# dnbaker/dashing

Hardware: AMD Instinct MI355X
Metric: genome-pairs/sec, all-pairs HLL Jaccard (Ertl-MLE), N=10000 p=14 (higher is better)
Workload: dtype u8/u32 popcount + f64 estimator; 1 GPU; BASELINE configs[2]: 10000 synthetic sketches, p=14 (16384 B each), all-pairs dist on MI355X; n_sketches=10000, p=14, k=31, estimator=ERTL_MLE

## Files before the change

### dashing_amd/csrc/abi.hip

```cpp
#include <algorithm>
#include <cstdlib>
#include <cstring>
#include <new>

#include "ctx.h"

using namespace dsh;

extern "C" {

const char *dsh_backend_name(void) { return "hip:gfx950"; }

int dsh_abi_version(void) { return DSH_ABI_VERSION; }

int dsh_device_count(void)
{
    int n = 0;
    if (hipGetDeviceCount(&n) != hipSuccess) return 0;
    return n;
}

static void release_ctx(dsh_ctx *c)
{
    (void)hipSetDevice(c->device);
    for (const Stream *s : {&c->stream, &c->copy_stream, &c->aux_stream, &c->place_stream})
        if (*s) (void)hipStreamSynchronize(*s);
    if (c->xch.spin_running && c->xch.spin_flag.ptr) *(volatile uint32_t *)c->xch.spin_flag.ptr = 1;
    if (c->spin_stream) (void)hipStreamSynchronize(c->spin_stream);
    c->xch.spin_running = false;
    (void)comm_release(c);
}

int dsh_create(int device, dsh_ctx **out)
{
    if (!out) return DSH_EINVAL;
    *out = nullptr;
    int n = 0;
    if (hipGetDeviceCount(&n) != hipSuccess || n <= 0) return DSH_ENODEV;
    if (device < 0 || device >= n) return DSH_EINVAL;
    hipDeviceProp_t prop;
    if (hipGetDeviceProperties(&prop, device) != hipSuccess) return DSH_ENODEV;
    if (std::strncmp(prop.gcnArchName, "gfx950", 6) != 0) return DSH_ENODEV;
    dsh_ctx *c = new (std::nothrow) dsh_ctx;
    if (!c) return DSH_ENOMEM;
    c->device = device;
    if (hipSetDevice(device) != hipSuccess ||
        c->stream.create() != hipSuccess || c->copy_stream.create_copy() != hipSuccess ||
        c->aux_stream.create() != hipSuccess || c->place_stream.create_copy() != hipSuccess ||
        c->ev_aux_fork.ensure() != hipSuccess || c->ev_aux_join.ensure() != hipSuccess) {
        release_ctx(c);
        delete c;
        return DSH_EIO;
    }
    *out = c;
    return DSH_OK;
}

void dsh_destroy(dsh_ctx *c)
{
    if (!c) return;
    release_ctx(c);
    delete c;
}

int dsh_preload(int device, unsigned what)
{
    if (hipSetDevice(device) != hipSuccess) {
        (void)hipGetLastError();
        return DSH_ENODEV;
    }
    hipError_t e = hipSuccess;
    if ((what & DSH_PRELOAD_SKETCH) && e == hipSuccess) e = preload_sketch_kernels();
    if ((what & DSH_PRELOAD_SKETCH) && e == hipSuccess) e = preload_fastx_kernels();
    if ((what & DSH_PRELOAD_COMPARE) && e == hipSuccess) e = preload_compare_kernels();
    if ((what & DSH_PRELOAD_COMPARE) && e == hipSuccess) e = preload_hist_kernels();
    if ((what & DSH_PRELOAD_COMPARE) && e == hipSuccess) e = preload_knn_kernels();
    if ((what & DSH_PRELOAD_COMPARE) && e == hipSuccess) e = preload_exchange_kernels();
    if (e != hipSuccess) (void)hipGetLastError();
    return e == hipSuccess ? DSH_OK : DSH_EIO;
}

const char *dsh_last_error(const dsh_ctx *c) { return c ? c->err.c_str() : "null ctx"; }

int dsh_synchronize(dsh_ctx *c)
{
    if (!c) return DSH_EINVAL;
    int rc = bind(c);
    if (rc) return rc;
    HIPCHK(c, hipStreamSynchronize(c->stream));
    HIPCHK(c, hipStreamSynchronize(c->copy_stream));
    HIPCHK(c, hipStreamSynchronize(c->place_stream));
    return DSH_OK;
}

void *dsh_stream(dsh_ctx *c) { return c ? (void *)c->stream : nullptr; }

int dsh_sketches_alloc(dsh_ctx *c, uint64_t n, int p)
{
    if (!c) return DSH_EINVAL;
    if (p < 4 || p > kMaxP) return fail(c, DSH_EINVAL, "p=%d outside [4,%d]", p, kMaxP);
    int rc = bind(c);
    if (rc) return rc;
    const size_t bytes = std::max<size_t>((size_t)n << p, 256);
    HIPCHK(c, c->regs_own.ensure(bytes));
    HIPCHK(c, hipMemsetAsync(c->regs_own.ptr, 0, bytes, c->stream));
    c->regs = (const uint8_t *)c->regs_own.ptr;
    c->n = n;
    c->p = p;
    c->have_sketches = true;
    invalidate(c);
    return DSH_OK;
}

int dsh_attach_device_sketches(dsh_ctx *c, const void *d_regs, uint64_t n, int p)
{
    if (!c || (!d_regs && n)) return DSH_EINVAL;
    if (p < 4 || p > kMaxP) return fail(c, DSH_EINVAL, "p=%d outside [4,%d]", p, kMaxP);
    if (((uintptr_t)d_regs & 15) != 0) return fail(c, DSH_EINVAL, "device sketches must be 16-byte aligned");
    c->regs = (const uint8_t *)d_regs;
    c->n = n;
    c->p = p;
    c->have_sketches = true;
    invalidate(c);
    return DSH_OK;
}

int dsh_upload_sketches(dsh_ctx *c, const uint8_t *regs, uint64_t first, uint64_t n)
{
    if (!c || (!regs && n)) return DSH_EINVAL;
    if (!c->have_sketches || c->regs != (const uint8_t *)c->regs_own.ptr)
        return fail(c, DSH_ESTATE, "dsh_sketches_alloc first");
    if (!slots_ok(first, n, c->n)) return fail(c, DSH_EINVAL, "slots [%llu,+%llu) out of range", (unsigned long long)first, (unsigned long long)n);
    int rc = bind(c);
    if (rc) return rc;
    if (n) {
        HIPCHK(c, hipMemcpyAsync((uint8_t *)c->regs_own.ptr + (first << c->p), regs, (size_t)n << c->p,
                                 hipMemcpyHostToDevice, c->stream));
        HIPCHK(c, hipStreamSynchronize(c->stream));
    }
    invalidate(c);
    return DSH_OK;
}

int dsh_download_sketches(dsh_ctx *c, uint64_t first, uint64_t n, uint8_t *out)
{
    if (!c || (!out && n)) return DSH_EINVAL;
    if (!c->have_sketches) return fail(c, DSH_ESTATE, "no sketches");
    if (!slots_ok(first, n, c->n)) return fail(c, DSH_EINVAL, "slots out of range");
    int rc = bind(c);
    if (rc) return rc;
    if (n) {
        HIPCHK(c, hipMemcpyAsync(out, c->regs + (first << c->p), (size_t)n << c->p,
                                 hipMemcpyDeviceToHost, c->stream));
        HIPCHK(c, hipStreamSynchronize(c->stream));
    }
    return DSH_OK;
}

// ... 650 lines not shown

int dsh_last_kernel_ms(dsh_ctx *c, double *pair_ms, double *fin_ms, double *prep_ms, uint32_t *launches)
{
    if (!c) return DSH_EINVAL;
    if (pair_ms) *pair_ms = c->pair_ms;
    if (fin_ms) *fin_ms = c->fin_ms;
    if (prep_ms) *prep_ms = c->prep_ms;
    if (launches) *launches = c->pair_launches;
    return DSH_OK;
}

int dsh_last_part_info(dsh_ctx *c, double *ready_ms, uint64_t *floats, uint32_t cap, uint32_t *nparts_out)
{
    if (!c || !nparts_out) return DSH_EINVAL;
    const uint32_t k = (uint32_t)c->part_ready_ms.size();
    *nparts_out = k;
    if (k > cap && (ready_ms || floats)) return DSH_EINVAL;
    for (uint32_t q = 0; q < k; ++q) {
        if (ready_ms) ready_ms[q] = c->part_ready_ms[q];
        if (floats) floats[q] = c->part_floats[q];
    }
    return DSH_OK;
}

int dsh_finalize_phase_cycles(dsh_ctx *c, uint64_t *out16)
{
    if (!c || !out16) return DSH_EINVAL;
    int rc = bind(c);
    if (rc) return rc;
    if (!c->phase_cyc.ptr) return fail(c, DSH_ESTATE, "no call with the option finalize_timing yet");
    HIPCHK(c, hipStreamSynchronize(c->stream));
    HIPCHK(c, hipMemcpy(out16, c->phase_cyc.ptr, 16 * sizeof(uint64_t), hipMemcpyDeviceToHost));
    return DSH_OK;
}

int dsh_get_info(dsh_ctx *c, const char *name, int64_t *out)
{
    if (!c || !name || !out) return DSH_EINVAL;
    if (!std::strcmp(name, "planes")) *out = c->lay.P;
    else if (!std::strcmp(name, "vlo")) *out = c->lay.vlo;
    else if (!std::strcmp(name, "vhi")) *out = c->lay.vhi;
    else if (!std::strcmp(name, "threshold")) *out = c->lay.pbase + (int64_t)c->lay.P;
    else if (!std::strcmp(name, "pbase")) *out = c->lay.pbase;
    else if (!std::strcmp(name, "host_layout_us")) *out = (int64_t)c->host_layout_us;
    else if (!std::strcmp(name, "host_lists_us")) *out = (int64_t)c->host_lists_us;
    else if (!std::strcmp(name, "host_keys_wait_us")) *out = (int64_t)c->host_keys_wait_us;
    else if (!std::strcmp(name, "emax")) *out = c->emax;
    else if (!std::strcmp(name, "elow")) *out = c->elow;
    else if (!std::strcmp(name, "kc")) *out = c->kc;
    else if (!std::strcmp(name, "pair_groups")) *out = c->pair_groups;
    else if (!std::strcmp(name, "pair_round")) *out = c->pp.band_round.empty() ? 0 : c->pp.band_round[0];
    else if (!std::strcmp(name, "tile")) *out = kTile;
    else if (!std::strcmp(name, "parts_done")) *out = c->parts_done;
    else if (!std::strcmp(name, "parts_signalled")) *out = c->parts_signalled ? 1 : 0;
    else if (!std::strcmp(name, "sketch_kernel_us")) *out = (int64_t)(c->sketch_ms * 1000.0);
    else if (!std::strcmp(name, "fastx_decode_us")) *out = (int64_t)(c->fastx_ms * 1000.0);
    else if (!std::strcmp(name, "xch_recv_gated")) *out = c->xch.recv_gated ? 1 : 0;
    else if (!std::strcmp(name, "stats_route")) *out = c->gs.route_last;
    else if (!std::strcmp(name, "linkage_route")) *out = c->lk.route_last;
    else if (!std::strcmp(name, "mst_rounds")) *out = c->mst.rounds_last;
    else if (!std::strcmp(name, "mst_band_us")) *out = (int64_t)(c->mst.band_ms * 1000.0);
    else if (!std::strcmp(name, "place_kernel_us")) *out = (int64_t)(c->xch.place_ms * 1000.0);
    else if (!std::strcmp(name, "whatif_mfma")) {
#ifdef DSH_WHATIF_MFMA
        *out = 1;
#else
        *out = 0;
#endif
    }
    else if (!std::strcmp(name, "npad")) *out = c->lay.Npad;
    else if (!std::strcmp(name, "kpad")) *out = c->Kpad;
    else if (!std::strcmp(name, "cum_bytes")) *out = c->cum_bytes;
    else if (!std::strcmp(name, "sorted")) *out = c->lay.sorted;
    else if (!std::strcmp(name, "ncols")) *out = (int64_t)c->lay.ncols;
    else if (!std::strcmp(name, "lockstep")) *out = c->planes_valid && use_lockstep(c) ? 1 : 0;
    else if (!std::strcmp(name, "tiles")) *out = (int64_t)c->pp.T.size();
    else if (!std::strcmp(name, "bands")) *out = (int64_t)c->last_bands;
    else if (!std::strcmp(name, "items")) *out = (int64_t)c->pp.items.size();
    else if (!std::strcmp(name, "frag_items")) {
        uint64_t f = 0;
        for (uint32_t x : c->pp.band_frags) f += x;
        *out = (int64_t)f;
    }
    else if (!std::strcmp(name, "words_per_plane")) *out = c->W;
    else if (!std::strcmp(name, "avg_tile_planes_x100")) {
        uint64_t tot = 0;
        for (const auto &t : c->pp.T) tot += t.w - t.z;
        *out = c->pp.T.empty() ? 0 : (int64_t)(tot * 100 / c->pp.T.size());
    }
    else return fail(c, DSH_EINVAL, "unknown info %s", name);
    return DSH_OK;
}

int dsh_set_option(dsh_ctx *c, const char *name, int64_t v)
{
    if (!c || !name) return DSH_EINVAL;
    if (!std::strcmp(name, "kc")) {
        if (v != 0 && v != 16 && v != 32) return fail(c, DSH_EINVAL, "kc must be 0 (auto), 16 or 32");
        c->kc_opt = (int)v;
        c->planes_valid = false;
        return DSH_OK;
    }
    if (!std::strcmp(name, "pair_groups")) {
        if (v != 0 && v != 2 && v != 3) return fail(c, DSH_EINVAL, "pair_groups must be 0 (auto), 2 or 3");
        c->pair_groups_opt = (int)v;
        c->planes_valid = false;
        return DSH_OK;
    }
    if (!std::strcmp(name, "cum_budget_bytes")) {
        if (v < (1 << 20)) return fail(c, DSH_EINVAL, "cum_budget_bytes too small");
        c->cum_budget = (uint64_t)v;
        return DSH_OK;
    }
    if (!std::strcmp(name, "knn_square_budget_bytes")) {
        if (v < 0) return fail(c, DSH_EINVAL, "knn_square_budget_bytes must be >= 0");
        c->knn_square_budget = (uint64_t)v;
        return DSH_OK;
    }
    if (!std::strcmp(name, "threshold_band_bytes")) {
        if (v < 4) return fail(c, DSH_EINVAL, "threshold_band_bytes must be at least 4");
        c->threshold_band_bytes = (uint64_t)v;
        return DSH_OK;
    }
    if (!std::strcmp(name, "pairs_chunk")) {
        if (v < 1 || v > (1 << 24)) return fail(c, DSH_EINVAL, "pairs_chunk must be in [1, 2^24]");
        c->pairs.chunk = (uint64_t)v;
        return DSH_OK;
    }
    if (!std::strcmp(name, "cluster_chunk")) {
        if (v < 1 || v > (1 << 26)) return fail(c, DSH_EINVAL, "cluster_chunk must be in [1, 2^26]");
        c->cc.chunk = (uint64_t)v;
        return DSH_OK;
    }
    if (!std::strcmp(name, "stats_route")) {
        if (v < -1 || v > 1) return fail(c, DSH_EINVAL, "stats_route must be -1 (auto), 0 (dense) or 1 (pairs)");
        c->gs.route = (int)v;
        return DSH_OK;
    }
    if (!std::strcmp(name, "linkage_route")) {
        if (v < -1 || v > 1) return fail(c, DSH_EINVAL, "linkage_route must be -1 (auto), 0 (dense) or 1 (pairs)");
        c->lk.route = (int)v;
        return DSH_OK;
    }
    if (!std::strcmp(name, "linkage_partition")) {
        if (v < 0 || v > 1) return fail(c, DSH_EINVAL, "linkage_partition must be 0 or 1");
        c->lk.partition = (int)v;
        return DSH_OK;
    }
    if (!std::strcmp(name, "linkage_budget_bytes")) {
        if (v < 64) return fail(c, DSH_EINVAL, "linkage_budget_bytes must be at least 64");
        c->lk.budget = (uint64_t)v;
        return DSH_OK;
    }
    if (!std::strcmp(name, "linkage_lds_max")) {
        if (v < 0 || v > 6144) return fail(c, DSH_EINVAL, "linkage_lds_max must be in [0, 6144]");
        c->lk.lds_max = (uint32_t)v;
        return DSH_OK;
    }
    if (!std::strcmp(name, "greedy_band_rows")) {
        if (v < 1 || v > (long long)kGreedyMaxRows) return fail(c, DSH_EINVAL, "greedy_band_rows must be in [1, %u]", kGreedyMaxRows);
        c->gr.band_rows = (uint64_t)v;
        return DSH_OK;
    }
    if (!std::strcmp(name, "derive_chunk_bytes")) {
        if (v < 1) return fail(c, DSH_EINVAL, "derive_chunk_bytes must be at least 1");
        c->derive.chunk_bytes = (uint64_t)v;
        return DSH_OK;
    }
    if (!std::strcmp(name, "sort")) {
        if (v < -1 || v > 1) return fail(c, DSH_EINVAL, "sort must be -1, 0 or 1");
        c->sort_mode = (int)v;
        return DSH_OK;
    }
    if (!std::strcmp(name, "range_sort_min_rows")) {
        if (v < 1) return fail(c, DSH_EINVAL, "range_sort_min_rows must be >= 1");
        c->range_sort_min_rows = (int)std::min<int64_t>(v, 1 << 30);
        return DSH_OK;
    }
#ifdef DSH_WHATIF_MFMA
    if (!std::strcmp(name, "pair_mfma")) {
        c->pair_mfma = v != 0;
        return DSH_OK;
    }
#endif
    if (!std::strcmp(name, "finalize_stop")) {
        if (v < 0 || v > 4) return fail(c, DSH_EINVAL, "finalize_stop must be in [0,4]");
        if (v && !c->profiling) return fail(c, DSH_ESTATE, "finalize_stop needs dsh_set_profiling(ctx, 1)");
        c->finalize_stop = (int)v;
        return DSH_OK;
    }
    if (!std::strcmp(name, "finalize_timing")) {
        if (v && !c->profiling) return fail(c, DSH_ESTATE, "finalize_timing needs dsh_set_profiling(ctx, 1)");
        c->finalize_timing = v != 0;
        return DSH_OK;
    }
    if (!std::strcmp(name, "nsplit")) {
        if (v < 0 || v > 64) return fail(c, DSH_EINVAL, "nsplit must be in [0,64]");
        c->nsplit = (int)v;
        return DSH_OK;
    }
    if (!std::strcmp(name, "emax") || !std::strcmp(name, "elow")) {
        if (v < -1 || v > (int64_t)kMaxListSide) return fail(c, DSH_EINVAL, "%s must be in [-1,%u]", name, kMaxListSide);
        (name[1] == 'm' ? c->emax_opt : c->elow_opt) = (int)v;
        return DSH_OK;
    }
    if (!std::strcmp(name, "part_band_tiles")) {
        if (v < 1 || v > (1 << 30)) return fail(c, DSH_EINVAL, "part_band_tiles out of range");
        c->part_band_tiles = (int)v;
        return DSH_OK;
    }
    if (!std::strcmp(name, "xch_tail_bands")) {
        if (v < 0 || v > 8) return fail(c, DSH_EINVAL, "xch_tail_bands out of range");
        c->tail_bands = (int)v;
        return DSH_OK;
    }
    if (!std::strcmp(name, "overflow_frag_permille")) {
        if (v < 0 || v > 1000) return fail(c, DSH_EINVAL, "overflow_frag_permille out of range");
        c->overflow_frag_permille = (int)v;
        return DSH_OK;
    }
    if (!std::strcmp(name, "xch_recv_gate")) {
        if (v < -1 || v > 1) return fail(c, DSH_EINVAL, "xch_recv_gate is -1 (auto), 0 or 1");
        c->xch.recv_gate = (int)v;
        return DSH_OK;
    }
    if (!std::strcmp(name, "finalize_signal")) {
        if (v < -1 || v > 1) return fail(c, DSH_EINVAL, "finalize_signal is -1 (auto), 0 or 1");
        c->finalize_signal = (int)v;
        return DSH_OK;
    }
    return fail(c, DSH_EINVAL, "unknown option %s", name);
}

}
```

### dashing_amd/csrc/ctx.h

```cpp
#pragma once
#include <hip/hip_runtime.h>
#include <rccl/rccl.h>

#include <cstdarg>
#include <cstdio>
#include <cstdlib>
#include <deque>
#include <string>
#include <vector>

#include "../../include/dashing_hip.h"
#include "kernels.h"
#include "plan.h"

struct NoCopy {
    NoCopy() = default;
    NoCopy(const NoCopy &) = delete;
    NoCopy &operator=(const NoCopy &) = delete;
};

struct DevBuf : NoCopy {
    void *ptr = nullptr;
    size_t cap = 0;
    ~DevBuf() { release(); }
// ... 64 lines not shown
        int least = 0, greatest = 0;
        if (hipDeviceGetStreamPriorityRange(&least, &greatest) != hipSuccess) greatest = 0;
        if (const char *e = std::getenv("DSH_COPY_STREAM_PRIORITY")) greatest = std::atoi(e);
        return hipStreamCreateWithPriority(&st, hipStreamNonBlocking, greatest);
    }
    operator hipStream_t() const { return st; }
};

struct Staging : NoCopy {
    PinBuf buf;
    Event sent_ev;
    bool in_flight = false;
    hipError_t wait()
    {
        if (!in_flight) return hipSuccess;
        const hipError_t e = hipEventSynchronize(sent_ev);
        if (e == hipSuccess) in_flight = false;
        return e;
    }
    hipError_t room(size_t bytes)
    {
        const hipError_t e = wait();
        return e == hipSuccess ? buf.ensure(bytes) : e;
    }
    hipError_t sent(hipStream_t st)
    {
        hipError_t e = sent_ev.ensure();
        if (e == hipSuccess) e = hipEventRecord(sent_ev, st);
        if (e == hipSuccess) in_flight = true;
        return e;
    }
    void *ptr() const { return buf.ptr; }
};

struct dsh_ctx {
    int device = 0;
    Stream stream;
    Stream copy_stream;
    Stream aux_stream;
    Stream place_stream;
    Stream spin_stream;
    std::string err;
    DevBuf regs_own;
    const uint8_t *regs = nullptr;
    uint64_t n = 0;
    int p = 0;
    bool have_sketches = false;
    bool planes_valid = false;
    int card_estim = -1;
    uint64_t card_from = 0;
    uint64_t pass_gen = 0, lay_gen = 0;
    DevBuf card, planes, cum, tiles, items, outbuf, exc, excv, exc_n, keys, perm, tailhist;
    Event ev_aux_fork, ev_aux_join;
    bool aux_join_pending = false;
    DevBuf outbuf2[2];
    Event ev_filled[2];
    Event ev_drained[2];
    bool drained_pending[2] = {false, false};
    unsigned out_turn = 0;
    std::deque<Event> tickets;
    uint64_t ticket_next = 0;
    Event ev_first_tiles;
    bool pass_from_zero = false;
    DevBuf hist;
    Event ev_keys;
    DevBuf cidx_rec, cidx_ent;
    uint32_t nbuckets = 0, ent_stride = 0;
    DevBuf colS_n, colS_key, colS_card, colS_th, colS_rl;
    uint32_t rl_stride = 0;
    dsh::plan::Layout lay;
    bool lay_built = false;
    dsh::plan::PairPlan pp;
    std::deque<Event> ev_part;
    uint32_t parts_done = 0;
    DevBuf sig;
    Staging st_sig;
    uint32_t sig_gen = 0;
    bool parts_signalled = false;
    int finalize_signal = -1;
    int can_wait_value = -1;
    int wall_clock_khz = 0;
    PinBuf pin_keys;
    const uint32_t *hk32 = nullptr;
    bool hk32_valid = false;
    double host_layout_us = 0, host_lists_us = 0, host_keys_wait_us = 0;
    Staging st_perm;
    DevBuf rowoff;
    Staging st_lists;
    uint32_t W = 0, Kpad = 0;
    int emax = 0, elow = 0, cum_bytes = 4;
    int kc = 16;
    int kc_opt = 0;
    int pair_groups = 3;
    int pair_groups_opt = 0;
    int emax_opt = -1;
    int elow_opt = -1;
    int part_band_tiles = 2048;
    int overflow_frag_permille = 500;
    int tail_bands = 2;
    std::vector<double> part_ready_ms;
    std::vector<uint64_t> part_floats;
    size_t last_bands = 0;
    uint64_t cum_budget = 8ull << 30;
    int sort_mode = -1;
    int range_sort_min_rows = 1024;
    DevBuf thr_vals;
    uint64_t threshold_band_bytes = (uint64_t)1 << 30;
    uint64_t knn_square_budget = (uint64_t)96 << 30;
    int pair_mfma = 0;
    int finalize_stop = 0;
    int finalize_timing = 0;
    DevBuf phase_cyc;
    int nsplit = 0;
    bool profiling = false;
    double pair_ms = 0, fin_ms = 0, prep_ms = 0, sketch_ms = 0, fastx_ms = 0;
    uint32_t pair_launches = 0;
    std::deque<Event> ev_pool;
    size_t ev_used = 0;

    struct {
        DevBuf seqbuf, workbuf, recbuf;
        Staging work, rec;
        DevBuf rawbuf, fx_tab, fx_summ, fx_state, fx_declen, fx_status;
        Staging fx;
    } sketch;
    struct {
        DevBuf cnt, off, total, col, val, rowptr;
    } thr;
    struct {
        DevBuf card, hist, lhs, rhs, out, err;
        Staging list;
        int card_estim = -1;
        uint64_t chunk = 1u << 18;
    } pairs;
    struct {
        DevBuf parent, state, lhs, rhs, rowptr, seed, labels;
        uint64_t chunk = 1u << 20;
    } cc;
    struct {
        DevBuf assign, state, labels;
        DevBuf best;
        uint64_t band_rows = 4096;
    } gr;
    struct {
        DevBuf labels, acc, grp, out, csr;
        int route = -1;
        int route_last = -1;
    } gs;
    struct {
        DevBuf edges, labels, counts;
        int cus = 0;
    } hs;
    struct {
        DevBuf tab, cells, nodes, labels, state;
        uint64_t budget = 8ull << 30;
        uint32_t lds_max = 4096;
        int partition = 1;
        int route = -1;
        int route_last = -1;
    } lk;
    struct {
        DevBuf best, ckey, cedge, elhs, erhs, ekey, state;
        int rounds_last = 0;
        double band_ms = 0;
    } mst;
    struct {
        DevBuf degree, best, kind, state;
    } db;
    struct {
        DevBuf err, stage, ptr, mem, dst, part[2], out;
        uint64_t chunk_bytes = (uint64_t)256 << 20;
    } derive;
    struct {
        ncclComm_t comm = nullptr;
        int rank = 0, world = 1;
        DevBuf gather_full, gather_local;
        DevBuf stage, tab;
        Staging tabs;
        DevBuf place_tab;
        bool recv_gated = false;
        int recv_gate = -1;
// ... 186 lines not shown
```

### dashing_amd/csrc/engine.hip

```cpp
#include <algorithm>
#include <chrono>
#include <cstring>

#include "ctx.h"

namespace dsh {

int prepare(dsh_ctx *c, int estim, int want_sorted, bool card_only, uint64_t want_rb, uint64_t want_re, uint32_t nparts,
            int rowsorted, const std::vector<uint64_t> *extra_in)
{
    static const std::vector<uint64_t> kNoExtra;
    std::vector<uint64_t> extra_cached;
    const std::vector<uint64_t> *extra = extra_in ? extra_in : &kNoExtra;
    if (!c->have_sketches) return fail(c, DSH_ESTATE, "no sketches loaded");
    if (estim < 0 || estim > 2) return fail(c, DSH_EINVAL, "bad estimator %d", estim);
    if (want_sorted < 0) {
        want_sorted = c->lay.sorted;
        want_rb = c->lay.rb;
        want_re = c->lay.re;
        rowsorted = 0;
        extra_cached = c->lay.extra;
        extra = &extra_cached;
    }
    if (!want_sorted) rowsorted = 0, extra = &kNoExtra;
    if (want_re > c->n) want_re = c->n;
    if (!want_sorted) want_rb = 0, want_re = c->n;
    if (want_rb > want_re) want_rb = want_re;
    const uint64_t n = c->n;
    std::vector<uint64_t> parts, rs_pos;
    if (want_rb >= want_re) extra = &kNoExtra;
    if (want_sorted && !rowsorted) {
        if (extra->empty()) plan::range_parts(n, want_rb, want_re, std::max<uint32_t>(nparts, 1), parts);
        else parts = {want_rb, want_re};
    }
    if (rowsorted) plan::rowsorted_part_positions(n, want_rb, want_re, std::max<uint32_t>(nparts, 1), rs_pos, extra);
    const int emax_new = c->emax_opt >= 0 ? std::min<int>(c->emax_opt, (int)kMaxListSide) : plan::auto_list_cap(c->p, true);
    const int elow_new = c->elow_opt >= 0 ? std::min<int>(c->elow_opt, (int)kMaxListSide) : plan::auto_list_cap(c->p, false);
    if (emax_new != c->emax || elow_new != c->elow) {
        c->planes_valid = false;
        c->card_estim = -1;
    }
    c->emax = emax_new;
    c->elow = elow_new;
    const bool same_layout = c->planes_valid && c->lay_gen == c->pass_gen && c->lay.sorted == want_sorted &&
                             (!want_sorted || (c->lay.rb == want_rb && c->lay.re == want_re && c->lay.rowsorted == rowsorted &&
                                               c->lay.extra == *extra && (rowsorted ? c->lay.part_w == rs_pos : c->lay.parts == parts)));
    const uint64_t need_from = (card_only || !want_sorted || c->pass_from_zero) ? 0 : want_rb;
    const bool have_pass = c->card_estim == estim && c->card_from <= need_from;
    if (have_pass && (card_only || same_layout)) return DSH_OK;
    const bool keep_layout = same_layout && have_pass;
    DeviceTimer timer(c, c->stream);
    if (!have_pass) {
        HIPCHK(c, c->card.ensure(std::max<uint64_t>(n, 1) * sizeof(double)));
        HIPCHK(c, c->exc.ensure(std::max<uint64_t>(n, 1) * kListCap * (c->p <= 15 ? 2 : 4)));
        HIPCHK(c, c->excv.ensure(std::max<uint64_t>(n, 1) * kListCap));
        HIPCHK(c, c->exc_n.ensure(std::max<uint64_t>(n, 1) * sizeof(uint32_t)));
        HIPCHK(c, c->keys.ensure(std::max<uint64_t>(n, 1) * sizeof(uint32_t)));
        HIPCHK(c, c->tailhist.ensure(std::max<uint64_t>(n, 1) * 64));
        HIPCHK(c, c->hist.ensure(std::max<uint64_t>(n, 1) * 64 * sizeof(uint32_t)));
        HIPCHK(c, launch_selfhist_card(c->stream, c->regs, need_from, n, c->p, estim, c->emax, c->elow,
                                       (uint32_t *)c->hist.ptr, c->exc.ptr, (uint8_t *)c->excv.ptr,
                                       (uint32_t *)c->exc_n.ptr, (uint32_t *)c->keys.ptr,
                                       (uint8_t *)c->tailhist.ptr));
        HIPCHK(c, c->pin_keys.ensure(std::max<uint64_t>(n, 1) * sizeof(uint32_t)));
        c->hk32 = (const uint32_t *)c->pin_keys.ptr;
        if (n > need_from)
            HIPCHK(c, hipMemcpyAsync((uint32_t *)c->pin_keys.ptr + need_from, (const uint32_t *)c->keys.ptr + need_from,
                                     (n - need_from) * sizeof(uint32_t), hipMemcpyDeviceToHost, c->stream));
        HIPCHK(c, c->ev_keys.ensure());
        HIPCHK(c, hipEventRecord(c->ev_keys, c->stream));
        HIPCHK(c, launch_card_from_hist(c->stream, (const uint32_t *)c->hist.ptr, (const uint32_t *)c->keys.ptr, need_from, n,
                                        c->p, estim, (double *)c->card.ptr));
        c->card_estim = estim;
        c->card_from = need_from;
        c->hk32_valid = false;
        ++c->pass_gen;
    }
    if (card_only) {
        timer.stop(c->prep_ms, true);
        return DSH_OK;
    }
#ifdef DSH_EXPERIMENT_REUSE_LAYOUT
    const bool reuse_host_layout = !keep_layout && c->lay_built && c->lay.n == n && c->lay.sorted == want_sorted &&
                                   (!want_sorted || (c->lay.rb == want_rb && c->lay.re == want_re && c->lay.rowsorted == rowsorted &&
                                                     c->lay.extra == *extra && (rowsorted ? c->lay.part_w == rs_pos : c->lay.parts == parts)));
#else
    constexpr bool reuse_host_layout = false;
#endif
    if (!keep_layout) {
        if (c->p > kMaxPCompare)
            return fail(c, DSH_EINVAL, "the compare path takes p <= %d (p=%d: sketching and cardinalities only)", kMaxPCompare, c->p);
        if (c->pair_groups_opt == 3 && c->kc_opt == 32)
            return fail(c, DSH_EINVAL, "pair_groups = 3 needs kc = 16 (or kc = 0, auto)");
        const auto t_h0 = std::chrono::steady_clock::now();
        if (!c->hk32_valid && !reuse_host_layout) {
            HIPCHK(c, hipEventSynchronize(c->ev_keys));
            c->hk32_valid = true;
        }
        const auto t_h1 = std::chrono::steady_clock::now();
        c->host_keys_wait_us = std::chrono::duration<double, std::micro>(t_h1 - t_h0).count();
        const uint32_t *k32 = c->hk32;
        for (uint64_t i = c->card_from; i < n && !reuse_host_layout; ++i)
            if (plan::key_bad(k32[i]))
                return fail(c, DSH_EINVAL, "sketch %llu holds a register value above %d (= 64 - p + 1): not an HLL of precision %d (corrupt or foreign .hll?)",
                            (unsigned long long)i, 64 - c->p + 1, c->p);
        c->planes_valid = false;
        plan::Layout &L = c->lay;
        if (!reuse_host_layout)
            plan::build_layout(k32, n, want_sorted, want_rb, want_re, parts, L, rowsorted ? std::max<uint32_t>(nparts, 1) : 0,
                               extra->empty() ? nullptr : extra);
        c->lay_built = true;
        c->cum_bytes = c->p <= 15 ? 2 : 4;
        const uint64_t m = 1ull << c->p;
        c->W = (uint32_t)std::max<uint64_t>(1, m / 32);
        c->pair_groups = c->pair_groups_opt ? c->pair_groups_opt : (c->kc_opt == 32 ? 2 : 3);
        c->kc = c->pair_groups == 3 ? 16 : c->kc_opt ? c->kc_opt : (c->W >= 32 ? 32 : 16);
        if (want_sorted && !reuse_host_layout) {
            const uint64_t nperm = L.perm.size();
            HIPCHK(c, c->perm.ensure(std::max<uint64_t>(nperm, 1) * sizeof(uint32_t)));
            if (nperm) {
                const size_t pb_ = (nperm * sizeof(uint32_t) + 15) & ~(size_t)15;
                const size_t rb_ = L.rowsorted ? L.rowoff.size() * sizeof(uint64_t) : 0;
                HIPCHK(c, c->st_perm.room(pb_ + rb_));
                uint8_t *h = (uint8_t *)c->st_perm.ptr();
                std::memcpy(h, L.perm.data(), nperm * sizeof(uint32_t));
                HIPCHK(c, launch_upload(c->stream, c->perm.ptr, h, nperm * sizeof(uint32_t)));
                if (L.rowsorted) {
                    HIPCHK(c, c->rowoff.ensure(rb_));
                    std::memcpy(h + pb_, L.rowoff.data(), rb_);
                    HIPCHK(c, launch_upload(c->stream, c->rowoff.ptr, h + pb_, rb_));
                }
                HIPCHK(c, c->st_perm.sent(c->stream));
            }
        }
        const uint32_t NT = L.Npad / kTile;
        c->nbuckets = (uint32_t)std::min<uint64_t>(2 * m, kMaxBuckets);
        c->ent_stride = std::max<uint32_t>(1, kTile * (uint32_t)(c->emax + c->elow));
        c->rl_stride = std::max<uint32_t>(1, (uint32_t)(c->emax + c->elow));
        const size_t nbk = std::max<size_t>(NT, 1);
        HIPCHK(c, c->cidx_rec.ensure(nbk * c->nbuckets * (size_t)(colindex_inline(c->p, c->rl_stride) + 1) * sizeof(uint32_t)));
        HIPCHK(c, c->cidx_ent.ensure(nbk * c->ent_stride * sizeof(uint32_t)));
        HIPCHK(c, c->colS_n.ensure(nbk * kTile * sizeof(uint32_t)));
        HIPCHK(c, c->colS_key.ensure(nbk * kTile * sizeof(uint32_t)));
        HIPCHK(c, c->colS_card.ensure(nbk * kTile * sizeof(double)));
        HIPCHK(c, c->colS_th.ensure(nbk * kTile * 64));
        HIPCHK(c, c->colS_rl.ensure(nbk * kTile * (size_t)c->rl_stride * sizeof(uint32_t)));
        c->host_layout_us = std::chrono::duration<double, std::micro>(std::chrono::steady_clock::now() - t_h1).count();
        HIPCHK(c, hipEventRecord(c->ev_aux_fork, c->stream));
        HIPCHK(c, hipStreamWaitEvent(c->aux_stream, c->ev_aux_fork, 0));
        {
            ColIndexLaunch ci;
            ci.exc = c->exc.ptr;
            ci.excv = (const uint8_t *)c->excv.ptr;
            ci.exc_n = (const uint32_t *)c->exc_n.ptr;
            ci.keys = (const uint32_t *)c->keys.ptr;
            ci.card = (const double *)c->card.ptr;
            ci.tailhist = (const uint8_t *)c->tailhist.ptr;
            ci.perm = want_sorted ? (const uint32_t *)c->perm.ptr : nullptr;
            ci.ncols = L.ncols;
            ci.p = c->p;
            ci.nblocks = NT;
            ci.nbuckets = c->nbuckets;
            ci.ent_stride = c->ent_stride;
            ci.E = c->rl_stride;
            ci.rec = (uint32_t *)c->cidx_rec.ptr;
            ci.ent = (uint32_t *)c->cidx_ent.ptr;
            ci.nS = (uint32_t *)c->colS_n.ptr;
            ci.keyS = (uint32_t *)c->colS_key.ptr;
            ci.cardS = (double *)c->colS_card.ptr;
            ci.thS = (uint8_t *)c->colS_th.ptr;
            ci.rl = (uint32_t *)c->colS_rl.ptr;
            HIPCHK(c, launch_build_colindex(c->aux_stream, ci));
        }
        HIPCHK(c, hipEventRecord(c->ev_aux_join, c->aux_stream));
        const uint64_t K = (uint64_t)L.P * c->W;
        c->Kpad = (uint32_t)((K + c->kc - 1) / c->kc * c->kc);
        if (c->Kpad) {
            const size_t bytes = (size_t)c->Kpad * L.Npad * sizeof(uint32_t);
            HIPCHK(c, c->planes.ensure(bytes));
            if (c->Kpad > K)
                HIPCHK(c, hipMemsetAsync((uint32_t *)c->planes.ptr + K * L.Npad, 0,
                                         (size_t)(c->Kpad - K) * L.Npad * sizeof(uint32_t),
                                         c->stream));
            HIPCHK(c, launch_transform(c->stream, c->regs, L.ncols, c->p, L.pbase, L.P, c->W, L.Npad,
                                       (uint32_t *)c->planes.ptr,
                                       want_sorted ? (const uint32_t *)c->perm.ptr : nullptr));
        }
        c->aux_join_pending = true;
        c->lay_gen = c->pass_gen;
        c->planes_valid = true;
    }
    timer.stop(c->prep_ms, true);
    return DSH_OK;
}

namespace {

struct JobLayout {
    int want_sorted = 0;
    uint64_t lrb = 0, lre = 0;
    bool with_parts = false;
    bool with_extra = false;
};

struct PairRun {
    plan::Tuning tu;
    std::vector<uint64_t> item_off;
    plan::U4 *pinT = nullptr, *pinF = nullptr, *pinI = nullptr;
    bool signal = false;
    bool sig_upload = false;
    FinalizeLaunch fin{};
    hipEvent_t e_call0 = nullptr;
    std::vector<std::pair<size_t, hipEvent_t>> ev_part_t;
    std::vector<std::pair<hipEvent_t, hipEvent_t>> evp, evf;
};

JobLayout choose_layout(const dsh_ctx *c, const PairJob &job)
{
    JobLayout jl;
    const uint64_t jre = std::min<uint64_t>(job.row_end, c->n);
    const bool full_tri = !job.rect && job.row_begin == 0 && jre >= c->n;
    jl.with_parts = job.nparts > 0 && !job.rect && !job.sorted_rows;
    jl.lre = c->n;
    if (job.sorted_rows) jl.want_sorted = 1;
    else if (!job.rect && jre > job.row_begin &&
             (jl.with_parts || (c->sort_mode != 0 && (full_tri || jre - job.row_begin >= (uint64_t)c->range_sort_min_rows)))) {
        jl.want_sorted = 1;
        jl.lrb = job.row_begin;
        jl.lre = jre;
    }
    jl.with_extra = jl.want_sorted && jl.with_parts && !job.extra.empty() && jl.lre > jl.lrb;
    return jl;
}

plan::Tuning tuning_of(const dsh_ctx *c)
{
    plan::Tuning tu;
    tu.W = c->W;
    tu.kc = c->kc;
    tu.cum_bytes = c->cum_bytes;
    tu.cum_budget = c->cum_budget;
    tu.nsplit = c->nsplit;
    tu.lockstep = use_lockstep(c);
    tu.round_items = 256u * (uint32_t)c->pair_groups;
    tu.small_round_items = c->pair_groups_opt == 0 && c->pair_groups == 3 ? 512u : 0u;
    tu.part_band_tiles = (uint32_t)c->part_band_tiles;
    tu.overflow_frag_max_permille = (uint32_t)c->overflow_frag_permille;
    tu.tail_bands = (uint32_t)c->tail_bands;
    return tu;
}

int reserve_lists(dsh_ctx *c, PairRun &r)
{
    plan::PairPlan &pp = c->pp;
    const std::vector<plan::U4> &T = pp.T;
    r.item_off.assign(pp.bands.size() + 1, 0);
    for (size_t bi = 0; bi < pp.bands.size(); ++bi) r.item_off[bi + 1] = r.item_off[bi] + plan::band_item_count(r.tu, pp, bi);
    const uint64_t nitems_total = r.item_off.back();
    pp.items.reserve(nitems_total);
    static_assert(sizeof(plan::U4) == sizeof(uint4), "plan::U4 must have the layout of uint4");
    HIPCHK(c, c->st_lists.room((2 * T.size() + std::max<uint64_t>(nitems_total, 1)) * sizeof(uint4)));
    r.pinT = (plan::U4 *)c->st_lists.ptr(), r.pinF = r.pinT + T.size(), r.pinI = r.pinF + T.size();
    HIPCHK(c, c->tiles.ensure(2 * T.size() * sizeof(uint4)));
    HIPCHK(c, c->items.ensure(std::max<uint64_t>(nitems_total, 1) * sizeof(uint4)));
    HIPCHK(c, c->cum.ensure(std::max<uint64_t>(pp.per_tile_bytes * pp.max_band, 256)));
    return DSH_OK;
}

int stage_signal_block(dsh_ctx *c, PairRun &r)
{
    ++c->sig_gen;
    if (c->sig_gen == 0) c->sig_gen = 1;
    HIPCHK(c, c->st_sig.room((2 * kSigMaxParts + 2) * sizeof(uint32_t)));
    static_assert(kSigPartTotal == kSigPartCnt + kSigMaxParts && kSigGen == kSigPartTotal + kSigMaxParts && kSigStamp == kSigGen + 1, "signal block layout");
    uint32_t *blk = (uint32_t *)c->st_sig.ptr(), *tot = blk + kSigMaxParts;
    for (uint32_t qd = 0; qd < kSigMaxParts; ++qd) blk[qd] = 0u;
    for (uint32_t qd = 0; qd < kSigMaxParts; ++qd) tot[qd] = qd < c->pp.part_tiles.size() ? c->pp.part_tiles[qd] : 0u;
    tot[kSigMaxParts] = c->sig_gen;
    tot[kSigMaxParts + 1] = c->profiling ? 1u : 0u;
    r.sig_upload = true;
    return DSH_OK;
}

FinalizeLaunch finalize_invariants(const dsh_ctx *c, const PairJob &job, bool with_extra)
{
    const plan::Layout &L = c->lay;
    FinalizeLaunch f{};
    f.cum_bytes = c->cum_bytes;
    FinalizeArgs &a = f.a;
    a.cum = c->cum.ptr;
    a.perm = L.sorted ? (const uint32_t *)c->perm.ptr : nullptr;
    a.rowoff = L.rowsorted ? (const uint64_t *)c->rowoff.ptr : nullptr;
    a.pbase = L.pbase;
    a.p = c->p;
    a.estim = job.estim;
    a.result_type = job.result_type;
    a.ksinv = job.ksinv_double ? 1. / (double)job.k : (double)(float)(1. / (double)job.k);
    a.nS = (const uint32_t *)c->colS_n.ptr;
    a.keyS = (const uint32_t *)c->colS_key.ptr;
    a.cardS = (const double *)c->colS_card.ptr;
    a.thS = (const uint8_t *)c->colS_th.ptr;
    a.rl = (const uint32_t *)c->colS_rl.ptr;
    a.E = c->rl_stride;
    a.cidx_rec = (const uint32_t *)c->cidx_rec.ptr;
    a.cidx_ent = (const uint32_t *)c->cidx_ent.ptr;
    a.nbuckets = c->nbuckets;
    a.ent_stride = c->ent_stride;
    a.n = c->n;
    a.ncols = L.ncols;
    a.rect = job.rect;
    a.sorted_out = job.sorted_rows;
    a.square = job.square;
    a.knn = job.knn;
    a.out2 = job.d_out2;
    a.knn_ld = job.knn_ld;
    a.knn_rows = job.knn_rows;
    a.stop = c->finalize_stop;
    a.phase_cyc = c->finalize_timing ? (unsigned long long *)c->phase_cyc.ptr : nullptr;
    a.row_begin = job.row_begin;
    a.row_end = with_extra ? c->n : job.row_end;
    a.col_begin = job.col_begin;
    a.col_end = job.col_end;
    a.base_index = job.base_index;
    a.out = job.d_out;
    return f;
}

int upload_band(dsh_ctx *c, PairRun &r, size_t bi)
{
    plan::PairPlan &pp = c->pp;
    const auto &bd = pp.bands[bi];
    const uint32_t nt = (uint32_t)(bd.second - bd.first);
    const size_t nT = pp.T.size();
    const auto t_b0 = std::chrono::steady_clock::now();
    plan::build_band_items(r.tu, pp, bi);
    if (pp.band_items[bi].first != r.item_off[bi] || pp.band_items[bi].second != r.item_off[bi + 1])
        return fail(c, DSH_EIO, "internal: band %zu has %zu items, %llu were planned for", bi,
                    pp.band_items[bi].second - pp.band_items[bi].first, (unsigned long long)(r.item_off[bi + 1] - r.item_off[bi]));
    plan::emit_band_lists(c->lay, pp, bi, r.pinT, r.pinF);
    const uint32_t ni = (uint32_t)(r.item_off[bi + 1] - r.item_off[bi]);
    if (ni) std::memcpy(r.pinI + r.item_off[bi], pp.items.data() + r.item_off[bi], (size_t)ni * sizeof(uint4));
    c->host_lists_us += std::chrono::duration<double, std::micro>(std::chrono::steady_clock::now() - t_b0).count();
    UploadSegs up;
    uint32_t nseg = 0;
    if (r.sig_upload) up.add(nseg, (uint32_t *)c->sig.ptr + kSigPartCnt, c->st_sig.ptr(), (2 * kSigMaxParts + 2) * sizeof(uint32_t));
    up.add(nseg, (uint4 *)c->tiles.ptr + bd.first, r.pinT + bd.first, (size_t)nt * sizeof(uint4));
    up.add(nseg, (uint4 *)c->tiles.ptr + nT + bd.first, r.pinF + bd.first, (size_t)nt * sizeof(uint4));
    up.add(nseg, (uint4 *)c->items.ptr + r.item_off[bi], r.pinI + r.item_off[bi], (size_t)ni * sizeof(uint4));
    HIPCHK(c, launch_upload_segs(c->stream, up, nseg));
    if (r.sig_upload) {
        HIPCHK(c, c->st_sig.sent(c->stream));
        r.sig_upload = false;
    }
    HIPCHK(c, c->st_lists.sent(c->stream));
    return DSH_OK;
}

int launch_tile_kernel(dsh_ctx *c, const PairRun &r, size_t bi, uint64_t nslots)
{
    const plan::Layout &L = c->lay;
    const plan::PairPlan &pp = c->pp;
    const uint4 *dt = (const uint4 *)c->tiles.ptr + pp.bands[bi].first;
    const uint4 *di = (const uint4 *)c->items.ptr + r.item_off[bi];
    const uint32_t ni = (uint32_t)(r.item_off[bi + 1] - r.item_off[bi]);
    if (c->pair_mfma)
        HIPCHK(c, launch_pair_counts_mfma(c->stream, c->kc, c->cum_bytes, (const uint32_t *)c->planes.ptr,
                                          L.Npad, c->Kpad, c->W, L.P, dt, di, ni, c->cum.ptr, nslots));
    else if (use_lockstep(c))
        HIPCHK(c, launch_pair_counts_lockstep(c->stream, c->kc, (int)(pp.band_round[bi] / 256), c->cum_bytes, (const uint32_t *)c->planes.ptr,
                                              L.Npad, c->Kpad, c->W, L.P, dt, di, ni, bi < pp.band_frags.size() ? pp.band_frags[bi] : 0u,
                                              c->cum.ptr, nslots));
    else
        HIPCHK(c, launch_pair_counts(c->stream, c->kc, c->cum_bytes, (const uint32_t *)c->planes.ptr,
                                     L.Npad, c->Kpad, c->W, L.P, dt, di, ni, c->cum.ptr, nslots));
    return DSH_OK;
}

int finalize_band(dsh_ctx *c, PairRun &r, size_t bi)
{
    const plan::PairPlan &pp = c->pp;
    const auto &bd = pp.bands[bi];
    std::vector<plan::Seg> one_seg;
    if (r.signal) {
        plan::Seg all{bd.first, bd.second, -1, 1};
        for (const plan::Seg &sg : pp.segs[bi]) all.hist_bins = std::max(all.hist_bins, sg.hist_bins);
        one_seg.push_back(all);
    }
    for (const plan::Seg &sg : r.signal ? one_seg : pp.segs[bi]) {
        hipStream_t fst = c->stream;
        FinalizeLaunch &f = r.fin;
        f.a.hist_bins = sg.hist_bins;
        f.a.tiles = (const uint4 *)c->tiles.ptr + pp.T.size() + sg.b;
        f.nslots = (uint64_t)(sg.e - sg.b) * kTile * kTile;
        f.a.sig = r.signal ? (uint32_t *)c->sig.ptr : nullptr;
        if (c->aux_join_pending) {
            HIPCHK(c, hipStreamWaitEvent(c->stream, c->ev_aux_join, 0));
            c->aux_join_pending = false;
        }
        HIPCHK(c, launch_finalize(fst, f));
        if (sg.part >= 0) {
            const size_t qp = (size_t)sg.part;
            while (c->ev_part.size() <= qp) HIPCHK(c, add_event(c->ev_part));
            HIPCHK(c, hipEventRecord(c->ev_part[qp], fst));
            c->parts_done = (uint32_t)qp + 1;
            if (r.e_call0) {
                hipEvent_t te = next_event(c);
                if (te) {
                    (void)hipEventRecord(te, fst);
                    r.ev_part_t.emplace_back(qp, te);
                }
            }
        }
    }
    return DSH_OK;
}

int read_profile(dsh_ctx *c, const PairRun &r)
{
    const plan::Layout &L = c->lay;
    HIPCHK(c, hipStreamSynchronize(c->stream));
    for (auto &e : r.evp) {
        float ms = 0;
        (void)hipEventElapsedTime(&ms, e.first, e.second);
        c->pair_ms += ms;
        if (c->Kpad) c->pair_launches++;
    }
    for (auto &e : r.evf) {
        float ms = 0;
        (void)hipEventElapsedTime(&ms, e.first, e.second);
        c->fin_ms += ms;
    }
    auto fill_part_floats = [&] {
        for (size_t i = 0; i < c->part_floats.size(); ++i) {
            if (L.rowsorted && i + 1 < L.part_w.size()) c->part_floats[i] = L.rowoff_w[L.part_w[i + 1]] - L.rowoff_w[L.part_w[i]];
            else if (!L.rowsorted && L.extra.empty() && i + 1 < L.parts.size()) c->part_floats[i] = plan::tri_span(c->n, L.parts[i], L.parts[i + 1]);
            else if (!L.rowsorted) c->part_floats[i] = plan::rowset_span(c->n, L.rb, L.re, L.extra);
        }
    };
    if (r.signal && r.e_call0 && c->wall_clock_khz > 0) {
        std::vector<unsigned long long> st(kSigMaxParts + 1);
        HIPCHK(c, hipMemcpy(st.data(), (uint32_t *)c->sig.ptr + kSigPartTime, kSigMaxParts * sizeof(unsigned long long), hipMemcpyDeviceToHost));
        HIPCHK(c, hipMemcpy(&st[kSigMaxParts], (uint32_t *)c->sig.ptr + kSigT0, sizeof(unsigned long long), hipMemcpyDeviceToHost));
        c->part_ready_ms.assign(c->parts_done, 0.0);
        c->part_floats.assign(c->parts_done, 0);
        for (size_t i = 0; i < c->part_ready_ms.size(); ++i)
            c->part_ready_ms[i] = (double)(long long)(st[i] - st[kSigMaxParts]) / (double)c->wall_clock_khz;
        fill_part_floats();
    } else if (r.e_call0 && !r.ev_part_t.empty()) {
        c->part_ready_ms.assign(c->parts_done, 0.0);
        c->part_floats.assign(c->parts_done, 0);
        for (auto &pe : r.ev_part_t) {
            float ms = 0;
            (void)hipEventElapsedTime(&ms, r.e_call0, pe.second);
            if (pe.first < c->part_ready_ms.size()) c->part_ready_ms[pe.first] = ms;
        }
        fill_part_floats();
    }
    return DSH_OK;
}

}

int run_pairs(dsh_ctx *c, const PairJob &job)
{
    PairRun r;
    const JobLayout jl = choose_layout(c, job);
    c->parts_done = 0;
    c->part_ready_ms.clear();
    c->part_floats.clear();
    if (jl.with_parts) {
        HIPCHK(c, c->sig.ensure((size_t)kSigWords * sizeof(uint32_t)));
        if (c->sig_gen == 0) {
            HIPCHK(c, hipMemsetAsync(c->sig.ptr, 0, (size_t)kSigWords * sizeof(uint32_t), c->stream));
            c->sig_gen = 1;
        }
    }
    if (c->profiling && jl.with_parts) {
        r.e_call0 = next_event(c);
        if (r.e_call0) (void)hipEventRecord(r.e_call0, c->stream);
        HIPCHK(c, launch_wall_stamp(c->stream, reinterpret_cast<unsigned long long *>((uint32_t *)c->sig.ptr + kSigT0)));
    }
    if (!job.extra.empty() && !jl.with_extra) return fail(c, DSH_EINVAL, "internal: extra row segments need a key-ordered range with parts");
    int rc = prepare(c, job.estim, jl.want_sorted, false, jl.lrb, jl.lre, jl.with_parts ? job.nparts : 1, jl.with_parts && job.rowsorted,
                     jl.with_extra ? &job.extra : nullptr);
    if (rc) return rc;
    if (job.result_type < 0 || job.result_type > 8)
        return fail(c, DSH_EINVAL, "unsupported result_type %d", job.result_type);
    if (job.k < 1) return fail(c, DSH_EINVAL, "bad k %d", job.k);
    const auto t_l0 = std::chrono::steady_clock::now();
    plan::PairPlan &pp = c->pp;
    plan::PairQuery q;
    q.rect = job.rect;
    q.sorted_rows = job.sorted_rows;
    q.want_parts = jl.with_parts;
    q.row_begin = job.row_begin;
    q.row_end = job.row_end;
    q.col_begin = job.col_begin;
    q.col_end = job.col_end;
    r.tu = tuning_of(c);
    if (!plan::build_tiles(c->lay, q, r.tu, pp)) {
        pp.T.clear();
        return DSH_OK;
    }
    c->last_bands = pp.bands.size();
    if ((rc = reserve_lists(c, r))) return rc;
    c->host_lists_us = std::chrono::duration<double, std::micro>(std::chrono::steady_clock::now() - t_l0).count();

    if (jl.with_parts && pp.nparts >= 1 && pp.nparts <= kSigMaxParts && !c->finalize_timing && !c->finalize_stop && c->finalize_signal != 0) {
        r.signal = device_can_wait_value(c);
        if (!r.signal && c->finalize_signal == 1) return fail(c, DSH_ENODEV, "option finalize_signal = 1, but the device does not support hipStreamWaitValue32");
    }
    c->parts_signalled = r.signal;
    if (r.signal && (rc = stage_signal_block(c, r))) return rc;
    if (c->finalize_timing) {
        HIPCHK(c, c->phase_cyc.ensure(16 * sizeof(unsigned long long)));
        HIPCHK(c, hipMemsetAsync(c->phase_cyc.ptr, 0, 16 * sizeof(unsigned long long), c->stream));
    }
    r.fin = finalize_invariants(c, job, jl.with_extra);
    for (size_t bi = 0; bi < pp.bands.size(); ++bi) {
        const uint64_t nslots = (uint64_t)(pp.bands[bi].second - pp.bands[bi].first) * kTile * kTile;
        if ((rc = upload_band(c, r, bi))) return rc;
        hipEvent_t a = nullptr, b = nullptr, d = nullptr;
        if (c->profiling) {
            a = next_event(c);
            b = next_event(c);
            d = next_event(c);
            if (a) (void)hipEventRecord(a, c->stream);
        }
        if ((rc = launch_tile_kernel(c, r, bi, nslots))) return rc;
        if (b) (void)hipEventRecord(b, c->stream);
        if (bi == 0) {
            HIPCHK(c, c->ev_first_tiles.ensure());
            HIPCHK(c, hipEventRecord(c->ev_first_tiles, c->stream));
        }
        r.fin.a.nslots = nslots;
        if ((rc = finalize_band(c, r, bi))) return rc;
        if (d) (void)hipEventRecord(d, c->stream);
        if (a && b && d) {
            r.evp.emplace_back(a, b);
            r.evf.emplace_back(b, d);
        }
    }
    if (r.signal) c->parts_done = pp.nparts;
    return c->profiling ? read_profile(c, r) : DSH_OK;
}

}
```

### dashing_amd/csrc/host/plan_capi.cpp

```cpp
#include <algorithm>
#include <cstdarg>
#include <cstdio>
#include <cstring>
#include <vector>

#include "../linkage.h"
#include "../mst.h"
#include "../plan.h"
#include "../uf.h"

using namespace dsh;
using namespace dsh::plan;

namespace {

struct Err {
    char *buf;
    size_t cap;
    int fail(const char *fmt, ...)
    {
        if (buf && cap) {
            va_list ap;
            va_start(ap, fmt);
            vsnprintf(buf, cap, fmt, ap);
            va_end(ap);
        }
        return -1;
    }
};

}

static int plan_check(uint64_t n, const uint32_t *keys, int mode, int want_sorted, uint64_t rb, uint64_t re, uint64_t cb,
                      uint64_t ce, uint32_t nparts, int want_parts, int p, uint64_t cum_budget, int lockstep, int nsplit,
                      int ls_item_chunks, const std::vector<uint64_t> &extra, uint64_t *stats, char *err, size_t cap,
                      uint32_t round_items = 0)
{
    Err E{err, cap};
    if (re > n) re = n;
    const bool rowsorted = mode == 3;
    if (rowsorted) mode = 0, want_sorted = 1, want_parts = 1;
    if (mode == 1 || !want_sorted) want_sorted = mode == 2 ? 1 : 0;
    if (mode == 2) want_sorted = 1;
    std::vector<uint64_t> parts;
    uint64_t lrb = 0, lre = n;
    if (want_sorted && mode == 0) lrb = rb, lre = re;
    if (want_sorted && !rowsorted) range_parts(n, lrb, lre, std::max<uint32_t>(want_parts ? nparts : 1, 1), parts);
    if (!extra.empty() && !(want_sorted && mode == 0)) return E.fail("extra segments need a sorted triangle layout");
    Layout L;
    build_layout(keys, n, want_sorted, lrb, lre, parts, L, rowsorted ? std::max<uint32_t>(nparts, 1) : 0, extra.empty() ? nullptr : &extra);
    std::vector<std::pair<uint64_t, uint64_t>> wsegs;
    wanted_order(n, lrb, lre, &extra, wsegs, rowsorted);
    auto in_rows = [&](uint64_t i) {
        for (auto &w : wsegs)
            if (i >= w.first && i < w.second) return true;
        return false;
    };
    uint64_t nw = 0, wspan = 0;
    for (auto &w : wsegs) nw += w.second - w.first, wspan += tri_span(n, w.first, w.second);
    if (want_sorted && mode == 0 && L.nwanted != nw) return E.fail("nwanted %llu != %llu", (unsigned long long)L.nwanted, (unsigned long long)nw);
    if (rowsorted) {
        auto skey = [&](uint32_t g) { return ((uint32_t)key_T(keys[g]) << 12) | ((uint32_t)key_L(keys[g]) << 6) | (uint32_t)key_hi(keys[g]); };
        for (auto &w : wsegs)
            for (uint64_t s = w.first - lrb + 1; s < w.second - lrb; ++s)
                if (skey(L.perm[s - 1]) > skey(L.perm[s])) return E.fail("row-sorted: a wanted segment is not one key-ordered run at %llu", (unsigned long long)s);
        if (L.part_w.empty() || L.part_w.front() != 0 || L.part_w.back() != nw) return E.fail("row-sorted: part cuts do not span the wanted rows");
        for (size_t q = 1; q + 1 < L.part_w.size(); ++q) {
            if (L.part_w[q] <= L.part_w[q - 1]) return E.fail("row-sorted: cut %zu at %llu", q, (unsigned long long)L.part_w[q]);
            uint64_t w0 = 0;
            bool ok = false;
            for (auto &w : wsegs) {
                if (L.part_w[q] >= w0 && L.part_w[q] < w0 + (w.second - w.first)) ok = (L.part_w[q] - w0) % kTile == 0;
                w0 += w.second - w.first;
            }
            if (!ok) return E.fail("row-sorted: cut %zu at %llu is not at a tile row of the wanted order", q, (unsigned long long)L.part_w[q]);
        }
        if (L.part_w.size() - 1 > std::max<uint32_t>(nparts, 1)) return E.fail("row-sorted: more parts than asked for");
        uint64_t acc = 0, w_ = 0;
        if (L.rowoff_w.size() != nw + 1) return E.fail("row-sorted: rowoff_w size");
        for (auto &w : wsegs)
            for (uint64_t s = w.first - lrb; s < w.second - lrb; ++s, ++w_) {
                if (s >= L.rowoff.size() || L.rowoff[s] != acc || L.rowoff_w[w_] != acc) return E.fail("row-sorted: rowoff[%llu]", (unsigned long long)s);
                acc += n - 1 - L.perm[s];
            }
        if (L.rowoff_w.back() != acc || acc != wspan) return E.fail("row-sorted: the rows do not add up to the span");
    }
    const uint64_t col0 = want_sorted ? lrb : 0;
    if (L.ncols != n - col0) return E.fail("ncols %llu != %llu", (unsigned long long)L.ncols, (unsigned long long)(n - col0));
    if (L.Npad % kTile || L.Npad < L.ncols || L.Npad >= L.ncols + kTile) return E.fail("bad Npad %u", L.Npad);
    std::vector<uint8_t> seen(n, 0);
    for (uint64_t s = 0; s < L.ncols; ++s) {
        const uint32_t g = L.perm[s];
        if (g < col0 || g >= n || seen[g]) return E.fail("perm[%llu] = %u is out of range or repeated", (unsigned long long)s, g);
        seen[g] = 1;
    }
    if (want_sorted) {
        uint64_t s = 0;
        for (size_t q = 0; q + 1 < L.parts.size(); ++q)
            for (uint64_t r = L.parts[q]; r < L.parts[q + 1]; ++r, ++s)
                if (L.perm[s] < L.parts[q] || L.perm[s] >= L.parts[q + 1])
                    return E.fail("column %llu holds sketch %u, not a row of part %zu", (unsigned long long)s, L.perm[s], q);
        if (!rowsorted && extra.empty()) {
            if (L.part_pos.size() != L.parts.size()) return E.fail("part positions and parts differ in number");
            for (size_t q = 0; q < L.parts.size(); ++q)
                if (L.part_pos[q] != L.parts[q] - lrb) return E.fail("part position %zu", q);
        }
        for (; s < L.ncols; ++s)
            if (L.perm[s] < lre) return E.fail("column %llu (after the wanted rows) holds wanted row %u", (unsigned long long)s, L.perm[s]);
        for (auto &w : wsegs)
            for (uint64_t s2 = w.first - lrb; s2 < w.second - lrb; ++s2)
                if (L.perm[s2] < w.first || L.perm[s2] >= w.second) return E.fail("position %llu of a wanted segment holds row %u", (unsigned long long)s2, L.perm[s2]);
        if (!extra.empty())
            for (uint64_t s2 = 0; s2 < L.ncols; ++s2) {
                const uint64_t b = s2 / kTile * kTile;
                if (in_rows(L.perm[s2]) != in_rows(L.perm[b])) return E.fail("block %llu mixes wanted and other rows", (unsigned long long)(b / kTile));
            }
        if (L.whole)
            for (uint64_t i = 0; i < n; ++i)
                if (L.perm[n + L.perm[i]] != i) return E.fail("inverse permutation wrong at %llu", (unsigned long long)i);
    }
    Tuning tu;
    const uint64_t m = 1ull << p;
    tu.W = (uint32_t)std::max<uint64_t>(1, m / 32);
    tu.kc = tu.W >= 32 ? 32 : 16;
    tu.cum_bytes = p <= 15 ? 2 : 4;
    tu.cum_budget = cum_budget;
    tu.nsplit = nsplit;
    tu.lockstep = lockstep && tu.W >= (uint32_t)tu.kc;
    tu.ls_item_chunks = ls_item_chunks;
    if (round_items) tu.round_items = round_items;
    if (round_items > 512) tu.small_round_items = 512;
    PairQuery q;
    q.rect = mode == 1;
    q.sorted_rows = mode == 2;
    q.want_parts = want_parts && mode == 0 && want_sorted;
    q.row_begin = rb;
    q.row_end = re;
    q.col_begin = cb;
    q.col_end = ce;
    PairPlan pp;
    const bool any = build_pairs(L, q, tu, pp);
    for (int i = 0; i < 9; ++i) stats[i] = 0;
    stats[5] = L.Npad;
    stats[6] = L.P;
    std::vector<uint8_t> hit;
    uint64_t wanted = 0;
    auto orig = [&](uint64_t s) -> uint64_t { return L.perm[s]; };
    if (mode == 1) {
        const uint64_t nr = re > rb ? re - rb : 0, nc = ce > cb ? ce - cb : 0;
        wanted = nr * nc;
        hit.assign(wanted, 0);
    } else {
        hit.assign(n * n, 0);
        for (uint64_t i = rb; i < re; ++i) wanted += n - 1 - i;
        for (size_t x = 0; x + 1 < extra.size(); x += 2)
            for (uint64_t i = extra[x]; i < extra[x + 1]; ++i) wanted += n - 1 - i;
        if (mode == 2) {
            wanted = 0;
            for (uint64_t si = rb; si < re; ++si) wanted += n - 1 - si;
        }
    }
    if (!any) {
        if (wanted) return E.fail("nothing planned although %llu pairs are wanted", (unsigned long long)wanted);
        return 0;
    }
    const std::vector<U4> &T = pp.T;
    uint64_t got = 0, planes_sum = 0;
    for (const U4 &t : T) {
        if (t.z > t.w || t.w > L.P) return E.fail("tile (%u,%u) has the plane range [%u,%u) of %u", t.x, t.y, t.z, t.w, L.P);
        planes_sum += t.w - t.z;
        for (uint32_t a = 0; a < kTile; ++a)
            for (uint32_t b = 0; b < kTile; ++b) {
                const uint64_t si = (uint64_t)t.x * kTile + a, sj = (uint64_t)t.y * kTile + b;
                if (si >= L.ncols || sj >= L.ncols) continue;
                const uint64_t i = orig(si), j = orig(sj);
                bool active;
                uint64_t slot;
                if (mode == 1) {
                    active = i >= rb && i < re && j >= cb && j < ce;
                    slot = active ? (i - rb) * (ce - cb) + (j - cb) : 0;
                } else if (mode == 2) {
                    active = si < sj && si >= rb && si < re;
                    slot = si * n + sj;
                } else {
                    const uint64_t oi = std::min(i, j), oj = std::max(i, j);
                    active = si < sj && oi >= rb && oi < (extra.empty() ? re : n);
                    slot = oi * n + oj;
                    if (active && !extra.empty() && !in_rows(oi))
                        return E.fail("tile (%u,%u) computes the pair (%llu,%llu) of a row this rank does not hold", t.x, t.y, (unsigned long long)oi, (unsigned long long)oj);
                }
                if (!active) continue;
                if (hit[slot]++) return E.fail("pair slot %llu computed twice (tile %u,%u)", (unsigned long long)slot, t.x, t.y);
                ++got;
                const uint32_t ka = keys[i], kb = keys[j];
                const int Tp = L.pbase + (int)t.w, Lp = L.pbase + (int)t.z;
                if (Tp < std::max(key_T(ka), key_T(kb))) return E.fail("tile (%u,%u): T %d below a sketch's threshold", t.x, t.y, Tp);
                if (Lp > std::max(std::max(key_lo(ka), key_lo(kb)), std::min(key_L(ka), key_L(kb))))
                    return E.fail("tile (%u,%u): Lp %d above what the low lists cover", t.x, t.y, Lp);
            }
    }
    if (got != wanted) return E.fail("%llu of %llu wanted pairs are covered", (unsigned long long)got, (unsigned long long)wanted);
    size_t at = 0;
    if (pp.bands.size() != pp.segs.size() || pp.bands.size() != pp.band_items.size()) return E.fail("band bookkeeping sizes differ");
    std::vector<int> part_done(pp.nparts, 0);
    int last_part = -1;
    for (size_t bi = 0; bi < pp.bands.size(); ++bi) {
        const auto &bd = pp.bands[bi];
        if (bd.first != at || bd.second <= bd.first || bd.second > T.size()) return E.fail("band %zu = [%zu,%zu) does not follow %zu", bi, bd.first, bd.second, at);
        at = bd.second;
        if (bd.second - bd.first > 1 && (bd.second - bd.first) * pp.per_tile_bytes > cum_budget)
            return E.fail("band %zu needs %llu bytes of C(v), budget %llu", bi, (unsigned long long)((bd.second - bd.first) * pp.per_tile_bytes), (unsigned long long)cum_budget);
        size_t sa = bd.first;
        for (const Seg &sg : pp.segs[bi]) {
            if (sg.b != sa || sg.e <= sg.b || sg.e > bd.second) return E.fail("segment [%zu,%zu) of band %zu does not follow %zu", sg.b, sg.e, bi, sa);
            sa = sg.e;
            if (sg.part >= 0) {
                if ((uint32_t)sg.part >= pp.nparts || part_done[sg.part]++ || sg.part != last_part + 1)
                    return E.fail("part %d completed out of order or twice", sg.part);
                last_part = sg.part;
            }
            if (q.want_parts)
                for (size_t t = sg.b; t < sg.e; ++t) {
                    uint64_t pos0 = ~0ull;
                    for (size_t k = 0; k < L.wtr.size(); ++k)
                        if (T[t].x >= L.wtr[k].first && T[t].x < L.wtr[k].second) pos0 = L.wtr_w[k] + (uint64_t)(T[t].x - L.wtr[k].first) * kTile;
                    const int cur = last_part + (sg.part >= 0 ? 0 : 1);
                    if (cur < 0 || (size_t)cur + 1 >= L.part_w.size() || pos0 < L.part_w[cur] || pos0 >= L.part_w[cur + 1])
                        return E.fail("tile row %u is not in part %d", T[t].x, cur);
                }
        }
        if (sa != bd.second) return E.fail("segments of band %zu end at %zu, not %zu", bi, sa, bd.second);
        const auto &bi_ = pp.band_items[bi];
        if (band_item_count(tu, pp, bi) != bi_.second - bi_.first) return E.fail("band %zu: band_item_count disagrees with the items built", bi);
        std::vector<uint32_t> next(bd.second - bd.first);
        for (size_t t = bd.first; t < bd.second; ++t) next[t - bd.first] = pp.chunks[t].x;
        std::vector<std::vector<std::pair<uint32_t, uint32_t>>> per(bd.second - bd.first);
        const uint32_t cpp_ = tu.W >= (uint32_t)tu.kc ? tu.W / tu.kc : 1;
        const uint32_t nfr = bi < pp.band_frags.size() ? pp.band_frags[bi] : 0u;
        const uint32_t bri = bi < pp.band_round.size() ? pp.band_round[bi] : 0u;
        if (bri != tu.round_items && !(tu.small_round_items && bri == tu.small_round_items)) return E.fail("band %zu: round of %u items", bi, bri);
        if (bi == 0 && round_items) stats[9] = bri;
        if (nfr > bi_.second - bi_.first || nfr > bri) return E.fail("band %zu: %u fragments", bi, nfr);
        if (nfr && (!tu.lockstep || (bi_.second - bi_.first - nfr) % bri)) return E.fail("band %zu: fragments behind %zu whole items", bi, bi_.second - bi_.first - nfr);
        stats[8] += nfr;
        for (size_t it = bi_.first; it < bi_.second; ++it) {
            const U4 &I = pp.items[it];
            if (I.x >= per.size() || I.y >= I.z) return E.fail("item %zu is malformed", it);
            const bool frag = it >= bi_.second - nfr;
            if ((I.w != 0) != frag) return E.fail("item %zu: fragment flag %u at the wrong place", it, I.w);
            if (frag && (I.y / cpp_ != (I.z - 1) / cpp_ || I.z - I.y != pp.items[bi_.second - 1].z - pp.items[bi_.second - 1].y))
                return E.fail("fragment %zu spans two planes or differs in length", it);
            per[I.x].emplace_back(I.y, I.z | (frag ? 0x80000000u : 0u));
        }
        for (size_t t = 0; t < per.size(); ++t) {
            std::sort(per[t].begin(), per[t].end());
            uint32_t x = pp.chunks[bd.first + t].x;
            for (size_t k = 0; k < per[t].size(); ++k) {
                auto &pr = per[t][k];
                const bool frag = (pr.second & 0x80000000u) != 0;
                pr.second &= 0x7FFFFFFFu;
                if (pr.first != x) return E.fail("items of tile %zu leave a gap or overlap at chunk %u", t, x);
                if (!frag && tu.W >= (uint32_t)tu.kc && ((pr.first % cpp_) || (pr.second % cpp_))) return E.fail("an item of tile %zu is not whole planes", t);
                if (frag && (pr.first % cpp_) && !(k > 0 && (per[t][k - 1].second & 0x7FFFFFFFu) == pr.first))
                    return E.fail("a fragment of tile %zu starts inside a plane that fragments do not cover from its start", t);
                x = pr.second;
            }
            if (x != pp.chunks[bd.first + t].y) return E.fail("items of tile %zu end at chunk %u, not %u", t, x, pp.chunks[bd.first + t].y);
        }
    }
    if (at != T.size()) return E.fail("bands end at %zu of %zu tiles", at, T.size());
    for (uint32_t qd = 0; qd < pp.nparts; ++qd)
        if (part_done[qd] != 1) return E.fail("part %u never completes", qd);
    if (pp.nparts) {
        uint64_t tsum = 0;
        if (pp.part_tiles.size() != pp.nparts) return E.fail("part_tiles has %zu entries for %u parts", pp.part_tiles.size(), pp.nparts);
        for (uint32_t c : pp.part_tiles) tsum += c;
        if (tsum != T.size()) return E.fail("the parts hold %llu tiles of %zu", (unsigned long long)tsum, T.size());
    }
    if (q.want_parts && pp.nparts + 1 != L.part_w.size()) return E.fail("%u parts planned, layout has %zu", pp.nparts, L.part_w.size() - 1);
    std::vector<U4> dt(T.size()), df(T.size());
    emit_tile_lists(L, pp, dt.data(), df.data());
    for (size_t bi = 0; bi < pp.bands.size(); ++bi)
        for (const Seg &sg : pp.segs[bi]) {
            std::vector<uint8_t> used(pp.bands[bi].second - pp.bands[bi].first, 0);
            for (size_t t = sg.b; t < sg.e; ++t) {
                const U4 &f = df[t];
                const uint32_t fw = f.w & 0xFFFFu, fpart = f.w >> 16;
                const size_t src = pp.bands[bi].first + fw;
                if (fw >= used.size() || src < sg.b || src >= sg.e || used[fw]++) return E.fail("finalize list names a C(v) block twice or outside its segment");
                if (pp.nparts) {
                    if (fpart >= pp.nparts || src < pp.part_first[fpart] || src >= pp.part_first[fpart + 1])
                        return E.fail("finalize list entry %zu carries part %u, which does not hold tile %zu", t, fpart, src);
                } else if (fpart) {
                    return E.fail("finalize list entry %zu carries a part without parts", t);
                }
                if (f.x != T[src].x || f.y != T[src].y || (f.z & 0xFFu) != T[src].z || ((f.z >> 8) & 0xFFu) != T[src].w)
                    return E.fail("finalize list entry %zu does not match tile %zu", t, src);
                if (dt[src].x != T[src].x || dt[src].y != T[src].y || dt[src].z != (T[src].z | (T[src].w << 8)))
                    return E.fail("tile list entry %zu is wrong", src);
                const int lo = (int)((f.z >> 16) & 0xFFu), hi = (int)(f.z >> 24);
                if (hi - lo + 1 > sg.hist_bins) return E.fail("segment hist_bins %d too small for tile %zu", sg.hist_bins, src);
            }
            {
                std::vector<uint32_t> rows_seen;
                for (size_t t = sg.b + 1; t < sg.e; ++t) {
                    if (df[t - 1].x == df[t].x) {
                        if (df[t - 1].y >= df[t].y) return E.fail("finalize list of a segment is not row-major at %zu", t);
                    } else {
                        rows_seen.push_back(df[t - 1].x);
                        if (std::find(rows_seen.begin(), rows_seen.end(), df[t].x) != rows_seen.end())
                            return E.fail("finalize list of a segment returns to tile row %u at %zu", df[t].x, t);
                    }
                }
            }
        }
    stats[0] = T.size();
    stats[1] = pp.bands.size();
    stats[2] = pp.items.size();
    stats[3] = pp.nparts;
    stats[4] = T.empty() ? 0 : planes_sum * 100 / T.size();
    stats[7] = 0;
    for (size_t b = 0; b < pp.band_items.size(); ++b) {
        const uint32_t nfr = b < pp.band_frags.size() ? pp.band_frags[b] : 0u;
        const uint32_t bri = pp.band_round[b];
        stats[7] += (pp.band_items[b].second - pp.band_items[b].first - nfr + bri - 1) / bri + (nfr ? 1 : 0);
    }
    return 0;
}

extern "C" {

int dshh_plan_check(uint64_t n, const uint32_t *keys, int mode, int want_sorted, uint64_t rb, uint64_t re, uint64_t cb,
                    uint64_t ce, uint32_t nparts, int want_parts, int p, uint64_t cum_budget, int lockstep, int nsplit,
                    int ls_item_chunks, uint64_t *stats, char *err, size_t cap)
{
    return plan_check(n, keys, mode, want_sorted, rb, re, cb, ce, nparts, want_parts, p, cum_budget, lockstep, nsplit, ls_item_chunks,
                      std::vector<uint64_t>(), stats, err, cap);
}

int dshh_plan_check_ri(uint64_t n, const uint32_t *keys, int mode, int want_sorted, uint64_t rb, uint64_t re, uint64_t cb,
                       uint64_t ce, uint32_t nparts, int want_parts, int p, uint64_t cum_budget, int lockstep, int nsplit,
                       int ls_item_chunks, uint32_t round_items, uint64_t *stats, char *err, size_t cap)
{
    Err E{err, cap};
    if (round_items == 0 || round_items % 256) return E.fail("round_items %u is not a positive multiple of 256", round_items);
    return plan_check(n, keys, mode, want_sorted, rb, re, cb, ce, nparts, want_parts, p, cum_budget, lockstep, nsplit, ls_item_chunks,
                      std::vector<uint64_t>(), stats, err, cap, round_items);
}

int dshh_plan_check_rowset(uint64_t n, const uint32_t *keys, const uint64_t *tab, uint32_t rank, int rowsorted, uint32_t nparts, int p,
                           uint64_t cum_budget, uint64_t *stats, char *err, size_t cap)
{
    Err E{err, cap};
    RowSets rs;
    if (const char *why = parse_rowsets(tab, n, rs)) return E.fail("%s", why);
    if (rank >= rs.world) return E.fail("rank %u of %u", rank, rs.world);
    uint64_t rb, re;
    std::vector<uint64_t> extra;
    rs.rank_rows(rank, rb, re, extra);
    for (int i = 0; i < 9; ++i) stats[i] = 0;
    if (rb >= re) return 0;
    return plan_check(n, keys, rowsorted ? 3 : 0, 1, rb, re, 0, 0, rowsorted ? nparts : 1, 1, p, cum_budget, 1, 0, 64, extra, stats, err, cap);
}

uint64_t dshh_rowsorted_split(uint64_t n, uint64_t rb, uint64_t re) { return rowsorted_split(n, rb, re); }

int64_t dshh_threshold_bands(uint64_t n, uint64_t rb, uint64_t re, uint64_t ncols, uint64_t band_bytes, uint64_t row_cap,
                             uint64_t *bounds, uint64_t cap)
{
    const uint64_t band_floats = std::max<uint64_t>(band_bytes / sizeof(float), 1);
    if (!ncols && re > n) re = n;
    uint64_t nb = 0;
    if (cap) bounds[0] = rb;
    for (uint64_t b0 = rb; b0 < re;) {
        b0 = ncols ? std::min<uint64_t>(re, b0 + rect_band_rows(ncols, band_floats)) : tri_band_end(n, b0, re, band_floats, row_cap);
        if (++nb >= cap) return -1;
        bounds[nb] = b0;
    }
    return (int64_t)nb;
}

uint64_t dshh_hist_grid(uint64_t units, uint64_t lds_bytes, uint32_t cus, uint64_t *iters)
{
    const uint64_t grid = hist_grid(units, lds_bytes, cus);
    if (iters) *iters = units / (4 * grid) + (units % (4 * grid) ? 1 : 0);
    return grid;
}

int64_t dshh_greedy_bands(uint64_t n, uint64_t band_bytes, uint64_t row_cap, uint64_t *bounds, uint64_t cap)
{
    const uint64_t band_floats = std::max<uint64_t>(band_bytes / sizeof(float), 1);
    uint64_t nb = 0;
    if (cap) bounds[0] = 0;
    for (uint64_t b0 = 0; b0 + 1 < n;) {
        b0 = tri_band_end(n, b0, n, band_floats, row_cap);
        if (++nb >= cap) return -1;
        bounds[nb] = b0;
    }
    return (int64_t)nb;
}

int64_t dshh_greedy_extend_bands(const uint32_t *labels_in, uint64_t m, uint64_t n, uint64_t band_bytes, uint64_t *bounds, uint64_t cap)
{
    if (m > n) return -1;
    const uint64_t band_floats = std::max<uint64_t>(band_bytes / sizeof(float), 1);
    uint64_t nb = 0, b0 = 0, b1 = 0;
    for (uint64_t from = 0; greedy_old_band(labels_in, m, n - m, from, band_floats, b0, b1); from = b1) {
        if (2 * nb + 2 > cap) return -1;
        bounds[2 * nb] = b0;
        bounds[2 * nb + 1] = b1;
        ++nb;
    }
    return (int64_t)nb;
}

int dsh_plan_uf_labels(uint64_t n, const uint32_t *lhs, const uint32_t *rhs, uint64_t n_edges, uint32_t step_cap, uint32_t *labels_out)
{
    if (n > 0xFFFFFFFFull) return -1;
    std::vector<uint32_t> parent(n);
    for (uint64_t x = 0; x < n; ++x) parent[x] = (uint32_t)x;
    for (uint64_t e = 0; e < n_edges; ++e) {
        if (lhs[e] >= n || rhs[e] >= n) return -1;
        uint32_t why = 0;
        if (uf_unite<UfPlain>(parent.data(), lhs[e], rhs[e], step_cap, &why) == kUfOverrun) return (int)why;
    }
    for (uint64_t x = 0; x < n; ++x) {
        const uint32_t l = uf_find<UfPlain>(parent.data(), (uint32_t)x, step_cap);
        if (l == kUfOverrun) return (int)kUfErrFind;
        labels_out[x] = l;
    }
// ... 68 lines not shown
```

### dashing_amd/csrc/kernels.h

```cpp
#pragma once
#include <hip/hip_runtime.h>
#include <stdint.h>

#include "consts.h"

namespace dsh {

hipError_t launch_selfhist_card(hipStream_t st, const uint8_t *regs, uint64_t first, uint64_t n, int p, int estim,
                                int emax, int elow, uint32_t *hist, void *exc, uint8_t *excv, uint32_t *exc_n,
                                uint32_t *keys, uint8_t *tailhist);
hipError_t launch_card_from_hist(hipStream_t st, const uint32_t *hist, const uint32_t *keys, uint64_t first, uint64_t n, int p,
                                 int estim, double *card);
inline int colindex_inline(int p, uint32_t E) { return p <= 12 && E <= 256 ? 7 : 3; }
struct ColIndexLaunch {
    const void *exc;
    const uint8_t *excv;
    const uint32_t *exc_n, *keys;
    const double *card;
    const uint8_t *tailhist;
    const uint32_t *perm;
    uint64_t ncols;
    int p;
    uint32_t nblocks, nbuckets, ent_stride, E;
    uint32_t *rec;
    uint32_t *ent;
    uint32_t *nS, *keyS;
    double *cardS;
    uint8_t *thS;
    uint32_t *rl;
};
hipError_t launch_build_colindex(hipStream_t st, const ColIndexLaunch &c);
hipError_t launch_transform(hipStream_t st, const uint8_t *regs, uint64_t n, int p, int vlo,
                            uint32_t P, uint32_t W, uint32_t Npad, uint32_t *planes,
                            const uint32_t *perm);
hipError_t launch_pair_counts(hipStream_t st, int kc, int cum_bytes, const uint32_t *planes,
                              uint32_t Npad, uint32_t Kpad, uint32_t W, uint32_t P,
                              const uint4 *tiles, const uint4 *items, uint32_t nitems, void *cum,
                              uint64_t nslots);

hipError_t launch_pair_counts_lockstep(hipStream_t st, int kc, int groups, int cum_bytes, const uint32_t *planes,
                                       uint32_t Npad, uint32_t Kpad, uint32_t W, uint32_t P, const uint4 *tiles,
                                       const uint4 *items, uint32_t nitems, uint32_t nfrag, void *cum, uint64_t nslots);
hipError_t launch_pair_counts_mfma(hipStream_t st, int kc, int cum_bytes, const uint32_t *planes,
                                   uint32_t Npad, uint32_t Kpad, uint32_t W, uint32_t P,
                                   const uint4 *tiles, const uint4 *items, uint32_t nitems, void *cum,
                                   uint64_t nslots);

struct FinalizeArgs {
    const void *cum;
    uint64_t nslots;
    const uint4 *tiles;
    const uint32_t *perm;
    const uint64_t *rowoff;
    int hist_bins;
    int pbase;
    int p;
    int estim;
    int result_type;
    double ksinv;
    const uint32_t *nS;
    const uint32_t *keyS;
    const double *cardS;
    const uint8_t *thS;
    const uint32_t *rl;
    uint32_t E;
    const uint32_t *cidx_rec;
    const uint32_t *cidx_ent;
    uint32_t nbuckets, ent_stride;
    uint64_t n;
    uint64_t ncols;
    int rect;
    int sorted_out;
    int square;
    int knn;
    float *out2;
    uint64_t knn_ld, knn_rows;
    int stop;
    uint32_t ntiles;
    unsigned long long *phase_cyc;
    uint64_t row_begin, row_end, col_begin, col_end;
    uint64_t base_index;
    float *out;
    uint32_t *sig;
};
static_assert(sizeof(FinalizeArgs) == 272, "the kernel argument of k_finalize changed its layout");
struct FinalizeLaunch {
    FinalizeArgs a;
    int cum_bytes;
    uint64_t nslots;
};
hipError_t launch_finalize(hipStream_t st, const FinalizeLaunch &f);
constexpr uint32_t kSigMaxParts = 256;
constexpr uint32_t kSigPartFlag = 0, kSigPartCnt = kSigMaxParts, kSigPartTotal = 2 * kSigMaxParts,
                   kSigGen = 3 * kSigMaxParts, kSigStamp = kSigGen + 1,
                   kSigPartTime = 3 * kSigMaxParts + 2, kSigT0 = 5 * kSigMaxParts + 2, kSigTileCnt = 5 * kSigMaxParts + 4,
                   kSigWords = kSigTileCnt + 65536;
struct UploadSeg {
    uint32_t *dst;
    const uint32_t *src;
    uint64_t nwords;
};
struct UploadSegs {
    UploadSeg s[4];
    void add(uint32_t &n, void *dst, const void *src, size_t bytes)
    {
        if (!bytes) return;
        s[n].dst = (uint32_t *)dst, s[n].src = (const uint32_t *)src, s[n].nwords = (bytes + 3) / 4;
        ++n;
    }
};
hipError_t launch_upload_segs(hipStream_t st, const UploadSegs &u, uint32_t nseg);
hipError_t launch_wall_stamp(hipStream_t st, unsigned long long *out);
struct PlaceEnt {
    const float *src;
    const uint32_t *order;
    const uint64_t *rowoff;
    uint64_t pos0;
    uint32_t row0, nrows;
};
hipError_t launch_rows_place(hipStream_t st, const PlaceEnt *ent, uint32_t nent, uint32_t total_rows, float *out, uint64_t n);
hipError_t launch_row_place(hipStream_t st, const float *src, float *out, const uint32_t *order, const uint64_t *rowoff,
// ... 87 lines not shown
    uint64_t room;
};
hipError_t launch_mst_band(hipStream_t st, const float *vals, const ThrRows &g, float cutoff, int descending, const uint32_t *labels,
                           uint64_t *best_v);
hipError_t launch_mst_pick(hipStream_t st, const uint64_t *best_v, const uint32_t *labels, uint32_t *ckey, uint64_t *cedge, uint64_t n);
hipError_t launch_mst_emit(hipStream_t st, const uint32_t *labels, const uint32_t *ckey, const uint64_t *cedge, uint64_t n, uint32_t *parent,
                           uint32_t cap, uint32_t *err, const MstEdges &e);

constexpr uint32_t kDbSlab = 512;
hipError_t launch_db_degree(hipStream_t st, const float *vals, const ThrRows &g, float t, int descending, uint32_t *degree);
hipError_t launch_db_band(hipStream_t st, const float *vals, const ThrRows &g, float t, int descending, const uint32_t *degree,
                          uint32_t min_pts, int assign_best, uint32_t *parent, uint32_t cap, uint32_t *err, uint64_t *best);
hipError_t launch_db_labels(hipStream_t st, uint32_t *parent, uint64_t n, uint32_t cap, const uint32_t *degree, const uint64_t *best,
                            uint32_t min_pts, uint32_t *labels, uint8_t *kind_out, uint32_t *degree_out, uint64_t *n_clusters,
                            uint64_t *n_noise, uint32_t *err);

hipError_t launch_hist(hipStream_t st, const float *vals, const ThrRows &g, const float *d_edges, uint32_t n_edges, const uint32_t *labels,
                       int descending, uint32_t cus, uint64_t *counts);
size_t hist_lds_bytes(uint32_t n_edges, int planes);

constexpr int kPairsMaxP16 = 15;
struct PairsTypes {
    int t[9];
};
hipError_t launch_pairs_hist(hipStream_t st, const uint8_t *regs, uint64_t n, int p, const uint32_t *lhs, const uint32_t *rhs,
                             uint64_t first, uint64_t xbase, uint64_t cnt, void *hist, unsigned long long *err);
hipError_t launch_pairs_card(hipStream_t st, const void *hist, uint64_t first, uint64_t cnt, int p, int estim, double *card);
hipError_t launch_pairs_finish(hipStream_t st, const void *hist, const uint32_t *lhs, const uint32_t *rhs, uint64_t n, uint64_t cnt,
                               int p, int estim, const double *card, const PairsTypes &types, uint32_t n_types, double ksinv,
                               float *out, uint64_t out_stride);

hipError_t launch_fold(hipStream_t st, const uint8_t *src, uint64_t n, int ps, int pd, uint64_t row0, uint8_t *dst,
                       unsigned long long *err);
hipError_t launch_union_groups(hipStream_t st, const uint8_t *src, int p, const uint64_t *ptr, const uint32_t *mem,
                               const uint32_t *dst, uint64_t nv, uint8_t *out_a, uint8_t *out_b);

hipError_t launch_upload(hipStream_t st, void *dst, const void *src_pinned, size_t bytes);

struct SketchWork {
    uint64_t gbeg;
    uint64_t gend;
    uint64_t start;
    uint32_t nsub;
    uint32_t slot;
};
hipError_t launch_sketch(hipStream_t st, const uint8_t *seq, const SketchWork *work,
                         uint32_t nwork, int k, int p, int canon, uint8_t *regs);

constexpr uint32_t kRecRunSpan = 8192;
constexpr uint32_t kRecRunSegs = 256;
constexpr uint32_t kRecRunRecs = 4096;
constexpr int kMaxPRecords = 17;
struct RecRun {
    uint64_t base;
    uint32_t seg0, nseg;
    uint32_t slot0, nrec;
    uint32_t span;
    uint32_t pad_;
};
hipError_t launch_sketch_records(hipStream_t st, const uint8_t *seq, const RecRun *runs, uint32_t nruns, const uint2 *segs,
                                 int k, int p, int canon, uint8_t *regs);
hipError_t launch_zero_rows(hipStream_t st, const uint32_t *slots, uint32_t nslots, int p, uint8_t *regs);

constexpr uint32_t kFastxChunk = 16384;
struct FastxChunk {
    uint64_t begin;
    uint32_t len, genome;
};
struct FastxGenome {
    uint64_t off, rawlen, region_end;
    uint32_t chunk0, nchunks;
    uint32_t fmt, pad_;
};
struct FastxSumm {
    uint32_t fn, bad8;
    uint32_t a[4], b[4];
};
hipError_t launch_fastx_decode(hipStream_t st, const uint8_t *raw, const FastxChunk *chunks, uint32_t nchunks,
                               const FastxGenome *genomes, uint32_t ngenomes, FastxSumm *summ, uint4 *state, uint64_t *declen,
                               uint32_t *status, unsigned long long *fingerprint, uint8_t *out);

hipError_t preload_compare_kernels();
hipError_t preload_hist_kernels();
hipError_t preload_knn_kernels();
hipError_t preload_exchange_kernels();
hipError_t preload_fastx_kernels();
hipError_t preload_sketch_kernels();

hipError_t ensure_dynamic_lds(const void *kernel, size_t bytes);

}
```

### dashing_amd/csrc/kernels_compare.hip

```cpp
#include <hip/hip_runtime.h>
#include <stdint.h>

#include <algorithm>

#include "estimators.h"
#include "kernels.h"

namespace dsh {

template <typename PT>
__global__ __launch_bounds__(256, 4) void k_selfhist_card(const uint8_t *__restrict__ regs, uint64_t first,
                                                        uint64_t n, int p, int estim, int emax, int elow,
                                                        uint32_t *__restrict__ hist_out,
                                                        PT *__restrict__ exc,
                                                        uint8_t *__restrict__ excv,
                                                        uint32_t *__restrict__ exc_n,
                                                        uint32_t *__restrict__ keys,
                                                        uint8_t *__restrict__ tailhist)
{
    __shared__ uint32_t hist[4][64];
    __shared__ uint32_t sub[4][8][72];
    __shared__ int thr[4], thrL[4];
    const int tid = threadIdx.x, lane = tid & 63, wave = tid >> 6;
    const uint64_t s = first + (uint64_t)blockIdx.x * 4 + wave;
#pragma unroll
    for (int k = 0; k < 8; ++k) sub[wave][k][lane] = 0;
    __syncthreads();
    const uint64_t m = 1ull << p;
    const uint4 *src = reinterpret_cast<const uint4 *>(regs + (s < n ? s : 0) * m);
    const uint64_t nch = m >> 4;
    constexpr int kRegCache = 16;
    uint4 cache[kRegCache];
#pragma unroll
    for (int k = 0; k < kRegCache; ++k) {
        const uint64_t c = (uint64_t)k * 64 + lane;
        cache[k] = src[c < nch ? c : nch - 1];
    }
#pragma unroll
    for (int k = 0; k < kRegCache; ++k)
        if (!(s < n && (uint64_t)k * 64 + lane < nch)) cache[k] = make_uint4(0, 0, 0, 0);
    uint32_t bad = 0;
    const uint32_t limrep = (uint32_t)(64 - p + 2) * 0x01010101u;
    if (s < n) {
        uint32_t *mysub = sub[wave][lane & 7];
        auto count16 = [mysub, limrep, &bad](const uint4 x) {
            const uint32_t w[4] = {x.x, x.y, x.z, x.w};
#pragma unroll
            for (int k = 0; k < 4; ++k) {
                bad |= (w[k] | (((w[k] & 0x7F7F7F7Fu) | 0x80808080u) - limrep)) & 0x80808080u;
                atomicAdd(&mysub[w[k] & 63], 1u);
                atomicAdd(&mysub[(w[k] >> 8) & 63], 1u);
                atomicAdd(&mysub[(w[k] >> 16) & 63], 1u);
                atomicAdd(&mysub[(w[k] >> 24) & 63], 1u);
            }
        };
#pragma unroll
        for (int k = 0; k < kRegCache; ++k)
            if ((uint64_t)k * 64 + lane < nch) count16(cache[k]);
        for (uint64_t c = (uint64_t)kRegCache * 64 + lane; c < nch; c += 64) count16(src[c]);
    }
    __syncthreads();
    {
        uint32_t t = 0;
#pragma unroll
        for (int k = 0; k < 8; ++k) t += sub[wave][k][lane];
        hist[wave][lane] = t;
    }
    __syncthreads();
    if (s < n && lane == 0) {
        const uint32_t *h = hist[wave];
        int lo = 0, hi = 63;
        while (lo < 63 && h[lo] == 0) ++lo;
        while (hi > 0 && h[hi] == 0) --hi;
        int T = hi;
        uint32_t cnt = 0;
        while (T > lo && cnt + h[T] <= (uint32_t)emax) {
            cnt += h[T];
            --T;
        }
        int L = lo;
        uint32_t cntl = 0;
        while (L < T && cntl + h[L] <= (uint32_t)elow) {
            cntl += h[L];
            ++L;
        }
        thr[wave] = T;
        thrL[wave] = L;
        exc_n[s] = cnt + cntl;
        keys[s] = ((uint32_t)hi << 18) | ((uint32_t)T << 12) | ((uint32_t)L << 6) | (uint32_t)lo;
    }
    if (s < n && __any(bad != 0) && lane == 0) atomicOr(&keys[s], 0x80000000u);
    __syncthreads();
    if (s >= n) return;
    const uint32_t T = (uint32_t)thr[wave], L = (uint32_t)thrL[wave];
    tailhist[s * 64 + lane] = (uint32_t)lane > T ? (uint8_t)hist[wave][lane] : (uint8_t)0;
    hist_out[s * 64 + lane] = hist[wave][lane];
    if (emax == 0 && elow == 0) return;
    PT *dstp = exc + s * kListCap;
    uint8_t *dstv = excv + s * kListCap;
    const uint32_t trep = (T + 1) * 0x01010101u, lrep = L * 0x01010101u;
    auto hits = [trep, lrep](uint32_t x) -> uint32_t {
        const uint32_t ge = ((x | 0x80808080u) - trep) & 0x80808080u;
        const uint32_t lt = ~((x | 0x80808080u) - lrep) & 0x80808080u;
        return ge | lt;
    };
    uint32_t mine = 0;
#pragma unroll
    for (int k = 0; k < kRegCache; ++k)
        if ((uint64_t)k * 64 + lane < nch) {
            const uint32_t w[4] = {cache[k].x, cache[k].y, cache[k].z, cache[k].w};
#pragma unroll
            for (int q = 0; q < 4; ++q) mine += (uint32_t)__popc(hits(w[q]));
        }
    for (uint64_t c = (uint64_t)kRegCache * 64 + lane; c < nch; c += 64) {
        const uint4 x = src[c];
        mine += (uint32_t)(__popc(hits(x.x)) + __popc(hits(x.y)) + __popc(hits(x.z)) + __popc(hits(x.w)));
    }
    uint32_t slot = mine;
#pragma unroll
    for (int d = 1; d < 64; d <<= 1) {
        const uint32_t o = __shfl_up(slot, d, 64);
        if (lane >= d) slot += o;
    }
    slot -= mine;
    auto emit4 = [&](uint32_t x, uint32_t pos0) {
        uint32_t h = hits(x);
        while (h) {
            const uint32_t b = (uint32_t)__builtin_ctz(h) >> 3;
            h &= h - 1;
            if (slot < kListCap) {
                dstp[slot] = (PT)(pos0 + b);
                dstv[slot] = (uint8_t)((x >> (8 * b)) & 0xFFu);
            }
            ++slot;
        }
    };
#pragma unroll
    for (int k = 0; k < kRegCache; ++k) {
        const uint64_t c = (uint64_t)k * 64 + lane;
        if (c < nch) {
            const uint32_t w[4] = {cache[k].x, cache[k].y, cache[k].z, cache[k].w};
#pragma unroll
            for (int q = 0; q < 4; ++q) emit4(w[q], (uint32_t)(c * 16 + q * 4));
        }
    }
    for (uint64_t c = (uint64_t)kRegCache * 64 + lane; c < nch; c += 64) {
        const uint4 x = src[c];
        emit4(x.x, (uint32_t)(c * 16));
        emit4(x.y, (uint32_t)(c * 16 + 4));
        emit4(x.z, (uint32_t)(c * 16 + 8));
        emit4(x.w, (uint32_t)(c * 16 + 12));
    }
}

__global__ __launch_bounds__(64) void k_card_from_hist(const uint32_t *__restrict__ hist, const uint32_t *__restrict__ keys,
                                                       uint64_t first, uint64_t n, int p, int estim, double *__restrict__ card)
{
    const uint64_t s = first + (uint64_t)blockIdx.x * 64 + threadIdx.x;
    if (s >= n) return;
    const uint32_t *h = hist + s * 64;
    struct Bins {
        const uint32_t *h;
        enum { stride = 1 };
        __device__ uint32_t operator()(int v) const { return h[v & 63]; }
        __device__ const uint32_t *at(int v) const { return h + v; }
    };
    const Bins c{h};
    const uint32_t key = keys[s];
    card[s] = estimate(c, c, p, estim, (int)(key & 63u), (int)((key >> 18) & 63u));
}

template <typename PT, int RK>
// ... 1031 lines not shown
            atomicAdd(&a.phase_cyc[12], (unsigned long long)mx_bins);
            atomicAdd(&a.phase_cyc[13], (unsigned long long)(mx_it * mx_bins));
        }
    }
}

template <typename CT, int RK, bool TIMED, bool GENERAL>
__global__ __launch_bounds__(128) __attribute__((amdgpu_waves_per_eu(8, 8), amdgpu_num_sgpr(96))) void k_finalize(FinalizeArgs a)
{
    finalize_block<CT, RK, TIMED, GENERAL>(a);
}

template <typename CT, int RK>
__global__ __launch_bounds__(128) __attribute__((amdgpu_waves_per_eu(8, 8), amdgpu_num_sgpr(96))) void k_finalize_signal(FinalizeArgs a)
{
    finalize_block<CT, RK, false, false>(a);
    if (a.sig == nullptr) return;
    const uint32_t tidx = finalize_row_of_block().tidx;
    if (tidx >= a.ntiles) return;
    asm volatile("s_waitcnt vmcnt(0)" ::: "memory");
    __builtin_amdgcn_fence(__ATOMIC_RELEASE, "workgroup");
    __syncthreads();
    if (threadIdx.x == 0) {
        uint32_t *sig = a.sig;
        if (atomicAdd(sig + kSigTileCnt + tidx, 1u) == kTile - 1) {
            atomicExch(sig + kSigTileCnt + tidx, 0u);
            const uint32_t q = a.tiles[tidx].w >> 16;
            if (atomicAdd(sig + kSigPartCnt + q, 1u) + 1u == sig[kSigPartTotal + q]) {
                if (sig[kSigStamp]) reinterpret_cast<unsigned long long *>(sig + kSigPartTime)[q] = wall_clock64();
                __hip_atomic_store(sig + kSigPartFlag + q, sig[kSigGen], __ATOMIC_RELEASE, __HIP_MEMORY_SCOPE_SYSTEM);
            }
        }
    }
}

__global__ void k_wall_stamp(unsigned long long *out) { *out = wall_clock64(); }

hipError_t launch_wall_stamp(hipStream_t st, unsigned long long *out)
{
    hipLaunchKernelGGL(k_wall_stamp, dim3(1), dim3(1), 0, st, out);
    return hipGetLastError();
}

hipError_t preload_compare_kernels()
{
    hipFuncAttributes fa;
    return hipFuncGetAttributes(&fa, reinterpret_cast<const void *>(k_wall_stamp));
}

__global__ __launch_bounds__(256) void k_upload(uint32_t *__restrict__ dst, const uint32_t *__restrict__ src, uint64_t nwords)
{
    const uint64_t stride = (uint64_t)gridDim.x * 256;
    for (uint64_t w = (uint64_t)blockIdx.x * 256 + threadIdx.x; w < nwords; w += stride) dst[w] = src[w];
}

__global__ __launch_bounds__(256) void k_upload_segs(UploadSegs u)
{
    const UploadSeg g = u.s[blockIdx.y];
    const uint64_t stride = (uint64_t)gridDim.x * 256;
    for (uint64_t w = (uint64_t)blockIdx.x * 256 + threadIdx.x; w < g.nwords; w += stride) g.dst[w] = g.src[w];
}

hipError_t launch_upload_segs(hipStream_t st, const UploadSegs &u, uint32_t nseg)
{
    uint64_t most = 0;
    for (uint32_t i = 0; i < nseg; ++i) most = std::max(most, u.s[i].nwords);
    if (!nseg || !most) return hipSuccess;
    const uint32_t blocks = (uint32_t)std::min<uint64_t>(256, (most + 255) / 256);
    hipLaunchKernelGGL(k_upload_segs, dim3(blocks, nseg), dim3(256), 0, st, u);
    return hipGetLastError();
}

hipError_t launch_upload(hipStream_t st, void *dst, const void *src_pinned, size_t bytes)
{
    if (bytes == 0) return hipSuccess;
    const uint64_t nwords = (bytes + 3) / 4;
    const uint32_t blocks = (uint32_t)std::min<uint64_t>(256, (nwords + 255) / 256);
    hipLaunchKernelGGL(k_upload, dim3(blocks), dim3(256), 0, st, (uint32_t *)dst, (const uint32_t *)src_pinned, nwords);
    return hipGetLastError();
}

hipError_t launch_selfhist_card(hipStream_t st, const uint8_t *regs, uint64_t first, uint64_t n, int p, int estim,
                                int emax, int elow, uint32_t *hist, void *exc, uint8_t *excv, uint32_t *exc_n,
                                uint32_t *keys, uint8_t *tailhist)
{
    if (n <= first) return hipSuccess;
    const uint32_t blocks = (uint32_t)((n - first + 3) / 4);
    if (p <= 15)
        hipLaunchKernelGGL(k_selfhist_card<uint16_t>, dim3(blocks), dim3(256), 0, st, regs, first, n, p, estim, emax, elow,
                           hist, (uint16_t *)exc, excv, exc_n, keys, tailhist);
    else
        hipLaunchKernelGGL(k_selfhist_card<uint32_t>, dim3(blocks), dim3(256), 0, st, regs, first, n, p, estim, emax, elow,
                           hist, (uint32_t *)exc, excv, exc_n, keys, tailhist);
    return hipGetLastError();
}

hipError_t launch_card_from_hist(hipStream_t st, const uint32_t *hist, const uint32_t *keys, uint64_t first, uint64_t n, int p,
                                 int estim, double *card)
{
    if (n <= first) return hipSuccess;
    hipLaunchKernelGGL(k_card_from_hist, dim3((uint32_t)((n - first + 63) / 64)), dim3(64), 0, st, hist, keys, first, n, p, estim, card);
    return hipGetLastError();
}

hipError_t launch_build_colindex(hipStream_t st, const ColIndexLaunch &c)
{
    if (c.nblocks == 0) return hipSuccess;
    uint32_t G = 1;
    while (G < 4 && c.nblocks * G < 256 && c.nbuckets / (2 * G) >= 4096) G *= 2;
    const size_t lds = (size_t)(c.nbuckets / G) * sizeof(uint32_t);
#define DSH_COLINDEX(PT, RK)                                                                                                  \
    do {                                                                                                                      \
        hipError_t e = ensure_dynamic_lds(reinterpret_cast<const void *>(k_build_colindex<PT, RK>), lds);                     \
        if (e != hipSuccess) return e;                                                                                        \
        hipLaunchKernelGGL((k_build_colindex<PT, RK>), dim3(c.nblocks, G), dim3(1024), lds, st, (const PT *)c.exc, c.excv,    \
                           c.exc_n, c.keys, c.card, c.tailhist, c.perm, c.ncols, c.p, c.nbuckets, c.ent_stride, c.E, c.rec,    \
                           c.ent, c.nS, c.keyS, c.cardS, c.thS, c.rl);                                                         \
    } while (0)
    if (c.p > 15) DSH_COLINDEX(uint32_t, 3);
    else if (colindex_inline(c.p, c.E) == 3) DSH_COLINDEX(uint16_t, 3);
    else DSH_COLINDEX(uint16_t, 7);
#undef DSH_COLINDEX
    return hipGetLastError();
}

hipError_t launch_transform(hipStream_t st, const uint8_t *regs, uint64_t n, int p, int vlo,
                            uint32_t P, uint32_t W, uint32_t Npad, uint32_t *planes,
                            const uint32_t *perm)
{
    if (P == 0) return hipSuccess;
    if (p >= 8 && ((uint64_t)1 << p) / 256 <= 65535) {
        hipLaunchKernelGGL(k_transform_t, dim3(Npad / 64, (uint32_t)(((uint64_t)1 << p) / 256)), dim3(256), 0, st, regs,
                           n, p, vlo, P, W, Npad, planes, perm);
        return hipGetLastError();
    }
    const uint64_t threads = (uint64_t)Npad * W;
    const uint32_t blocks = (uint32_t)((threads + 255) / 256);
    hipLaunchKernelGGL(k_transform, dim3(blocks), dim3(256), 0, st, regs, n, p, vlo, P, W, Npad,
                       planes, perm);
    return hipGetLastError();
}

template <int KC, int U, typename CT>
static hipError_t launch_pc(hipStream_t st, const uint32_t *planes, uint32_t Npad, uint32_t Kpad,
                            uint32_t W, uint32_t P, const uint4 *tiles, const uint4 *items,
                            uint32_t nitems, void *cum, uint64_t nslots)
{
    const size_t lds = (size_t)KC * 2048;
    hipError_t e = ensure_dynamic_lds(reinterpret_cast<const void *>(k_pair_counts<KC, U, CT>), lds);
    if (e != hipSuccess) return e;
    hipLaunchKernelGGL((k_pair_counts<KC, U, CT>), dim3(nitems), dim3(256), lds, st, planes, Npad,
                       Kpad, W, P, tiles, items, reinterpret_cast<CT *>(cum), nslots);
    return hipGetLastError();
}

template <int KC, typename CT>
static hipError_t launch_pc_u(hipStream_t st, const uint32_t *planes, uint32_t Npad,
                              uint32_t Kpad, uint32_t W, uint32_t P, const uint4 *tiles,
                              const uint4 *items, uint32_t nitems, void *cum, uint64_t nslots)
{
    if (W >= 8) return launch_pc<KC, 8, CT>(st, planes, Npad, Kpad, W, P, tiles, items, nitems, cum, nslots);
    if (W == 4) return launch_pc<KC, 4, CT>(st, planes, Npad, Kpad, W, P, tiles, items, nitems, cum, nslots);
    if (W == 2) return launch_pc<KC, 2, CT>(st, planes, Npad, Kpad, W, P, tiles, items, nitems, cum, nslots);
    return launch_pc<KC, 1, CT>(st, planes, Npad, Kpad, W, P, tiles, items, nitems, cum, nslots);
}

hipError_t launch_pair_counts(hipStream_t st, int kc, int cum_bytes, const uint32_t *planes,
                              uint32_t Npad, uint32_t Kpad, uint32_t W, uint32_t P,
                              const uint4 *tiles, const uint4 *items, uint32_t nitems, void *cum,
                              uint64_t nslots)
{
    if (nitems == 0 || Kpad == 0) return hipSuccess;
    if (cum_bytes == 2) {
        switch (kc) {
        case 16: return launch_pc_u<16, uint16_t>(st, planes, Npad, Kpad, W, P, tiles, items, nitems, cum, nslots);
        case 32: return launch_pc_u<32, uint16_t>(st, planes, Npad, Kpad, W, P, tiles, items, nitems, cum, nslots);
// ... 84 lines not shown
```

### dashing_amd/csrc/plan.cpp

```cpp
#include "plan.h"

#include <algorithm>
#include <cstring>

namespace dsh {
namespace plan {

uint64_t tri_index(uint64_t n, uint64_t i, uint64_t j) { return i * (2 * n - i - 1) / 2 + j - (i + 1); }

uint64_t tri_span(uint64_t n, uint64_t rb, uint64_t re)
{
    if (re > n) re = n;
    if (rb >= re) return 0;
    const uint64_t cnt = re - rb;
    return cnt * (n - 1) - (rb + re - 1) * cnt / 2;
}

uint64_t tri_band_end(uint64_t n, uint64_t b0, uint64_t re, uint64_t band_floats, uint64_t row_cap)
{
    const uint64_t max_rows = std::min<uint64_t>(std::max<uint64_t>(row_cap, 1), kBandMaxRows);
    uint64_t b1 = b0, span = 0;
    do {
        span += n - 1 - b1;
        ++b1;
// ... 330 lines not shown
                while (u < NT && cost[r] + (double)(NT - u) <= limit) cost[r] += (double)(NT - u), deal[u++ - t_pool] = r;
            }
            for (; u < NT; ++u) {
                uint32_t to = 0;
                for (uint32_t r = 1; r < world; ++r)
                    if (cost[r] < cost[to]) to = r;
                cost[to] += (double)(NT - u);
                deal[u - t_pool] = to;
            }
            double mx = 0;
            for (uint32_t r = 0; r < world; ++r) mx = std::max(mx, cost[r]);
            size_t segs = 0;
            for (size_t d = 0; d < deal.size(); ++d) segs += d == 0 || deal[d] != deal[d - 1];
            if (sweep == 0) {
                if (best_max < 0 || mx < best_max) best_max = mx;
            } else if (mx <= accept && (best_t == NT + 1 || segs < best_segs)) {
                best_t = t_pool;
                best_segs = segs;
                best_deal = deal;
                best_start = start;
                best_stop = stop;
            }
        }
    }
    if (best_t >= NT && bonus == 0.0) return;
    if (best_t > NT) return;
    rs.seg.clear();
    rs.owner.clear();
    rs.seg.push_back(0);
    auto push = [&](uint64_t end_row, uint32_t who) {
        if (end_row <= rs.seg.back()) return;
        if (!rs.owner.empty() && rs.owner.back() == who) rs.seg.back() = end_row;
        else rs.seg.push_back(end_row), rs.owner.push_back(who);
    };
    for (uint32_t r = 0; r < world; ++r) push(std::min<uint64_t>(n, best_stop[r] * kTile), r);
    for (uint64_t u = best_t; u < NT; ++u) push(std::min<uint64_t>(n, (u + 1) * kTile), best_deal[u - best_t]);
    if (rs.owner.empty()) rs.owner.push_back(0), rs.seg.push_back(n);
    rs.seg.back() = n;
}

void sort_rows_by_key(const uint32_t *k32, uint64_t lo, uint64_t hi, uint32_t *dst, std::vector<uint32_t> &a)
{
    auto skey = [&](uint64_t i) -> uint32_t {
        const uint32_t key = k32[i];
        return ((uint32_t)key_T(key) << 12) | ((uint32_t)key_L(key) << 6) | (uint32_t)key_hi(key);
    };
    const uint64_t cnt_ = hi - lo;
    if (a.size() < 2 * cnt_) a.resize(2 * cnt_);
    uint32_t *const ks = a.data() + cnt_;
    uint32_t c0[513], c1[513];
    std::memset(c0, 0, sizeof c0);
    std::memset(c1, 0, sizeof c1);
    for (uint64_t i = 0; i < cnt_; ++i) {
        const uint32_t k = skey(lo + i);
        ks[i] = k;
        c0[(k & 511u) + 1u]++;
        c1[(k >> 9) + 1u]++;
    }
    for (int k = 1; k < 513; ++k) c0[k] += c0[k - 1], c1[k] += c1[k - 1];
    for (uint64_t i = 0; i < cnt_; ++i) a[c0[ks[i] & 511u]++] = (uint32_t)i;
    for (uint64_t i = 0; i < cnt_; ++i) dst[c1[ks[a[i]] >> 9]++] = (uint32_t)(lo + a[i]);
}

void rowsorted_offsets(uint64_t n, const uint32_t *order, uint64_t cnt, std::vector<uint64_t> &rowoff)
{
    rowoff.resize(cnt + 1);
    uint64_t acc = 0;
    for (uint64_t s = 0; s < cnt; ++s) {
        rowoff[s] = acc;
        acc += n - 1 - order[s];
    }
    rowoff[cnt] = acc;
}

void tile_planes(const Layout &L, uint32_t ti, uint32_t tj, int &pb, int &pe)
{
    const int lo_t = std::max<int>(std::max<int>(L.blk_lo[ti], L.blk_lo[tj]), std::min<int>(L.blk_L[ti], L.blk_L[tj]));
    const int T_t = std::max<int>(L.blk_T[ti], L.blk_T[tj]);
    pb = std::max(0, lo_t - L.pbase);
    pe = std::max(pb, T_t - L.pbase);
}

void build_layout(const uint32_t *k32, uint64_t n, int want_sorted, uint64_t rb, uint64_t re,
                  const std::vector<uint64_t> &parts, Layout &L, uint32_t rowsorted_nparts, const std::vector<uint64_t> *extra_in)
{
    if (re > n) re = n;
    if (!want_sorted) rb = 0, re = n;
    if (rb > re) rb = re;
    static const std::vector<uint64_t> kNoExtra;
    const std::vector<uint64_t> &extra = (want_sorted && extra_in && rb < re) ? *extra_in : kNoExtra;
    const uint64_t col0 = want_sorted ? rb : 0;
    const uint64_t ncols = n - col0;
    int vr[3] = {63, 0, 0};
    for (uint64_t i = col0; i < n; ++i) {
        const uint32_t key = k32[i];
        vr[0] = std::min<int>(vr[0], key_lo(key));
        vr[1] = std::max<int>(vr[1], key_hi(key));
        vr[2] = std::max<int>(vr[2], key_T(key));
    }
    if (ncols == 0) vr[0] = vr[1] = vr[2] = 0;
    L.sorted = want_sorted;
    L.rb = rb;
    L.re = re;
    L.rowsorted = want_sorted && rowsorted_nparts > 0;
    L.extra = extra;
    if (L.rowsorted) {
        const uint64_t x = rowsorted_split(n, rb, re);
        if (x > rb && x < re) L.parts = {rb, x, re};
        else L.parts = {rb, re};
    } else if (!extra.empty()) {
        L.parts = {rb, re};
    } else {
        L.parts = want_sorted ? parts : std::vector<uint64_t>();
    }
    L.n = n;
    L.vlo = vr[0];
    L.vhi = vr[1];
    L.ncols = ncols;
    L.Npad = (uint32_t)((ncols + kTile - 1) / kTile * kTile);
    L.whole = want_sorted && rb == 0 && re == n;
    L.perm.resize(ncols);
    L.part_pos.clear();
    L.part_w.clear();
    L.rowoff.clear();
    L.rowoff_w.clear();
    L.wtr.clear();
    L.wtr_w.clear();
    L.nwanted = want_sorted ? rowset_rows(rb, re, extra) : n;
    if (want_sorted) {
        for (size_t q = 0; q + 1 < L.parts.size(); ++q)
            sort_rows_by_key(k32, L.parts[q], L.parts[q + 1], L.perm.data() + (L.parts[q] - rb), L.sort_a);
        uint64_t at = re;
        for (size_t x = 0; x + 1 < extra.size(); x += 2) {
            if (extra[x] > at) sort_rows_by_key(k32, at, extra[x], L.perm.data() + (at - rb), L.sort_a);
            sort_rows_by_key(k32, extra[x], extra[x + 1], L.perm.data() + (extra[x] - rb), L.sort_a);
            at = extra[x + 1];
        }
        if (at < n) sort_rows_by_key(k32, at, n, L.perm.data() + (at - rb), L.sort_a);
        std::vector<std::pair<uint64_t, uint64_t>> wsegs;
        wanted_order(n, rb, re, &extra, wsegs, L.rowsorted);
        uint64_t wrows = 0;
        for (auto &sg : wsegs) {
            L.wtr.emplace_back((uint32_t)((sg.first - rb) / kTile), (uint32_t)((sg.second - rb + kTile - 1) / kTile));
            L.wtr_w.push_back(wrows);
            wrows += sg.second - sg.first;
        }
        const uint64_t wend = extra.empty() ? re - rb : extra.back() - rb;
        if (L.rowsorted) {
            rowsorted_part_positions(n, rb, re, rowsorted_nparts, L.part_w, &extra);
            L.rowoff_w.resize(L.nwanted + 1);
            L.rowoff.assign(wend + 1, 0);
            uint64_t acc = 0, w = 0;
            for (auto &sg : wsegs)
                for (uint64_t s = sg.first - rb; s < sg.second - rb; ++s, ++w) {
                    L.rowoff_w[w] = L.rowoff[s] = acc;
                    acc += n - 1 - L.perm[s];
                }
            L.rowoff_w[L.nwanted] = acc;
        } else if (!extra.empty()) {
            L.part_w = {0, L.nwanted};
        } else {
            for (uint64_t r : L.parts) L.part_w.push_back(r - rb);
        }
        if (extra.empty()) L.part_pos = L.part_w;
        else L.part_pos = {0, wend};
        if (L.whole) {
            L.perm.resize(2 * n);
            for (uint64_t s = 0; s < n; ++s) L.perm[n + L.perm[s]] = (uint32_t)s;
        }
    } else {
        for (uint64_t i = 0; i < n; ++i) L.perm[i] = (uint32_t)i;
    }
    const uint32_t NT = L.Npad / kTile;
    L.blk_T.assign(NT, 0);
    L.blk_lo.assign(NT, 255);
    L.blk_L.assign(NT, 255);
    L.blk_hi.assign(NT, 0);
    int pbase = vr[2];
    const uint32_t *perm = L.perm.data();
    for (uint32_t b = 0; b < NT; ++b) {
        const uint64_t s0 = (uint64_t)b * kTile, s1 = std::min<uint64_t>(ncols, s0 + kTile);
        int bt = 0, blo = 255, bl = 255, bhi = 0;
        for (uint64_t s = s0; s < s1; ++s) {
            const uint32_t key = k32[perm[s]];
            bt = std::max(bt, key_T(key));
            blo = std::min(blo, key_lo(key));
            bl = std::min(bl, key_L(key));
            bhi = std::max(bhi, key_hi(key));
        }
        L.blk_T[b] = (uint8_t)bt;
        L.blk_lo[b] = (uint8_t)blo;
        L.blk_L[b] = (uint8_t)bl;
        L.blk_hi[b] = (uint8_t)bhi;
        pbase = std::min(pbase, bl);
    }
    L.pbase = pbase;
    L.P = (uint32_t)(vr[2] - pbase);
}

static void xcd_order(std::vector<U4> &t, std::vector<uint32_t> &rank, size_t b, size_t e, size_t group)
{
    const size_t cnt = e - b;
    if (cnt < 16) return;
    std::vector<U4> tmp(cnt);
    std::vector<uint32_t> rtmp(cnt);
    const size_t nx = 8, per = (cnt + nx - 1) / nx;
    size_t q = 0;
    for (size_t r = 0; r < per; r += group)
        for (size_t x = 0; x < nx; ++x)
            for (size_t u = 0; u < group && r + u < per; ++u) {
                const size_t src = x * per + r + u;
                if (src < cnt) {
                    rtmp[q] = rank[b + src];
                    tmp[q++] = t[b + src];
                }
            }
    std::copy(tmp.begin(), tmp.begin() + q, t.begin() + b);
    std::copy(rtmp.begin(), rtmp.begin() + q, rank.begin() + b);
}

static void tile_vrange(const Layout &L, const U4 &t, int &lo, int &hi)
{
    lo = std::min<int>(L.blk_lo[t.x], L.blk_lo[t.y]);
    hi = std::max<int>(L.blk_hi[t.x], L.blk_hi[t.y]);
    if (hi < lo) hi = lo;
}

bool build_tiles(const Layout &L, const PairQuery &job, const Tuning &tu, PairPlan &pp)
{
    std::vector<U4> &T = pp.T;
    T.clear();
    pp.bands.clear();
    pp.band_items.clear();
    pp.segs.clear();
    pp.items.clear();
    pp.band_frags.clear();
    pp.band_round.clear();
    pp.nparts = 0;
    pp.max_band = 0;
    const uint32_t NT = L.Npad / kTile;
    const uint8_t *bLo = L.blk_lo.data(), *bL = L.blk_L.data(), *bT = L.blk_T.data();
    const int pbase = L.pbase;
    auto tile_row = [&](uint32_t ti, uint32_t c0, uint32_t c1) {
        const size_t at = T.size();
        T.resize(at + (c1 - c0));
        U4 *out = T.data() + at;
        const int lo_i = bLo[ti], L_i = bL[ti], T_i = bT[ti];
        for (uint32_t tj = c0; tj < c1; ++tj) {
            const int lo_t = std::max(std::max<int>(lo_i, bLo[tj]), std::min<int>(L_i, bL[tj]));
            const int pb = std::max(0, lo_t - pbase), pe = std::max(pb, std::max<int>(T_i, bT[tj]) - pbase);
            *out++ = U4{ti, tj, (uint32_t)pb, (uint32_t)pe};
        }
    };
    std::vector<size_t> trow_first;
    std::vector<uint64_t> trow_w;
    if (job.rect) {
        if (job.row_begin >= job.row_end || job.col_begin >= job.col_end) return false;
        const uint32_t r0 = (uint32_t)(job.row_begin / kTile), r1 = (uint32_t)((job.row_end + kTile - 1) / kTile);
        const uint32_t c0 = (uint32_t)(job.col_begin / kTile), c1 = (uint32_t)((job.col_end + kTile - 1) / kTile);
        T.reserve((size_t)(r1 - r0) * (c1 - c0));
        for (uint32_t ti = r0; ti < r1; ++ti) tile_row(ti, c0, c1);
    } else {
        if (job.row_begin >= job.row_end) return false;
        if (!L.sorted || job.sorted_rows) {
            const uint32_t r0 = (uint32_t)(job.row_begin / kTile);
            const uint32_t r1 = std::min<uint32_t>(NT, (uint32_t)((job.row_end + kTile - 1) / kTile));
            if (r1 > r0) T.reserve((size_t)(r1 - r0) * (NT - r0) - (size_t)(r1 - r0) * (r1 - r0 - 1) / 2);
            for (uint32_t ti = r0; ti < r1; ++ti) tile_row(ti, ti, NT);
        } else {
            size_t cnt = 0;
            for (const auto &w : L.wtr)
                for (uint32_t ti = w.first; ti < std::min(w.second, NT); ++ti) cnt += NT - ti;
            T.reserve(cnt);
            for (size_t k = 0; k < L.wtr.size(); ++k)
                for (uint32_t ti = L.wtr[k].first; ti < std::min(L.wtr[k].second, NT); ++ti) {
                    trow_first.push_back(T.size());
                    trow_w.push_back(L.wtr_w[k] + (uint64_t)(ti - L.wtr[k].first) * kTile);
                    tile_row(ti, ti, NT);
                }
        }
    }
    if (T.empty()) return false;
    pp.per_tile_bytes = (uint64_t)kTile * kTile * tu.cum_bytes * std::max<uint32_t>(L.P, 1);
    const uint64_t max_tiles = std::min<uint64_t>(65536, std::max<uint64_t>(1, tu.cum_budget / pp.per_tile_bytes));
    const size_t kPartBandTiles = tu.part_band_tiles;
    const bool parts_on = job.want_parts && !job.rect && !job.sorted_rows && L.sorted && L.part_w.size() >= 2;
    std::vector<size_t> pstart{0};
    if (parts_on) {
        size_t q = 0;
        for (size_t r = 0; r < trow_first.size(); ++r)
            while (q + 2 < L.part_w.size() && trow_w[r] >= L.part_w[q + 1]) {
                ++q;
                pstart.push_back(trow_first[r]);
            }
        pp.nparts = (uint32_t)pstart.size();
    }
    pstart.push_back(T.size());
    pp.part_first = pstart;
    pp.part_tiles.clear();
    if (parts_on)
        for (size_t q = 0; q + 1 < pstart.size(); ++q) pp.part_tiles.push_back((uint32_t)(pstart[q + 1] - pstart[q]));
    auto part_of_tile = [&](size_t t) -> size_t {
        return (size_t)(std::upper_bound(pstart.begin(), pstart.end() - 1, t) - pstart.begin()) - 1;
    };
    std::vector<size_t> cuts;
    if (parts_on && pp.nparts >= 2 && tu.tail_bands > 0 && tu.lockstep && tu.W >= (uint32_t)tu.kc && tu.nsplit == 0 && tu.round_items > 0) {
        const uint64_t RI = tu.round_items;
        uint64_t items = 0;
        for (const U4 &t : T) items += t.w - t.z;
        const uint64_t R = (items + RI - 1) / RI;
        constexpr uint64_t kBandRounds = 16;
        for (uint32_t ntails = tu.tail_bands; ntails >= 1 && cuts.empty() && items <= 4 * kBandRounds * RI && R >= 3; --ntails) {
            std::vector<uint64_t> tails;
            uint64_t left = R;
            for (uint32_t b = 0; b < ntails; ++b) {
                const uint64_t pm = b == 0 ? tu.tail_permille : tu.tail_permille2;
                const uint64_t r = std::max<uint64_t>(1, (left * pm + 500) / 1000);
                if (left < r + 2 || (b > 0 && left < r + tu.tail_head_min_rounds)) break;
                tails.push_back(r);
                left -= r;
            }
            std::vector<uint64_t> quota;
            {
                const uint64_t nb = (left + kBandRounds - 1) / kBandRounds;
                for (uint64_t b = 0; b < nb; ++b) quota.push_back(left / nb + (b < left % nb ? 1 : 0));
            }
            for (size_t b = tails.size(); b-- > 0;) {
                const uint64_t nb = (tails[b] + kBandRounds - 1) / kBandRounds;
                for (uint64_t x = 0; x < nb; ++x) quota.push_back(tails[b] / nb + (x < tails[b] % nb ? 1 : 0));
            }
            uint64_t acc = 0, rounds = 0, band_items = 0;
            size_t t = 0;
            for (size_t b = 0; b + 1 < quota.size(); ++b) {
                while (t < T.size() && band_items + (T[t].w - T[t].z) <= quota[b] * RI) {
                    acc += T[t].w - T[t].z;
                    band_items += T[t].w - T[t].z;
                    ++t;
                }
                if (t == 0 || t >= T.size() || (!cuts.empty() && cuts.back() == t)) continue;
                cuts.push_back(t);
                rounds += (band_items + RI - 1) / RI;
                band_items = 0;
            }
            rounds += (items - acc + band_items + RI - 1) / RI;
            if (rounds != R && !(R > kBandRounds && rounds == R + 1)) cuts.clear();
        }
    }
    size_t next_cut = 0;
    for (size_t b = 0; b < T.size();) {
        size_t e = std::min<size_t>(T.size(), b + max_tiles);
        if (parts_on) {
            const size_t q = part_of_tile(b);
            if (pstart[q + 1] - pstart[q] >= kPartBandTiles) e = std::min(e, pstart[q + 1]);
        }
        while (next_cut < cuts.size() && cuts[next_cut] <= b) ++next_cut;
        if (next_cut < cuts.size()) e = std::min(e, cuts[next_cut]);
        pp.bands.emplace_back(b, e);
        b = e;
    }
    pp.segs.resize(pp.bands.size());
    for (size_t bi = 0; bi < pp.bands.size(); ++bi) {
        size_t b = pp.bands[bi].first;
        while (b < pp.bands[bi].second) {
            const size_t q = part_of_tile(b);
            const size_t e = std::min(pp.bands[bi].second, pstart[q + 1]);
            const bool last_of_part = e == pstart[q + 1];
            Seg sg{b, e, parts_on && last_of_part ? (int)q : -1, 1};
            for (size_t t = b; t < e; ++t) {
                int lo, hi;
                tile_vrange(L, T[t], lo, hi);
                sg.hist_bins = std::max(sg.hist_bins, hi - lo + 1);
            }
            pp.segs[bi].push_back(sg);
            b = e;
        }
    }
    std::vector<uint32_t> &rank = pp.rank;
    rank.resize(T.size());
    for (auto &sv : pp.segs)
        for (auto &sg : sv)
            for (size_t t = sg.b; t < sg.e; ++t) rank[t] = (uint32_t)(t - sg.b);
    for (auto &sv : pp.segs)
        for (auto &sg : sv) xcd_order(T, rank, sg.b, sg.e, tu.lockstep ? 2 : 1);
    const uint32_t KC = (uint32_t)tu.kc;
    const uint32_t cpp = tu.W >= KC ? tu.W / KC : 1;
    std::vector<U2> &CR = pp.chunks;
    CR.resize(T.size());
    if (tu.W >= KC) {
        for (size_t t = 0; t < T.size(); ++t) CR[t] = U2{T[t].z * cpp, T[t].w * cpp};
    } else {
        for (size_t t = 0; t < T.size(); ++t)
            CR[t] = U2{(uint32_t)(((uint64_t)T[t].z * tu.W) / KC), (uint32_t)(((uint64_t)T[t].w * tu.W + KC - 1) / KC)};
    }
    for (auto &bd : pp.bands) pp.max_band = std::max(pp.max_band, bd.second - bd.first);
    return true;
}

static void overflow_fragments(const Tuning &tu, uint64_t RI, uint32_t cpp, uint64_t piece, uint64_t ni, uint64_t &over, uint32_t &f)
{
    over = 0;
    f = 1;
    if (!tu.lockstep || tu.nsplit != 0 || RI == 0 || tu.overflow_frag_max_permille == 0 || piece != cpp || cpp < 2 || ni == 0) return;
    const uint64_t o = ni % RI;
    if (o == 0 || o * 1000 > RI * tu.overflow_frag_max_permille) return;
    uint32_t ff = 1;
    while (ff * 2 <= cpp && o * (ff * 2) <= RI) ff *= 2;
    if (ff < 2) return;
    over = o;
    f = ff;
}

static uint32_t band_round_items(const Tuning &tu, uint64_t ni)
{
    if (!tu.lockstep || tu.small_round_items == 0 || tu.small_round_items >= tu.round_items) return tu.round_items;
    return ni <= 2 * (uint64_t)tu.small_round_items ? tu.small_round_items : tu.round_items;
}

void build_band_items(const Tuning &tu, PairPlan &pp, size_t bi)
{
    const auto &bd = pp.bands[bi];
    const std::vector<U2> &CR = pp.chunks;
    std::vector<U4> &I = pp.items;
    const uint32_t KC = (uint32_t)tu.kc;
    const uint32_t cpp = tu.W >= KC ? tu.W / KC : 1;
    const size_t nt = bd.second - bd.first;
    uint64_t tot = 0;
    uint32_t maxlen = 0;
    for (size_t t = bd.first; t < bd.second; ++t) {
        const uint32_t len = CR[t].y - CR[t].x;
        tot += len;
        maxlen = std::max(maxlen, len);
    }
    uint64_t piece = tu.nsplit > 0 ? std::max<uint64_t>(1, (tot / std::max<size_t>(nt, 1) + tu.nsplit - 1) / tu.nsplit)
                                   : std::max<uint64_t>(1, tot / (16 * 512));
    if (tu.nsplit == 0 && tu.lockstep)
        piece = std::min<uint64_t>(piece, std::max<uint64_t>(cpp, (uint64_t)tu.ls_item_chunks));
    piece = (piece + cpp - 1) / cpp * cpp;
    const size_t i0 = I.size();
    const uint32_t maxpieces = (uint32_t)((maxlen + piece - 1) / piece);
    const bool by_length = tu.lockstep && piece <= 65536;
    std::vector<uint32_t> &first = pp.sort_first;
    for (uint32_t s = 0; s < maxpieces; ++s) {
        const size_t g0 = I.size();
        const uint64_t off = (uint64_t)s * piece;
        size_t cnt = 0;
        uint32_t lmin = ~0u, lmax = 0;
        if (by_length) first.assign((size_t)piece + 2, 0);
        for (size_t t = bd.first; t < bd.second; ++t) {
            const uint64_t b0 = CR[t].x + off;
            if (b0 >= CR[t].y) continue;
            const uint32_t len = (uint32_t)std::min<uint64_t>(CR[t].y - b0, piece);
            ++cnt;
            lmin = std::min(lmin, len);
            lmax = std::max(lmax, len);
            if (by_length) ++first[piece - len + 1];
        }
        I.resize(g0 + cnt);
        U4 *out = I.data() + g0;
        const bool place = by_length && lmin != lmax;
        if (place)
            for (size_t v = 1; v < first.size(); ++v) first[v] += first[v - 1];
        for (size_t t = bd.first; t < bd.second; ++t) {
            const uint64_t b0 = CR[t].x + off;
            if (b0 >= CR[t].y) continue;
            const uint32_t len = (uint32_t)std::min<uint64_t>(CR[t].y - b0, piece);
            const U4 it{(uint32_t)(t - bd.first), (uint32_t)b0, (uint32_t)b0 + len, 0};
            if (place) out[first[piece - len]++] = it;
            else *out++ = it;
        }
        if (!by_length && tu.lockstep && lmin != lmax)
            std::stable_sort(I.begin() + g0, I.end(), [](const U4 &x, const U4 &y) { return x.z - x.y > y.z - y.y; });
    }
// ... 156 lines not shown
```

### dashing_amd/csrc/plan.h

```cpp
#pragma once
#include <stddef.h>
#include <stdint.h>

#include <utility>
#include <vector>

#include "consts.h"

namespace dsh {
namespace plan {

struct U4 { uint32_t x, y, z, w; };
struct U2 { uint32_t x, y; };

inline int key_lo(uint32_t k) { return (int)(k & 63u); }
inline int key_L(uint32_t k) { return (int)((k >> 6) & 63u); }
inline int key_T(uint32_t k) { return (int)((k >> 12) & 63u); }
inline int key_hi(uint32_t k) { return (int)((k >> 18) & 63u); }
inline bool key_bad(uint32_t k) { return (k & 0x80000000u) != 0; }

uint64_t tri_index(uint64_t n, uint64_t i, uint64_t j);
uint64_t tri_span(uint64_t n, uint64_t rb, uint64_t re);
void partition_rows(uint64_t n, uint32_t nparts, uint32_t align, uint64_t *bounds);
void balance_rows(uint64_t n, uint32_t nparts, uint64_t *bounds);
void range_parts(uint64_t n, uint64_t rb, uint64_t re, uint32_t nparts, std::vector<uint64_t> &out);
uint64_t tri_band_end(uint64_t n, uint64_t b0, uint64_t re, uint64_t band_floats, uint64_t row_cap);
uint64_t rect_band_rows(uint64_t ncols, uint64_t band_floats);
bool greedy_old_band(const uint32_t *labels_in, uint64_t m, uint64_t ncols, uint64_t from, uint64_t band_floats, uint64_t &b0, uint64_t &b1);
constexpr uint64_t kHistMaxIters = (1u << 18) - 1;
constexpr uint64_t kHistLdsPerCu = 160u << 10;
constexpr uint64_t kHistMaxPerCu = 8;
static_assert(4 * kHistMaxIters * kThrChunk < (1ull << 32), "a workgroup's share of a band must fit its 32-bit counters");
uint64_t hist_grid(uint64_t units, uint64_t lds_bytes, uint32_t cus);

struct RowSets {
    uint32_t world = 0;
    std::vector<uint64_t> seg;
    std::vector<uint32_t> owner;
    size_t words() const { return 3 + 2 * owner.size(); }
    void write(uint64_t *tab) const;
    void rank_rows(uint32_t r, uint64_t &rb, uint64_t &re, std::vector<uint64_t> &extra) const;
};
const char *parse_rowsets(const uint64_t *tab, uint64_t n, RowSets &rs);
void rowsets_from_bounds(const uint64_t *bounds, uint32_t world, RowSets &rs);
constexpr uint64_t kTopupMaxRows = 32768;
void balance_rowsets(uint64_t n, uint32_t world, RowSets &rs, uint32_t prep_permille = ~0u, int dst = -1, uint32_t dst_bonus_permille = ~0u);
void wanted_order(uint64_t n, uint64_t rb, uint64_t re, const std::vector<uint64_t> *extra, std::vector<std::pair<uint64_t, uint64_t>> &segs,
                  bool rowsorted = false);
uint64_t rowsorted_split(uint64_t n, uint64_t rb, uint64_t re);
uint64_t rowset_tiles(uint64_t n, uint64_t rb, uint64_t re, const std::vector<uint64_t> &extra);
uint64_t rowset_rows(uint64_t rb, uint64_t re, const std::vector<uint64_t> &extra);
uint64_t rowset_span(uint64_t n, uint64_t rb, uint64_t re, const std::vector<uint64_t> &extra);

int auto_list_cap(int p, bool upper);

bool rowsorted_rule(uint64_t n, uint64_t rb, uint64_t re, uint32_t nparts);
void rowsorted_part_positions(uint64_t n, uint64_t rb, uint64_t re, uint32_t nparts, std::vector<uint64_t> &pos,
                              const std::vector<uint64_t> *extra = nullptr);
void sort_rows_by_key(const uint32_t *keys, uint64_t lo, uint64_t hi, uint32_t *dst, std::vector<uint32_t> &scratch);
void rowsorted_offsets(uint64_t n, const uint32_t *order, uint64_t cnt, std::vector<uint64_t> &rowoff);

struct Layout {
    int sorted = 0;
    uint64_t rb = 0, re = 0;
    std::vector<uint64_t> extra;
    std::vector<std::pair<uint32_t, uint32_t>> wtr;
    std::vector<uint64_t> wtr_w;
    uint64_t nwanted = 0;
    std::vector<uint64_t> part_w;
    std::vector<uint64_t> rowoff_w;
    std::vector<uint64_t> parts;
    int rowsorted = 0;
    std::vector<uint64_t> part_pos;
    std::vector<uint64_t> rowoff;
    uint64_t n = 0, ncols = 0;
    uint32_t Npad = 0;
    bool whole = false;
    std::vector<uint32_t> perm;
    std::vector<uint8_t> blk_T, blk_lo, blk_L, blk_hi;
    int vlo = 0, vhi = 0;
    int pbase = 0;
    uint32_t P = 0;
    std::vector<uint32_t> sort_a;
};

void build_layout(const uint32_t *keys, uint64_t n, int want_sorted, uint64_t rb, uint64_t re,
                  const std::vector<uint64_t> &parts, Layout &L, uint32_t rowsorted_nparts = 0,
                  const std::vector<uint64_t> *extra = nullptr);

void tile_planes(const Layout &L, uint32_t ti, uint32_t tj, int &pb, int &pe);

struct PairQuery {
    int rect = 0;
    int sorted_rows = 0;
    int want_parts = 0;
    uint64_t row_begin = 0, row_end = 0, col_begin = 0, col_end = 0;
};

struct Tuning {
    uint32_t W = 0;
    int kc = 32;
    int cum_bytes = 2;
    uint64_t cum_budget = 8ull << 30;
    int nsplit = 0;
    bool lockstep = true;
    int ls_item_chunks = 64;
    uint32_t part_band_tiles = 2048;
    uint32_t round_items = 512;
    uint32_t small_round_items = 0;
    uint32_t overflow_frag_max_permille = 500;
    uint32_t tail_bands = 2;
    uint32_t tail_permille = 100;
    uint32_t tail_permille2 = 350;
    uint32_t tail_head_min_rounds = 7;
};

struct Seg {
    size_t b, e;
    int part;
    int hist_bins;
};

struct PairPlan {
    std::vector<U4> T;
    std::vector<std::pair<size_t, size_t>> bands;
    std::vector<std::pair<size_t, size_t>> band_items;
    std::vector<uint32_t> band_round;
    std::vector<std::vector<Seg>> segs;
    std::vector<U4> items;
    std::vector<uint32_t> band_frags;
    std::vector<uint32_t> rank;
    std::vector<U2> chunks;
    uint64_t per_tile_bytes = 0;
    size_t max_band = 0;
    uint32_t nparts = 0;
    std::vector<uint32_t> part_tiles;
    std::vector<size_t> part_first;
    std::vector<uint32_t> sort_first;
    std::vector<U4> sort_tmp;
};

bool build_pairs(const Layout &L, const PairQuery &q, const Tuning &t, PairPlan &pp);
bool build_tiles(const Layout &L, const PairQuery &q, const Tuning &t, PairPlan &pp);
void build_band_items(const Tuning &t, PairPlan &pp, size_t band);
void emit_tile_lists(const Layout &L, const PairPlan &pp, U4 *tiles_out, U4 *ftiles_out);
void emit_band_lists(const Layout &L, const PairPlan &pp, size_t band, U4 *tiles_out, U4 *ftiles_out);
uint64_t band_item_count(const Tuning &t, const PairPlan &pp, size_t band);

}
}
```

Baseline: 3.987 billion pairs/s.

## Route sparse top register planes through list-based sparse count kernels

Adds a sparse-plane path. For sorted triangle jobs, the top one or two value planes of each tile are counted from per-sketch position lists (slabs built on device) instead of dense bitplane popcounts. The planner trims the dense chunk range by those planes and interleaves sparse items across XCDs by column load. The cost is an extra slab build pass, extra memory for the tables, and a second kernel launch per band.

Measured after the change: 4.303 billion pairs/s (median of 6 runs). 7.9% higher.

```diff
diff --git a/dashing_amd/csrc/abi.hip b/dashing_amd/csrc/abi.hip
--- a/dashing_amd/csrc/abi.hip
+++ b/dashing_amd/csrc/abi.hip
@@ -74,6 +74,7 @@
     if ((what & DSH_PRELOAD_SKETCH) && e == hipSuccess) e = preload_fastx_kernels();
     if ((what & DSH_PRELOAD_COMPARE) && e == hipSuccess) e = preload_compare_kernels();
     if ((what & DSH_PRELOAD_COMPARE) && e == hipSuccess) e = preload_hist_kernels();
+    if ((what & DSH_PRELOAD_COMPARE) && e == hipSuccess) e = preload_sparseplane_kernels();
     if ((what & DSH_PRELOAD_COMPARE) && e == hipSuccess) e = preload_knn_kernels();
     if ((what & DSH_PRELOAD_COMPARE) && e == hipSuccess) e = preload_exchange_kernels();
     if (e != hipSuccess) (void)hipGetLastError();
@@ -890,6 +891,10 @@
         for (uint32_t x : c->pp.band_frags) f += x;
         *out = (int64_t)f;
     }
+    else if (!std::strcmp(name, "sparse_items")) *out = (int64_t)c->pp.sp_items.size();
+    else if (!std::strcmp(name, "sparse_plane_us")) *out = (int64_t)(c->sparse_ms * 1000.0);
+    else if (!std::strcmp(name, "sparse_planes")) *out = c->sparse_planes;
+    else if (!std::strcmp(name, "sparse_cap")) *out = c->sparse_cap;
     else if (!std::strcmp(name, "words_per_plane")) *out = c->W;
     else if (!std::strcmp(name, "avg_tile_planes_x100")) {
         uint64_t tot = 0;
@@ -1027,6 +1032,21 @@
         c->overflow_frag_permille = (int)v;
         return DSH_OK;
     }
+    if (!std::strcmp(name, "sparse_planes")) {
+        if (v < -1 || v > 2) return fail(c, DSH_EINVAL, "sparse_planes is -1 (auto), 0 (off), 1 or 2");
+        c->sparse_planes = (int)v;
+        return DSH_OK;
+    }
+    if (!std::strcmp(name, "sparse_lds")) {
+        if (v < 0 || v > 1) return fail(c, DSH_EINVAL, "sparse_lds must be 0 or 1");
+        c->sparse_lds = (int)v;
+        return DSH_OK;
+    }
+    if (!std::strcmp(name, "sparse_cap")) {
+        if (v < 0 || v > (int64_t)plan::kSparseCapMax) return fail(c, DSH_EINVAL, "sparse_cap must be in [0, %u]", plan::kSparseCapMax);
+        c->sparse_cap = (int)v;
+        return DSH_OK;
+    }
     if (!std::strcmp(name, "xch_recv_gate")) {
         if (v < -1 || v > 1) return fail(c, DSH_EINVAL, "xch_recv_gate is -1 (auto), 0 or 1");
         c->xch.recv_gate = (int)v;
diff --git a/dashing_amd/csrc/ctx.h b/dashing_amd/csrc/ctx.h
--- a/dashing_amd/csrc/ctx.h
+++ b/dashing_amd/csrc/ctx.h
@@ -170,6 +170,7 @@
     int wall_clock_khz = 0;
     PinBuf pin_keys;
     const uint32_t *hk32 = nullptr;
+    const uint32_t *hg32 = nullptr;
     bool hk32_valid = false;
     double host_layout_us = 0, host_lists_us = 0, host_keys_wait_us = 0;
     Staging st_perm;
@@ -185,6 +186,16 @@
     int elow_opt = -1;
     int part_band_tiles = 2048;
     int overflow_frag_permille = 500;
+    int sparse_planes = -1;
+    int sparse_cap = (int)dsh::plan::kSparseCapDefault;
+    int sparse_lds = 1;
+    DevBuf sp_tab, sp_lists, sp_len, sp_slabs, sp_items;
+    Staging st_sparse;
+    std::vector<dsh::plan::U2> sp_have;
+    uint64_t sp_serial = 0, lay_serial = 0;
+    uint32_t sp_cap_have = 0;
+    double sparse_ms = 0;
+    std::vector<std::pair<hipEvent_t, hipEvent_t>> ev_sparse;
     int tail_bands = 2;
     std::vector<double> part_ready_ms;
     std::vector<uint64_t> part_floats;
diff --git a/dashing_amd/csrc/engine.hip b/dashing_amd/csrc/engine.hip
--- a/dashing_amd/csrc/engine.hip
+++ b/dashing_amd/csrc/engine.hip
@@ -55,18 +55,19 @@
         HIPCHK(c, c->exc.ensure(std::max<uint64_t>(n, 1) * kListCap * (c->p <= 15 ? 2 : 4)));
         HIPCHK(c, c->excv.ensure(std::max<uint64_t>(n, 1) * kListCap));
         HIPCHK(c, c->exc_n.ensure(std::max<uint64_t>(n, 1) * sizeof(uint32_t)));
-        HIPCHK(c, c->keys.ensure(std::max<uint64_t>(n, 1) * sizeof(uint32_t)));
+        HIPCHK(c, c->keys.ensure(std::max<uint64_t>(n, 1) * 2 * sizeof(uint32_t)));
         HIPCHK(c, c->tailhist.ensure(std::max<uint64_t>(n, 1) * 64));
         HIPCHK(c, c->hist.ensure(std::max<uint64_t>(n, 1) * 64 * sizeof(uint32_t)));
         HIPCHK(c, launch_selfhist_card(c->stream, c->regs, need_from, n, c->p, estim, c->emax, c->elow,
                                        (uint32_t *)c->hist.ptr, c->exc.ptr, (uint8_t *)c->excv.ptr,
                                        (uint32_t *)c->exc_n.ptr, (uint32_t *)c->keys.ptr,
-                                       (uint8_t *)c->tailhist.ptr));
-        HIPCHK(c, c->pin_keys.ensure(std::max<uint64_t>(n, 1) * sizeof(uint32_t)));
+                                       (uint8_t *)c->tailhist.ptr, (uint32_t *)c->keys.ptr + n));
+        HIPCHK(c, c->pin_keys.ensure(std::max<uint64_t>(n, 1) * 2 * sizeof(uint32_t)));
         c->hk32 = (const uint32_t *)c->pin_keys.ptr;
+        c->hg32 = c->hk32 + n;
         if (n > need_from)
             HIPCHK(c, hipMemcpyAsync((uint32_t *)c->pin_keys.ptr + need_from, (const uint32_t *)c->keys.ptr + need_from,
-                                     (n - need_from) * sizeof(uint32_t), hipMemcpyDeviceToHost, c->stream));
+                                     (2 * n - need_from) * sizeof(uint32_t), hipMemcpyDeviceToHost, c->stream));
         HIPCHK(c, c->ev_keys.ensure());
         HIPCHK(c, hipEventRecord(c->ev_keys, c->stream));
         HIPCHK(c, launch_card_from_hist(c->stream, (const uint32_t *)c->hist.ptr, (const uint32_t *)c->keys.ptr, need_from, n,
@@ -108,7 +109,8 @@
         plan::Layout &L = c->lay;
         if (!reuse_host_layout)
             plan::build_layout(k32, n, want_sorted, want_rb, want_re, parts, L, rowsorted ? std::max<uint32_t>(nparts, 1) : 0,
-                               extra->empty() ? nullptr : extra);
+                               extra->empty() ? nullptr : extra, c->hg32);
+        ++c->lay_serial;
         c->lay_built = true;
         c->cum_bytes = c->p <= 15 ? 2 : 4;
         const uint64_t m = 1ull << c->p;
@@ -233,6 +235,17 @@
     return jl;
 }
 
+constexpr uint64_t kSparseSlabBudget = 2ull << 30;
+uint32_t sparse_list_stride(const dsh_ctx *c)
+{
+    return std::max<uint32_t>(8, (std::min<uint32_t>((uint32_t)c->sparse_cap, plan::kSparseCapMax) + 7) / 8 * 8);
+}
+int sparse_wordmajor(const dsh_ctx *c) { return c->sparse_lds && c->p <= 15 ? 1 : 0; }
+uint64_t sparse_slab_bytes(const dsh_ctx *c)
+{
+    return ((uint64_t)16 << c->p) + (uint64_t)kTile * sparse_list_stride(c) * sizeof(uint16_t) + kTile * sizeof(uint32_t);
+}
+
 plan::Tuning tuning_of(const dsh_ctx *c)
 {
     plan::Tuning tu;
@@ -247,6 +260,10 @@
     tu.part_band_tiles = (uint32_t)c->part_band_tiles;
     tu.overflow_frag_max_permille = (uint32_t)c->overflow_frag_permille;
     tu.tail_bands = (uint32_t)c->tail_bands;
+    tu.p = c->p;
+    tu.sparse_planes = c->sparse_planes;
+    tu.sparse_cap = (uint32_t)c->sparse_cap;
+    tu.sparse_max_slabs = (uint32_t)std::min<uint64_t>(1u << 16, kSparseSlabBudget / sparse_slab_bytes(c));
     return tu;
 }
 
@@ -356,6 +373,60 @@
     return DSH_OK;
 }
 
+int prepare_sparse(dsh_ctx *c)
+{
+    const plan::PairPlan &pp = c->pp;
+    const plan::Layout &L = c->lay;
+    const size_t ns = pp.slabs.size(), ni = pp.sp_items.size();
+    const uint32_t cap = sparse_list_stride(c);
+    const uint64_t m = 1ull << c->p;
+    static_assert(sizeof(plan::U2) == sizeof(uint2), "plan::U2 must have the layout of uint2");
+    HIPCHK(c, c->sp_items.ensure(ni * sizeof(uint4)));
+    HIPCHK(c, c->sp_slabs.ensure(ns * sizeof(uint2)));
+    const size_t ib = ni * sizeof(uint4), sb = ns * sizeof(uint2);
+    HIPCHK(c, c->st_sparse.room(ib + sb));
+    uint8_t *h = (uint8_t *)c->st_sparse.ptr();
+    std::memcpy(h, pp.sp_items.data(), ib);
+    std::memcpy(h + ib, pp.slabs.data(), sb);
+    HIPCHK(c, launch_upload(c->stream, c->sp_items.ptr, h, ib));
+    const bool have = c->sp_serial == c->lay_serial && c->sp_cap_have == (cap | (uint32_t)sparse_wordmajor(c) << 31) && c->sp_have.size() == ns &&
+                      std::memcmp(c->sp_have.data(), pp.slabs.data(), sb) == 0;
+    if (!have) {
+        DeviceTimer timer(c, c->stream);
+        c->sp_have.clear();
+        HIPCHK(c, launch_upload(c->stream, c->sp_slabs.ptr, h + ib, sb));
+        HIPCHK(c, c->sp_tab.ensure(ns * m * 16));
+        HIPCHK(c, c->sp_lists.ensure(ns * kTile * (size_t)cap * sizeof(uint16_t)));
+        HIPCHK(c, c->sp_len.ensure(ns * kTile * sizeof(uint32_t)));
+        HIPCHK(c, launch_sparse_build(c->stream, (const uint32_t *)c->planes.ptr, L.Npad, c->W, L.ncols, (const uint2 *)c->sp_slabs.ptr,
+                                      (uint32_t)ns, cap, sparse_wordmajor(c), (uint32_t *)c->sp_tab.ptr, (uint16_t *)c->sp_lists.ptr, (uint32_t *)c->sp_len.ptr));
+        c->sp_have = pp.slabs;
+        c->sp_serial = c->lay_serial;
+        c->sp_cap_have = cap | (uint32_t)sparse_wordmajor(c) << 31;
+        timer.stop(c->prep_ms, true);
+    }
+    HIPCHK(c, c->st_sparse.sent(c->stream));
+    return DSH_OK;
+}
+
+int launch_sparse_items(dsh_ctx *c, size_t bi, uint64_t nslots)
+{
+    const plan::PairPlan &pp = c->pp;
+    if (bi >= pp.band_sp_items.size()) return DSH_OK;
+    const auto &rg = pp.band_sp_items[bi];
+    if (rg.first == rg.second) return DSH_OK;
+    hipEvent_t a = c->profiling ? next_event(c) : nullptr, b = c->profiling ? next_event(c) : nullptr;
+    if (a && b) (void)hipEventRecord(a, c->stream);
+    HIPCHK(c, launch_sparse_count(c->stream, c->cum_bytes, (const uint4 *)c->sp_items.ptr + rg.first, (uint32_t)(rg.second - rg.first),
+                                  sparse_wordmajor(c), (const uint32_t *)c->sp_tab.ptr, (const uint16_t *)c->sp_lists.ptr, (const uint32_t *)c->sp_len.ptr,
+                                  sparse_list_stride(c), 1u << c->p, c->cum.ptr, nslots));
+    if (a && b) {
+        (void)hipEventRecord(b, c->stream);
+        c->ev_sparse.emplace_back(a, b);
+    }
+    return DSH_OK;
+}
+
 int launch_tile_kernel(dsh_ctx *c, const PairRun &r, size_t bi, uint64_t nslots)
 {
     const plan::Layout &L = c->lay;
@@ -430,6 +501,13 @@
         (void)hipEventElapsedTime(&ms, e.first, e.second);
         c->fin_ms += ms;
     }
+    c->sparse_ms = 0;
+    for (auto &e : c->ev_sparse) {
+        float ms = 0;
+        (void)hipEventElapsedTime(&ms, e.first, e.second);
+        c->sparse_ms += ms;
+    }
+    c->ev_sparse.clear();
     auto fill_part_floats = [&] {
         for (size_t i = 0; i < c->part_floats.size(); ++i) {
             if (L.rowsorted && i + 1 < L.part_w.size()) c->part_floats[i] = L.rowoff_w[L.part_w[i + 1]] - L.rowoff_w[L.part_w[i]];
@@ -517,6 +595,8 @@
         HIPCHK(c, hipMemsetAsync(c->phase_cyc.ptr, 0, 16 * sizeof(unsigned long long), c->stream));
     }
     r.fin = finalize_invariants(c, job, jl.with_extra);
+    c->ev_sparse.clear();
+    if (!pp.sp_items.empty() && (rc = prepare_sparse(c))) return rc;
     for (size_t bi = 0; bi < pp.bands.size(); ++bi) {
         const uint64_t nslots = (uint64_t)(pp.bands[bi].second - pp.bands[bi].first) * kTile * kTile;
         if ((rc = upload_band(c, r, bi))) return rc;
@@ -527,6 +607,7 @@
             d = next_event(c);
             if (a) (void)hipEventRecord(a, c->stream);
         }
+        if ((rc = launch_sparse_items(c, bi, nslots))) return rc;
         if ((rc = launch_tile_kernel(c, r, bi, nslots))) return rc;
         if (b) (void)hipEventRecord(b, c->stream);
         if (bi == 0) {
diff --git a/dashing_amd/csrc/host/plan_capi.cpp b/dashing_amd/csrc/host/plan_capi.cpp
--- a/dashing_amd/csrc/host/plan_capi.cpp
+++ b/dashing_amd/csrc/host/plan_capi.cpp
@@ -13,6 +13,14 @@
 using namespace dsh::plan;
 
 namespace {
+
+struct SparseCheck {
+    const uint32_t *gcnt = nullptr;
+    int planes = 0;
+    uint32_t cap = 0;
+    uint32_t *routes = nullptr;
+    uint64_t routes_cap = 0;
+};
 
 struct Err {
     char *buf;
@@ -34,7 +42,7 @@
 static int plan_check(uint64_t n, const uint32_t *keys, int mode, int want_sorted, uint64_t rb, uint64_t re, uint64_t cb,
                       uint64_t ce, uint32_t nparts, int want_parts, int p, uint64_t cum_budget, int lockstep, int nsplit,
                       int ls_item_chunks, const std::vector<uint64_t> &extra, uint64_t *stats, char *err, size_t cap,
-                      uint32_t round_items = 0)
+                      uint32_t round_items = 0, const SparseCheck *sc = nullptr)
 {
     Err E{err, cap};
     if (re > n) re = n;
@@ -48,7 +56,8 @@
     if (want_sorted && !rowsorted) range_parts(n, lrb, lre, std::max<uint32_t>(want_parts ? nparts : 1, 1), parts);
     if (!extra.empty() && !(want_sorted && mode == 0)) return E.fail("extra segments need a sorted triangle layout");
     Layout L;
-    build_layout(keys, n, want_sorted, lrb, lre, parts, L, rowsorted ? std::max<uint32_t>(nparts, 1) : 0, extra.empty() ? nullptr : &extra);
+    build_layout(keys, n, want_sorted, lrb, lre, parts, L, rowsorted ? std::max<uint32_t>(nparts, 1) : 0, extra.empty() ? nullptr : &extra,
+                 sc ? sc->gcnt : nullptr);
     std::vector<std::pair<uint64_t, uint64_t>> wsegs;
     wanted_order(n, lrb, lre, &extra, wsegs, rowsorted);
     auto in_rows = [&](uint64_t i) {
@@ -130,6 +139,8 @@
     tu.ls_item_chunks = ls_item_chunks;
     if (round_items) tu.round_items = round_items;
     if (round_items > 512) tu.small_round_items = 512;
+    tu.p = p;
+    if (sc) tu.sparse_planes = sc->planes, tu.sparse_cap = sc->cap;
     PairQuery q;
     q.rect = mode == 1;
     q.sorted_rows = mode == 2;
@@ -269,6 +280,57 @@
         }
     }
     if (at != T.size()) return E.fail("bands end at %zu of %zu tiles", at, T.size());
+    if (pp.sp.size() != T.size() || pp.band_sp_items.size() != pp.bands.size()) return E.fail("sparse bookkeeping sizes differ");
+    {
+        const uint32_t cpp_ = tu.W >= (uint32_t)tu.kc ? tu.W / tu.kc : 1;
+        std::vector<uint8_t> seen_pl;
+        size_t sat = 0;
+        for (size_t bi = 0; bi < pp.bands.size(); ++bi) {
+            const auto &bd = pp.bands[bi];
+            const auto &rg = pp.band_sp_items[bi];
+            if (rg.first != sat || rg.second < rg.first || rg.second > pp.sp_items.size()) return E.fail("sparse items of band %zu do not follow %zu", bi, sat);
+            sat = rg.second;
+            seen_pl.assign((bd.second - bd.first) * 2, 0);
+            for (size_t k = rg.first; k < rg.second; ++k) {
+                const U4 &I = pp.sp_items[k];
+                if (I.x >= bd.second - bd.first) return E.fail("sparse item %zu names tile %u of band %zu", k, I.x, bi);
+                const size_t t = bd.first + I.x;
+                const uint32_t sp = pp.sp[t];
+                if (I.y >= T[t].w || I.y + sp < T[t].w) return E.fail("sparse item %zu: plane %u is not one of the top %u of tile %zu", k, I.y, sp, t);
+                if (seen_pl[I.x * 2 + (T[t].w - 1 - I.y)]++) return E.fail("plane %u of tile %zu has two sparse items", I.y, t);
+                if (I.z >= pp.slabs.size() || I.w >= pp.slabs.size() || pp.slabs[I.z].x != T[t].x || pp.slabs[I.z].y != I.y ||
+                    pp.slabs[I.w].x != T[t].y || pp.slabs[I.w].y != I.y)
+                    return E.fail("sparse item %zu names the wrong slabs", k);
+                const int v = L.pbase + 1 + (int)I.y;
+                if (sparse_bound(L, T[t].x, v) > tu.sparse_cap || sparse_bound(L, T[t].y, v) > tu.sparse_cap) return E.fail("sparse item %zu: a set may exceed the cap", k);
+                if (sc && sc->gcnt)
+                    for (int side = 0; side < 2; ++side)
+                        for (uint32_t a = 0; a < kTile; ++a) {
+                            const uint64_t sx = (uint64_t)(side ? T[t].y : T[t].x) * kTile + a;
+                            if (sx >= L.ncols) continue;
+                            const uint32_t key = keys[orig(sx)], g = sc->gcnt[orig(sx)];
+                            const uint32_t own = v >= key_T(key) ? (g & 0xFFFFu) : v == key_T(key) - 1 ? g >> 16 : 65535u;
+                            if (own > tu.sparse_cap) return E.fail("sparse item %zu: sketch %llu may hold %u positions", k, (unsigned long long)orig(sx), own);
+                        }
+            }
+            for (size_t t = bd.first; t < bd.second; ++t) {
+                const uint32_t sp = pp.sp[t];
+                if (sp > 2 || sp > T[t].w - T[t].z) return E.fail("tile %zu routes %u planes of %u", t, sp, T[t].w - T[t].z);
+                for (uint32_t x = 0; x < sp; ++x)
+                    if (!seen_pl[(t - bd.first) * 2 + x]) return E.fail("routed plane %u of tile %zu has no sparse item", T[t].w - 1 - x, t);
+                if (tu.W >= (uint32_t)tu.kc && (pp.chunks[t].x != T[t].z * cpp_ || pp.chunks[t].y != (T[t].w - sp) * cpp_))
+                    return E.fail("tile %zu: the dense chunk range is not the planes left over", t);
+            }
+        }
+        if (sat != pp.sp_items.size()) return E.fail("sparse items end at %zu of %zu", sat, pp.sp_items.size());
+        if (sc && sc->routes) {
+            if (T.size() > sc->routes_cap) return E.fail("%zu tiles, room for %llu routes", T.size(), (unsigned long long)sc->routes_cap);
+            for (size_t t = 0; t < T.size(); ++t) {
+                uint32_t *o = sc->routes + 5 * t;
+                o[0] = T[t].x, o[1] = T[t].y, o[2] = T[t].z, o[3] = T[t].w, o[4] = pp.sp[t];
+            }
+        }
+    }
     for (uint32_t qd = 0; qd < pp.nparts; ++qd)
         if (part_done[qd] != 1) return E.fail("part %u never completes", qd);
     if (pp.nparts) {
@@ -319,6 +381,7 @@
     stats[2] = pp.items.size();
     stats[3] = pp.nparts;
     stats[4] = T.empty() ? 0 : planes_sum * 100 / T.size();
+    if (sc) stats[10] = pp.sp_items.size(), stats[11] = pp.slabs.size();
     stats[7] = 0;
     for (size_t b = 0; b < pp.band_items.size(); ++b) {
         const uint32_t nfr = b < pp.band_frags.size() ? pp.band_frags[b] : 0u;
@@ -346,6 +409,23 @@
     if (round_items == 0 || round_items % 256) return E.fail("round_items %u is not a positive multiple of 256", round_items);
     return plan_check(n, keys, mode, want_sorted, rb, re, cb, ce, nparts, want_parts, p, cum_budget, lockstep, nsplit, ls_item_chunks,
                       std::vector<uint64_t>(), stats, err, cap, round_items);
+}
+
+int dshh_plan_check_sparse(uint64_t n, const uint32_t *keys, const uint32_t *gcnt, int mode, int want_sorted, uint64_t rb, uint64_t re,
+                           uint32_t nparts, int want_parts, int p, uint64_t cum_budget, uint32_t round_items, int sparse_planes,
+                           uint32_t sparse_cap, uint64_t *stats, uint32_t *routes, uint64_t routes_cap, char *err, size_t cap)
+{
+    Err E{err, cap};
+    if (round_items == 0 || round_items % 256) return E.fail("round_items %u is not a positive multiple of 256", round_items);
+    SparseCheck sc;
+    sc.gcnt = gcnt;
+    sc.planes = sparse_planes;
+    sc.cap = sparse_cap;
+    sc.routes = routes;
+    sc.routes_cap = routes_cap;
+    stats[10] = stats[11] = 0;
+    return plan_check(n, keys, mode, want_sorted, rb, re, 0, 0, nparts, want_parts, p, cum_budget, 1, 0, 64, std::vector<uint64_t>(), stats, err,
+                      cap, round_items, &sc);
 }
 
 int dshh_plan_check_rowset(uint64_t n, const uint32_t *keys, const uint64_t *tab, uint32_t rank, int rowsorted, uint32_t nparts, int p,
diff --git a/dashing_amd/csrc/kernels.h b/dashing_amd/csrc/kernels.h
--- a/dashing_amd/csrc/kernels.h
+++ b/dashing_amd/csrc/kernels.h
@@ -8,7 +8,7 @@
 
 hipError_t launch_selfhist_card(hipStream_t st, const uint8_t *regs, uint64_t first, uint64_t n, int p, int estim,
                                 int emax, int elow, uint32_t *hist, void *exc, uint8_t *excv, uint32_t *exc_n,
-                                uint32_t *keys, uint8_t *tailhist);
+                                uint32_t *keys, uint8_t *tailhist, uint32_t *gcnt);
 hipError_t launch_card_from_hist(hipStream_t st, const uint32_t *hist, const uint32_t *keys, uint64_t first, uint64_t n, int p,
                                  int estim, double *card);
 inline int colindex_inline(int p, uint32_t E) { return p <= 12 && E <= 256 ? 7 : 3; }
@@ -37,6 +37,11 @@
                               uint32_t Npad, uint32_t Kpad, uint32_t W, uint32_t P,
                               const uint4 *tiles, const uint4 *items, uint32_t nitems, void *cum,
                               uint64_t nslots);
+
+hipError_t launch_sparse_build(hipStream_t st, const uint32_t *planes, uint32_t Npad, uint32_t W, uint64_t ncols, const uint2 *slabs,
+                               uint32_t nslabs, uint32_t cap, int wordmajor, uint32_t *tab, uint16_t *lists, uint32_t *len);
+hipError_t launch_sparse_count(hipStream_t st, int cum_bytes, const uint4 *items, uint32_t nitems, int wordmajor, const uint32_t *tab,
+                               const uint16_t *lists, const uint32_t *len, uint32_t cap, uint32_t m, void *cum, uint64_t nslots);
 
 hipError_t launch_pair_counts_lockstep(hipStream_t st, int kc, int groups, int cum_bytes, const uint32_t *planes,
                                        uint32_t Npad, uint32_t Kpad, uint32_t W, uint32_t P, const uint4 *tiles,
@@ -290,6 +295,7 @@
 
 hipError_t preload_compare_kernels();
 hipError_t preload_hist_kernels();
+hipError_t preload_sparseplane_kernels();
 hipError_t preload_knn_kernels();
 hipError_t preload_exchange_kernels();
 hipError_t preload_fastx_kernels();
diff --git a/dashing_amd/csrc/kernels_compare.hip b/dashing_amd/csrc/kernels_compare.hip
--- a/dashing_amd/csrc/kernels_compare.hip
+++ b/dashing_amd/csrc/kernels_compare.hip
@@ -16,7 +16,8 @@
                                                         uint8_t *__restrict__ excv,
                                                         uint32_t *__restrict__ exc_n,
                                                         uint32_t *__restrict__ keys,
-                                                        uint8_t *__restrict__ tailhist)
+                                                        uint8_t *__restrict__ tailhist,
+                                                        uint32_t *__restrict__ gcnt)
 {
     __shared__ uint32_t hist[4][64];
     __shared__ uint32_t sub[4][8][72];
@@ -88,6 +89,8 @@
         thrL[wave] = L;
         exc_n[s] = cnt + cntl;
         keys[s] = ((uint32_t)hi << 18) | ((uint32_t)T << 12) | ((uint32_t)L << 6) | (uint32_t)lo;
+        const uint32_t g0 = cnt + h[T], g1 = g0 + (T > 0 ? h[T - 1] : 0u);
+        gcnt[s] = (g0 < 65535u ? g0 : 65535u) | ((g1 < 65535u ? g1 : 65535u) << 16);
     }
     if (s < n && __any(bad != 0) && lane == 0) atomicOr(&keys[s], 0x80000000u);
     __syncthreads();
@@ -1285,16 +1288,16 @@
 
 hipError_t launch_selfhist_card(hipStream_t st, const uint8_t *regs, uint64_t first, uint64_t n, int p, int estim,
                                 int emax, int elow, uint32_t *hist, void *exc, uint8_t *excv, uint32_t *exc_n,
-                                uint32_t *keys, uint8_t *tailhist)
+                                uint32_t *keys, uint8_t *tailhist, uint32_t *gcnt)
 {
     if (n <= first) return hipSuccess;
     const uint32_t blocks = (uint32_t)((n - first + 3) / 4);
     if (p <= 15)
         hipLaunchKernelGGL(k_selfhist_card<uint16_t>, dim3(blocks), dim3(256), 0, st, regs, first, n, p, estim, emax, elow,
-                           hist, (uint16_t *)exc, excv, exc_n, keys, tailhist);
+                           hist, (uint16_t *)exc, excv, exc_n, keys, tailhist, gcnt);
     else
         hipLaunchKernelGGL(k_selfhist_card<uint32_t>, dim3(blocks), dim3(256), 0, st, regs, first, n, p, estim, emax, elow,
-                           hist, (uint32_t *)exc, excv, exc_n, keys, tailhist);
+                           hist, (uint32_t *)exc, excv, exc_n, keys, tailhist, gcnt);
     return hipGetLastError();
 }
 
diff --git a/dashing_amd/csrc/kernels_sparseplane.hip b/dashing_amd/csrc/kernels_sparseplane.hip
--- /dev/null
+++ b/dashing_amd/csrc/kernels_sparseplane.hip
@@ -0,0 +1,265 @@
+#include <hip/hip_runtime.h>
+#include <stdint.h>
+
+#include "kernels.h"
+
+namespace dsh {
+
+namespace {
+
+constexpr int kSpChunk = 16;
+constexpr int kSpCounters = 11;
+
+__global__ __launch_bounds__(256) void k_sparse_build(const uint32_t *__restrict__ planes, uint32_t Npad, uint32_t W, uint64_t ncols,
+                                                      const uint2 *__restrict__ slabs, uint32_t nslabs, uint32_t cap, int wordmajor,
+                                                      uint32_t *__restrict__ tab, uint16_t *__restrict__ lists, uint32_t *__restrict__ len)
+{
+    const uint32_t lane = threadIdx.x & 63u;
+    const uint32_t nch = W / kSpChunk;
+    const uint64_t unit = (uint64_t)blockIdx.x * 4 + (threadIdx.x >> 6);
+    if (unit >= (uint64_t)nslabs * 2 * nch) return;
+    const uint32_t ch = (uint32_t)(unit % nch), h = (uint32_t)(unit / nch) & 1u, s = (uint32_t)(unit / (2 * (uint64_t)nch));
+    const uint2 sl = slabs[s];
+    const uint32_t row = h * 64 + lane;
+    const uint64_t col = (uint64_t)sl.x * kTile + row;
+    const uint32_t w0 = ch * kSpChunk;
+    const uint32_t *src = planes + ((uint64_t)sl.y * W + w0) * Npad + col;
+    const uint32_t real = col < ncols ? 0xFFFFFFFFu : 0u;
+    uint32_t x[kSpChunk];
+#pragma unroll
+    for (int k = 0; k < kSpChunk; ++k) x[k] = ~src[(uint64_t)k * Npad] & real;
+    const uint64_t m = (uint64_t)W * 32;
+    uint32_t *trow = tab + ((uint64_t)s * m + (uint64_t)w0 * 32 + lane) * 4 + 2 * h;
+    uint32_t *tcol = tab + ((uint64_t)s * 4 + 2 * h) * m + (uint64_t)w0 * 32 + (lane & 31u);
+#pragma unroll
+    for (int k = 0; k < kSpChunk; ++k) {
+        const uint32_t xx = x[k];
+        uint32_t lo = 0, hi = 0;
+#pragma unroll
+        for (uint32_t b = 0; b < 32; ++b) {
+            const unsigned long long bal = __ballot((xx >> b) & 1u);
+            if (lane == b) {
+                lo = (uint32_t)bal;
+                hi = (uint32_t)(bal >> 32);
+            }
+        }
+        if (wordmajor) {
+            const uint32_t hi2 = __shfl(hi, (int)(lane & 31u), 64);
+            tcol[(lane >> 5) * m + (uint64_t)k * 32] = lane < 32 ? lo : hi2;
+        } else if (lane < 32) {
+            *reinterpret_cast<uint2 *>(trow + (uint64_t)k * 32 * 4) = make_uint2(lo, hi);
+        }
+    }
+    uint32_t mine = 0;
+#pragma unroll
+    for (int k = 0; k < kSpChunk; ++k) mine += (uint32_t)__popc(x[k]);
+    if (!mine) return;
+    uint32_t slot = atomicAdd(&len[(uint64_t)s * kTile + row], mine);
+    uint16_t *dst = lists + ((uint64_t)s * kTile + row) * cap;
+#pragma unroll
+    for (int k = 0; k < kSpChunk; ++k) {
+        uint32_t xx = x[k];
+        while (xx) {
+            const uint32_t b = (uint32_t)__builtin_ctz(xx);
+            xx &= xx - 1;
+            if (slot < cap) dst[slot] = (uint16_t)((w0 + k) * 32 + b);
+            ++slot;
+        }
+    }
+}
+
+__device__ __forceinline__ void csa(uint32_t &h, uint32_t &l, uint32_t a, uint32_t b, uint32_t c)
+{
+    const uint32_t u = a ^ b;
+    h = (a & b) | (u & c);
+    l = u ^ c;
+}
+
+__device__ __forceinline__ void put32(uint16_t *dst, const uint32_t (&v)[32])
+{
+#pragma unroll
+    for (int q = 0; q < 4; ++q)
+        reinterpret_cast<uint4 *>(dst)[q] = make_uint4(v[8 * q] | (v[8 * q + 1] << 16), v[8 * q + 2] | (v[8 * q + 3] << 16),
+                                                       v[8 * q + 4] | (v[8 * q + 5] << 16), v[8 * q + 6] | (v[8 * q + 7] << 16));
+}
+__device__ __forceinline__ void put32(uint32_t *dst, const uint32_t (&v)[32])
+{
+#pragma unroll
+    for (int q = 0; q < 8; ++q) reinterpret_cast<uint4 *>(dst)[q] = make_uint4(v[4 * q], v[4 * q + 1], v[4 * q + 2], v[4 * q + 3]);
+}
+
+template <typename CT>
+__global__ __launch_bounds__(512) void k_sparse_count(const uint4 *__restrict__ items, const uint32_t *__restrict__ tab,
+                                                      const uint16_t *__restrict__ lists, const uint32_t *__restrict__ len, uint32_t cap,
+                                                      uint32_t m, CT *__restrict__ cum, uint64_t nslots)
+{
+    __shared__ uint32_t lenj[kTile];
+    const uint4 it = items[blockIdx.x];
+    const uint32_t tid = threadIdx.x, r = tid >> 2, w = tid & 3u;
+    if (tid < kTile) lenj[tid] = len[(uint64_t)it.w * kTile + tid];
+    __syncthreads();
+    const uint32_t li_all = len[(uint64_t)it.z * kTile + r];
+    const uint32_t li = li_all < cap ? li_all : cap;
+    const uint16_t *lp = lists + ((uint64_t)it.z * kTile + r) * cap;
+    const uint32_t *tb = tab + (uint64_t)it.w * m * 4 + w;
+    uint32_t c[kSpCounters];
+#pragma unroll
+    for (int b = 0; b < kSpCounters; ++b) c[b] = 0;
+    for (uint32_t k0 = 0; k0 < li; k0 += 8) {
+        const uint4 pk = *reinterpret_cast<const uint4 *>(lp + k0);
+        const uint32_t pw[4] = {pk.x, pk.y, pk.z, pk.w};
+        uint32_t x[8];
+#pragma unroll
+        for (int q = 0; q < 8; ++q) {
+            const bool valid = k0 + q < li;
+            const uint32_t pos = valid ? (pw[q >> 1] >> (16 * (q & 1))) & 0xFFFFu : 0u;
+            const uint32_t v = tb[(uint64_t)pos * 4];
+            x[q] = valid ? v : 0u;
+        }
+        uint32_t t0, t1, t2, t3, f0, f1, e;
+        csa(t0, c[0], c[0], x[0], x[1]);
+        csa(t1, c[0], c[0], x[2], x[3]);
+        csa(f0, c[1], c[1], t0, t1);
+        csa(t2, c[0], c[0], x[4], x[5]);
+        csa(t3, c[0], c[0], x[6], x[7]);
+        csa(f1, c[1], c[1], t2, t3);
+        csa(e, c[2], c[2], f0, f1);
+#pragma unroll
+        for (int b = 3; b < kSpCounters; ++b) {
+            const uint32_t carry = c[b] & e;
+            c[b] ^= e;
+            e = carry;
+        }
+    }
+    const uint32_t base = m - li_all;
+    uint32_t out[32];
+#pragma unroll
+    for (int cc = 0; cc < 32; ++cc) {
+        uint32_t cnt = 0;
+#pragma unroll
+        for (int b = 0; b < kSpCounters; ++b) cnt |= ((c[b] >> cc) & 1u) << b;
+        out[cc] = (base - lenj[w * 32 + cc] + cnt) & (sizeof(CT) == 2 ? 0xFFFFu : 0xFFFFFFFFu);
+    }
+    put32(cum + (uint64_t)it.y * nslots + (uint64_t)it.x * (kTile * kTile) + (uint64_t)r * kTile + w * 32, out);
+}
+
+template <typename CT>
+__global__ __launch_bounds__(512) void k_sparse_count_lds(const uint4 *__restrict__ items, uint32_t nitems, const uint32_t *__restrict__ tabw,
+                                                          const uint16_t *__restrict__ lists, const uint32_t *__restrict__ len, uint32_t cap,
+                                                          uint32_t m, CT *__restrict__ cum, uint64_t nslots)
+{
+    extern __shared__ __attribute__((aligned(16))) uint32_t sp_lds[];
+    const uint32_t g = blockIdx.x, item = (g >> 5) * 8 + (g & 7u), w = (g >> 3) & 3u;
+    if (item >= nitems) return;
+    const uint4 it = items[item];
+    const uint32_t tid = threadIdx.x, r = tid >> 2, q = tid & 3u;
+    const uint4 *src = reinterpret_cast<const uint4 *>(tabw + ((uint64_t)it.w * 4 + w) * m);
+    for (uint32_t i = tid; i < m / 4; i += 512) reinterpret_cast<uint4 *>(sp_lds)[i] = src[i];
+    if (tid < 32) sp_lds[m + tid] = len[(uint64_t)it.w * kTile + w * 32 + tid];
+    __syncthreads();
+    const uint32_t li_all = len[(uint64_t)it.z * kTile + r];
+    const uint32_t li = li_all < cap ? li_all : cap;
+    const uint16_t *lp = lists + ((uint64_t)it.z * kTile + r) * cap;
+    uint32_t c[kSpCounters];
+#pragma unroll
+    for (int b = 0; b < kSpCounters; ++b) c[b] = 0;
+    for (uint32_t k0 = 8 * q; k0 < li; k0 += 32) {
+        const uint4 pk = *reinterpret_cast<const uint4 *>(lp + k0);
+        const uint32_t pw[4] = {pk.x, pk.y, pk.z, pk.w};
+        uint32_t x[8];
+#pragma unroll
+        for (int j = 0; j < 8; ++j) {
+            const bool valid = k0 + j < li;
+            const uint32_t pos = valid ? (pw[j >> 1] >> (16 * (j & 1))) & 0xFFFFu : 0u;
+            const uint32_t v = sp_lds[pos];
+            x[j] = valid ? v : 0u;
+        }
+        uint32_t t0, t1, t2, t3, f0, f1, e;
+        csa(t0, c[0], c[0], x[0], x[1]);
+        csa(t1, c[0], c[0], x[2], x[3]);
+        csa(f0, c[1], c[1], t0, t1);
+        csa(t2, c[0], c[0], x[4], x[5]);
+        csa(t3, c[0], c[0], x[6], x[7]);
+        csa(f1, c[1], c[1], t2, t3);
+        csa(e, c[2], c[2], f0, f1);
+#pragma unroll
+        for (int b = 3; b < kSpCounters; ++b) {
+            const uint32_t carry = c[b] & e;
+            c[b] ^= e;
+            e = carry;
+        }
+    }
+#pragma unroll
+    for (int d = 1; d <= 2; d <<= 1) {
+        uint32_t carry = 0;
+#pragma unroll
+        for (int b = 0; b < kSpCounters; ++b) {
+            const uint32_t o = __shfl_xor(c[b], d, 64);
+            const uint32_t u = c[b] ^ o;
+            const uint32_t sum = u ^ carry;
+            carry = (c[b] & o) | (u & carry);
+            c[b] = sum;
+        }
+    }
+    if (q != 0) return;
+    const uint32_t base = m - li_all;
+    uint32_t out[32];
+#pragma unroll
+    for (int cc = 0; cc < 32; ++cc) {
+        uint32_t cnt = 0;
+#pragma unroll
+        for (int b = 0; b < kSpCounters; ++b) cnt |= ((c[b] >> cc) & 1u) << b;
+        out[cc] = (base - sp_lds[m + cc] + cnt) & (sizeof(CT) == 2 ? 0xFFFFu : 0xFFFFFFFFu);
+    }
+    put32(cum + (uint64_t)it.y * nslots + (uint64_t)it.x * (kTile * kTile) + (uint64_t)r * kTile + w * 32, out);
+}
+
+}
+
+hipError_t launch_sparse_build(hipStream_t st, const uint32_t *planes, uint32_t Npad, uint32_t W, uint64_t ncols, const uint2 *slabs,
+                               uint32_t nslabs, uint32_t cap, int wordmajor, uint32_t *tab, uint16_t *lists, uint32_t *len)
+{
+    if (nslabs == 0) return hipSuccess;
+    if (W < kSpChunk || W % kSpChunk || cap % 8) return hipErrorInvalidValue;
+    hipError_t e = hipMemsetAsync(len, 0, (size_t)nslabs * kTile * sizeof(uint32_t), st);
+    if (e != hipSuccess) return e;
+    const uint64_t units = (uint64_t)nslabs * 2 * (W / kSpChunk);
+    hipLaunchKernelGGL(k_sparse_build, dim3((uint32_t)((units + 3) / 4)), dim3(256), 0, st, planes, Npad, W, ncols, slabs, nslabs, cap,
+                       wordmajor, tab, lists, len);
+    return hipGetLastError();
+}
+
+hipError_t launch_sparse_count(hipStream_t st, int cum_bytes, const uint4 *items, uint32_t nitems, int wordmajor, const uint32_t *tab,
+                               const uint16_t *lists, const uint32_t *len, uint32_t cap, uint32_t m, void *cum, uint64_t nslots)
+{
+    if (nitems == 0) return hipSuccess;
+    if (cap % 8 || cap > 2047) return hipErrorInvalidValue;
+    if (wordmajor) {
+        if (m < 512 || m > (1u << 15)) return hipErrorInvalidValue;
+        const size_t lds = (size_t)m * 4 + 32 * 4;
+        const uint32_t grid = (nitems + 7) / 8 * 32;
+#define DSH_SPL(CT)                                                                                                                   \
+    do {                                                                                                                              \
+        const hipError_t e = ensure_dynamic_lds(reinterpret_cast<const void *>(k_sparse_count_lds<CT>), lds);                          \
+        if (e != hipSuccess) return e;                                                                                                \
+        hipLaunchKernelGGL(k_sparse_count_lds<CT>, dim3(grid), dim3(512), lds, st, items, nitems, tab, lists, len, cap, m, (CT *)cum, nslots); \
+    } while (0)
+        if (cum_bytes == 2) DSH_SPL(uint16_t);
+        else DSH_SPL(uint32_t);
+#undef DSH_SPL
+        return hipGetLastError();
+    }
+    if (cum_bytes == 2)
+        hipLaunchKernelGGL(k_sparse_count<uint16_t>, dim3(nitems), dim3(512), 0, st, items, tab, lists, len, cap, m, (uint16_t *)cum, nslots);
+    else
+        hipLaunchKernelGGL(k_sparse_count<uint32_t>, dim3(nitems), dim3(512), 0, st, items, tab, lists, len, cap, m, (uint32_t *)cum, nslots);
+    return hipGetLastError();
+}
+
+hipError_t preload_sparseplane_kernels()
+{
+    hipFuncAttributes fa;
+    return hipFuncGetAttributes(&fa, reinterpret_cast<const void *>(k_sparse_build));
+}
+
+}
diff --git a/dashing_amd/csrc/plan.cpp b/dashing_amd/csrc/plan.cpp
--- a/dashing_amd/csrc/plan.cpp
+++ b/dashing_amd/csrc/plan.cpp
@@ -436,7 +436,8 @@
 }
 
 void build_layout(const uint32_t *k32, uint64_t n, int want_sorted, uint64_t rb, uint64_t re,
-                  const std::vector<uint64_t> &parts, Layout &L, uint32_t rowsorted_nparts, const std::vector<uint64_t> *extra_in)
+                  const std::vector<uint64_t> &parts, Layout &L, uint32_t rowsorted_nparts, const std::vector<uint64_t> *extra_in,
+                  const uint32_t *gcnt)
 {
     if (re > n) re = n;
     if (!want_sorted) rb = 0, re = n;
@@ -530,6 +531,8 @@
     L.blk_lo.assign(NT, 255);
     L.blk_L.assign(NT, 255);
     L.blk_hi.assign(NT, 0);
+    L.blk_g0.assign(gcnt ? NT : 0, 0);
+    L.blk_g1.assign(gcnt ? NT : 0, 0);
     int pbase = vr[2];
     const uint32_t *perm = L.perm.data();
     for (uint32_t b = 0; b < NT; ++b) {
@@ -547,6 +550,16 @@
         L.blk_L[b] = (uint8_t)bl;
         L.blk_hi[b] = (uint8_t)bhi;
         pbase = std::min(pbase, bl);
+        if (gcnt) {
+            uint32_t g0 = 0, g1 = 0;
+            for (uint64_t s = s0; s < s1; ++s) {
+                const uint32_t g = gcnt[perm[s]];
+                g0 = std::max(g0, g & 0xFFFFu);
+                g1 = std::max(g1, key_T(k32[perm[s]]) == bt ? g >> 16 : g & 0xFFFFu);
+            }
+            L.blk_g0[b] = (uint16_t)g0;
+            L.blk_g1[b] = (uint16_t)g1;
+        }
     }
     L.pbase = pbase;
     L.P = (uint32_t)(vr[2] - pbase);
@@ -573,6 +586,23 @@
     std::copy(rtmp.begin(), rtmp.begin() + q, rank.begin() + b);
 }
 
+uint32_t sparse_bound(const Layout &L, uint32_t b, int v)
+{
+    if (b >= L.blk_g0.size()) return 65535u;
+    const int Tb = L.blk_T[b];
+    return v >= Tb ? L.blk_g0[b] : v == Tb - 1 ? L.blk_g1[b] : 65535u;
+}
+
+static uint32_t sparse_route(const Layout &L, uint32_t cap, int nplanes, const U4 &t)
+{
+    uint32_t k = 0;
+    for (; (int)k < nplanes && t.w - k > t.z; ++k) {
+        const int v = L.pbase + (int)(t.w - k);
+        if (std::max(sparse_bound(L, t.x, v), sparse_bound(L, t.y, v)) > cap) break;
+    }
+    return k;
+}
+
 static void tile_vrange(const Layout &L, const U4 &t, int &lo, int &hi)
 {
     lo = std::min<int>(L.blk_lo[t.x], L.blk_lo[t.y]);
@@ -590,6 +620,10 @@
     pp.items.clear();
     pp.band_frags.clear();
     pp.band_round.clear();
+    pp.sp.clear();
+    pp.sp_items.clear();
+    pp.band_sp_items.clear();
+    pp.slabs.clear();
     pp.nparts = 0;
     pp.max_band = 0;
     const uint32_t NT = L.Npad / kTile;
@@ -635,6 +669,14 @@
         }
     }
     if (T.empty()) return false;
+    const uint32_t sp_cap = std::min(tu.sparse_cap, kSparseCapMax);
+    const bool sp_can = tu.sparse_planes != 0 && !job.rect && !job.sorted_rows && L.sorted && !L.blk_g0.empty() && tu.lockstep &&
+                        tu.nsplit == 0 && tu.W >= (uint32_t)tu.kc && tu.p >= 9 && tu.p <= 16 && (tu.sparse_planes > 0 || tu.p >= 13);
+    const int sp_planes = !sp_can ? 0 : tu.sparse_planes < 0 ? kSparseAutoPlanes : std::min(tu.sparse_planes, 2);
+    const uint64_t sp_min_planes = tu.sparse_planes < 0 ? std::max<uint64_t>(tu.small_round_items, 512) : 0;
+    uint64_t job_planes = 0;
+    for (const U4 &t : T) job_planes += t.w - t.z;
+    const int sp_planes_job = job_planes > sp_min_planes ? sp_planes : 0;
     pp.per_tile_bytes = (uint64_t)kTile * kTile * tu.cum_bytes * std::max<uint32_t>(L.P, 1);
     const uint64_t max_tiles = std::min<uint64_t>(65536, std::max<uint64_t>(1, tu.cum_budget / pp.per_tile_bytes));
     const size_t kPartBandTiles = tu.part_band_tiles;
@@ -660,8 +702,9 @@
     std::vector<size_t> cuts;
     if (parts_on && pp.nparts >= 2 && tu.tail_bands > 0 && tu.lockstep && tu.W >= (uint32_t)tu.kc && tu.nsplit == 0 && tu.round_items > 0) {
         const uint64_t RI = tu.round_items;
+        auto dense_planes = [&](const U4 &t) -> uint64_t { return t.w - t.z - (sp_planes_job ? sparse_route(L, sp_cap, sp_planes_job, t) : 0u); };
         uint64_t items = 0;
-        for (const U4 &t : T) items += t.w - t.z;
+        for (const U4 &t : T) items += dense_planes(t);
         const uint64_t R = (items + RI - 1) / RI;
         constexpr uint64_t kBandRounds = 16;
         for (uint32_t ntails = tu.tail_bands; ntails >= 1 && cuts.empty() && items <= 4 * kBandRounds * RI && R >= 3; --ntails) {
@@ -686,9 +729,9 @@
             uint64_t acc = 0, rounds = 0, band_items = 0;
             size_t t = 0;
             for (size_t b = 0; b + 1 < quota.size(); ++b) {
-                while (t < T.size() && band_items + (T[t].w - T[t].z) <= quota[b] * RI) {
-                    acc += T[t].w - T[t].z;
-                    band_items += T[t].w - T[t].z;
+                while (t < T.size() && band_items + dense_planes(T[t]) <= quota[b] * RI) {
+                    acc += dense_planes(T[t]);
+                    band_items += dense_planes(T[t]);
                     ++t;
                 }
                 if (t == 0 || t >= T.size() || (!cuts.empty() && cuts.back() == t)) continue;
@@ -736,12 +779,71 @@
             for (size_t t = sg.b; t < sg.e; ++t) rank[t] = (uint32_t)(t - sg.b);
     for (auto &sv : pp.segs)
         for (auto &sg : sv) xcd_order(T, rank, sg.b, sg.e, tu.lockstep ? 2 : 1);
+    pp.sp.assign(T.size(), 0);
+    pp.band_sp_items.assign(pp.bands.size(), std::make_pair((size_t)0, (size_t)0));
+    if (sp_planes) {
+        pp.slab_of.assign((size_t)NT * std::max<uint32_t>(L.P, 1), -1);
+        auto slab = [&](uint32_t b, uint32_t pl) -> uint32_t {
+            int32_t &s = pp.slab_of[(size_t)b * L.P + pl];
+            if (s < 0) {
+                s = (int32_t)pp.slabs.size();
+                pp.slabs.push_back(U2{b, pl});
+            }
+            return (uint32_t)s;
+        };
+        for (size_t bi = 0; bi < pp.bands.size(); ++bi) {
+            const auto &bd = pp.bands[bi];
+            const size_t i0 = pp.sp_items.size();
+            uint64_t band_planes = 0;
+            for (size_t t = bd.first; t < bd.second; ++t) band_planes += T[t].w - T[t].z;
+            if (band_planes > sp_min_planes)
+                for (size_t t = bd.first; t < bd.second; ++t) {
+                    const uint32_t k = sparse_route(L, sp_cap, sp_planes, T[t]);
+                    if (!k || pp.slabs.size() + 2 * k > tu.sparse_max_slabs) continue;
+                    pp.sp[t] = (uint8_t)k;
+                    for (uint32_t x = 0; x < k; ++x) {
+                        const uint32_t pl = T[t].w - 1 - x;
+                        pp.sp_items.push_back(U4{(uint32_t)(t - bd.first), pl, slab(T[t].x, pl), slab(T[t].y, pl)});
+                    }
+                }
+            const size_t cnt = pp.sp_items.size() - i0;
+            if (cnt > 1) {
+                constexpr size_t nx = 8;
+                std::vector<uint32_t> per_col(NT, 0), cols;
+                for (size_t k = i0; k < pp.sp_items.size(); ++k) per_col[T[bd.first + pp.sp_items[k].x].y]++;
+                for (uint32_t b = 0; b < NT; ++b)
+                    if (per_col[b]) cols.push_back(b);
+                std::stable_sort(cols.begin(), cols.end(), [&](uint32_t a, uint32_t b) { return per_col[a] > per_col[b]; });
+                std::vector<uint32_t> xcd_of(NT, 0);
+                size_t load[nx] = {0};
+                for (uint32_t b : cols) {
+                    size_t x = 0;
+                    for (size_t y = 1; y < nx; ++y)
+                        if (load[y] < load[x]) x = y;
+                    xcd_of[b] = (uint32_t)x;
+                    load[x] += per_col[b];
+                }
+                std::vector<U4> lists[nx];
+                for (size_t k = i0; k < pp.sp_items.size(); ++k) lists[xcd_of[T[bd.first + pp.sp_items[k].x].y]].push_back(pp.sp_items[k]);
+                for (auto &l : lists)
+                    std::stable_sort(l.begin(), l.end(), [&](const U4 &a, const U4 &b) {
+                        const U4 &ta = T[bd.first + a.x], &tb = T[bd.first + b.x];
+                        return ta.y != tb.y ? ta.y < tb.y : a.y != b.y ? a.y > b.y : ta.x < tb.x;
+                    });
+                size_t q = i0;
+                for (size_t r = 0; q < pp.sp_items.size(); ++r)
+                    for (size_t x = 0; x < nx; ++x)
+                        if (r < lists[x].size()) pp.sp_items[q++] = lists[x][r];
+            }
+            pp.band_sp_items[bi] = std::make_pair(i0, pp.sp_items.size());
+        }
+    }
     const uint32_t KC = (uint32_t)tu.kc;
     const uint32_t cpp = tu.W >= KC ? tu.W / KC : 1;
     std::vector<U2> &CR = pp.chunks;
     CR.resize(T.size());
     if (tu.W >= KC) {
-        for (size_t t = 0; t < T.size(); ++t) CR[t] = U2{T[t].z * cpp, T[t].w * cpp};
+        for (size_t t = 0; t < T.size(); ++t) CR[t] = U2{T[t].z * cpp, (T[t].w - pp.sp[t]) * cpp};
     } else {
         for (size_t t = 0; t < T.size(); ++t)
             CR[t] = U2{(uint32_t)(((uint64_t)T[t].z * tu.W) / KC), (uint32_t)(((uint64_t)T[t].w * tu.W + KC - 1) / KC)};
diff --git a/dashing_amd/csrc/plan.h b/dashing_amd/csrc/plan.h
--- a/dashing_amd/csrc/plan.h
+++ b/dashing_amd/csrc/plan.h
@@ -78,6 +78,7 @@
     bool whole = false;
     std::vector<uint32_t> perm;
     std::vector<uint8_t> blk_T, blk_lo, blk_L, blk_hi;
+    std::vector<uint16_t> blk_g0, blk_g1;
     int vlo = 0, vhi = 0;
     int pbase = 0;
     uint32_t P = 0;
@@ -86,7 +87,7 @@
 
 void build_layout(const uint32_t *keys, uint64_t n, int want_sorted, uint64_t rb, uint64_t re,
                   const std::vector<uint64_t> &parts, Layout &L, uint32_t rowsorted_nparts = 0,
-                  const std::vector<uint64_t> *extra = nullptr);
+                  const std::vector<uint64_t> *extra = nullptr, const uint32_t *gcnt = nullptr);
 
 void tile_planes(const Layout &L, uint32_t ti, uint32_t tj, int &pb, int &pe);
 
@@ -96,6 +97,9 @@
     int want_parts = 0;
     uint64_t row_begin = 0, row_end = 0, col_begin = 0, col_end = 0;
 };
+
+constexpr uint32_t kSparseCapDefault = 1280, kSparseCapMax = 2040;
+constexpr int kSparseAutoPlanes = 2;
 
 struct Tuning {
     uint32_t W = 0;
@@ -113,6 +117,10 @@
     uint32_t tail_permille = 100;
     uint32_t tail_permille2 = 350;
     uint32_t tail_head_min_rounds = 7;
+    int sparse_planes = 0;
+    uint32_t sparse_cap = kSparseCapDefault;
+    uint32_t sparse_max_slabs = 1u << 16;
+    int p = 0;
 };
 
 struct Seg {
@@ -138,7 +146,13 @@
     std::vector<size_t> part_first;
     std::vector<uint32_t> sort_first;
     std::vector<U4> sort_tmp;
+    std::vector<uint8_t> sp;
+    std::vector<U4> sp_items;
+    std::vector<std::pair<size_t, size_t>> band_sp_items;
+    std::vector<U2> slabs;
+    std::vector<int32_t> slab_of;
 };
+uint32_t sparse_bound(const Layout &L, uint32_t b, int v);
 
 bool build_pairs(const Layout &L, const PairQuery &q, const Tuning &t, PairPlan &pp);
 bool build_tiles(const Layout &L, const PairQuery &q, const Tuning &t, PairPlan &pp);
```
